# jdalcorso/radar-sounder-crw

Measured on AMD Instinct MI355X. Metric: radargram columns/sec (CRW fwd+bwd), higher is better.
Workload: dtype f32 (conv2-5 multiply on the bf16 matrix cores with hi/lo operand pairs, fp32 accumulate: fp32-grade; everything else fp32); 1 GPU; one synthetic 512x4096 radargram per GPU per step = 8 items [T=32,N=63,16x16] (patch 16x16, overlap (8, 0)), tau=0.01, CNN encoder, fwd+bwd+all-reduce+Adam; parallelism=dp1 (independent sequences), chain=fp32 MFMA 16x16x4, prefix form, encoder_convs=bf16x3

## Files before the change

include/crw_hip.h:

```cpp
#ifndef CRW_HIP_H
#define CRW_HIP_H

#include <stddef.h>
#include <stdint.h>

#ifdef __cplusplus
extern "C" {
#endif

#define CRW_ABI_VERSION 8

#define CRW_OK 0
#define CRW_EINVAL 1
#define CRW_EWORKSPACE 2
#define CRW_EHIP 3

#define CRW_CHAIN_F32 0
#define CRW_CHAIN_BF16 1
#define CRW_CHAIN_BF16X3 2

typedef void *crw_stream_t;

int crw_abi_version(void);
const char *crw_build_arch(void);
int crw_last_hip_error(void);

int crw_padded_nodes(int N, int chain);
size_t crw_walk_state_bytes(int B, int T, int N, int chain);
size_t crw_walk_scratch_bytes(int B, int T, int N, int chain);

size_t crw_affinity_ws_bytes(int B, int T, int N);
int crw_affinity_fwd(const float *emb, int B, int T, int N, int C, float tau,
                     float *ehat, float *norm, float *A, float *stats, void *ws, size_t ws_bytes, crw_stream_t stream);

int crw_walk_fwd(const float *A, const float *stats , int B, int T, int N,
                 int chain, void *state, size_t state_bytes, float *At_out, float *loss, crw_stream_t stream);

int crw_walk_bwd(const float *gloss, const float *A, int B, int T, int N, int chain,
                 void *state, size_t state_bytes, void *scratch, size_t scratch_bytes,
                 float *dA, crw_stream_t stream);

int crw_affinity_bwd(const float *dA, const float *ehat, const float *norm, int B, int T, int N, int C,
                     float tau, float *dehat_ws, float *demb, crw_stream_t stream);

int crw_normalize(const float *emb, int rows, int C, float *ehat, float *norm, crw_stream_t stream);

int crw_labelprop_topk(const float *ehat, int T, int N, int C, int cxt_size, int radius, float temp,
                       int knn, int first_frame, float *W, int32_t *I, crw_stream_t stream);
int crw_labelprop_topk_grid(const float *ehat, int T, int N, int C, int cxt_size, int radius, float temp, int knn, int first_frame,
                            int grid_w, float *W, int32_t *I, crw_stream_t stream);

int crw_labelprop_gather(const float *seed, const float *W, const int32_t *I, int T, int N, int M, int knn,
                         int first_frame, float *L, float *pred, crw_stream_t stream);
int crw_labelprop_propagate(const float *seed, const float *W, const int32_t *I, int T, int N, int M, int knn, int first_frame,
                            int cxt_size, float *L, float *pred, crw_stream_t stream);

int crw_labelprop_topk_scores(const float *ehat, int T, int N, int C, int cxt_size, int radius, float temp, int kcap, int first_frame,
                              int grid_w, float *V, int32_t *I, crw_stream_t stream);
int crw_labelprop_sweep_weights(const float *V, int F, int kcap, int N, const int *knns, int nk, float *W, crw_stream_t stream);
int crw_labelprop_propagate_batch(const float *seed, const float *W, const int32_t *I, size_t i_stride, int G, int T, int N, int M,
                                  int knn, int first_frame, int cxt_size, float *L, float *pred, crw_stream_t stream);

int crw_pelt_rbf(const double *signal, int n, double pen, int min_size, int jump, double gamma, int *bkps, int max_bkps);

int crw_xent_metric(const float *ehat, int T, int N, int C, float *xent, crw_stream_t stream);

#define CRW_DT_F32 0
#define CRW_DT_I8 1
size_t crw_confusion_ws_bytes(size_t P, int K);
int crw_confusion(const void *gt, int gt_dtype, const void *pred, int pred_dtype, const void *aux, int aux_dtype, size_t P, int K,
                  int ignore_gt, int ignore_pred, int ignore_aux, int64_t *counts ,
                  int64_t *dropped , void *ws, size_t ws_bytes, crw_stream_t stream);

#define CRW_CONF_MAXPROB 0
#define CRW_CONF_MARGIN 1
#define CRW_CONF_ENTROPY 2
int crw_labelprop_confidence(const float *L, int T, int N, int M, int kind, int first_frame, float *conf, crw_stream_t stream);

int crw_merge_confidence(const void *fwd_lab, const float *fwd_conf, const void *rev_lab, const float *rev_conf, int lab_dtype,
                         size_t P, void *out_lab, float *out_conf, uint8_t *took, crw_stream_t stream);

size_t crw_calibration_ws_bytes(size_t P, int K, int bins);
int crw_calibration(const void *gt, int gt_dtype, const void *pred, int pred_dtype, const float *conf, const void *aux, int aux_dtype,
                    size_t P, int K, int bins, int ignore_gt, int ignore_pred, int ignore_aux, int64_t *counts ,
                    double *conf_sum , int64_t *dropped , void *ws, size_t ws_bytes, crw_stream_t stream);

size_t crw_linear128_wgrad_ws_bytes(int P);
int crw_linear128_wgrad(const float *dy, const float *x, float *dw, int P, void *ws, size_t ws_bytes, crw_stream_t stream);

int crw_adam_step(float *p, const float *g, float *m, float *v, long n, float lr, float beta1, float beta2, float eps, int step,
                  crw_stream_t stream);

int crw_gemm_f32(const float *A, const float *B, float *C, int n, int batch, int transA, int transB,
                 int beta, crw_stream_t stream);

int crw_enc_pack_weights(const float *w, int cout, int cin, uint16_t *fwd_hi, uint16_t *fwd_lo,
                         uint16_t *bwd_hi, uint16_t *bwd_lo, crw_stream_t stream);
int crw_enc_pack_input(const float *x, int P, int C, uint16_t *x_hi, uint16_t *x_lo, crw_stream_t stream);
int crw_enc_pack_input_map(const float *x, int P, int C, int H, int W, uint16_t *x_hi, uint16_t *x_lo,
                           crw_stream_t stream);
int crw_enc_conv3x3(int mode, int split, int P, int cin, int cout, const uint16_t *x_hi, const uint16_t *x_lo,
                    const uint16_t *w_hi, const uint16_t *w_lo, const float *bias, const uint16_t *mask_hi,
                    uint16_t *y_hi, uint16_t *y_lo, float *y_f32, float *gap, const float *dgap,
                    crw_stream_t stream);
int crw_enc_conv3x3_map(int mode, int split, int P, int H, int W, int cin, int cout, const uint16_t *x_hi, const uint16_t *x_lo,
                        const uint16_t *w_hi, const uint16_t *w_lo, const float *bias, const uint16_t *mask_hi,
                        uint16_t *y_hi, uint16_t *y_lo, float *y_f32, float *gap_part, crw_stream_t stream);
int crw_enc_conv3x3_wgrad_map(int split, int P, int H, int W, int cin, int cout, const uint16_t *dy_hi, const uint16_t *dy_lo,
                              const uint16_t *x_hi, const uint16_t *x_lo, float *dw, float *db, void *ws, size_t ws_bytes,
                              crw_stream_t stream);
int crw_enc_gap_bwd(const float *dgap, const uint16_t *y_hi, int P, int C, int npix, uint16_t *dy_hi, uint16_t *dy_lo,
                    crw_stream_t stream);
size_t crw_enc_wgrad_ws_bytes(int P, int cin, int cout, int split);
int crw_enc_conv3x3_wgrad(int split, int P, int cin, int cout, const uint16_t *dy_hi, const uint16_t *dy_lo,
                          const uint16_t *x_hi, const uint16_t *x_lo, const float *dgap, float *dw, float *db,
                          void *ws, size_t ws_bytes, crw_stream_t stream);

int crw_enc_front_pack(const float *w2, uint16_t *fwd_hi, uint16_t *fwd_lo, uint16_t *bwd_hi, uint16_t *bwd_lo,
                       crw_stream_t stream);
size_t crw_enc_front_saved_bytes(int P);
int crw_enc_front_fwd(int split, const float *x, int P, int cin, const float *w1, const float *b1,
                      const uint16_t *w2_hi, const uint16_t *w2_lo, const float *b2, uint16_t *y_hi,
                      uint16_t *y_lo, void *saved, crw_stream_t stream);
int crw_enc_front_fwd_map(int split, const float *x, int P, int cin, int H, int W, const float *w1, const float *b1,
                          const uint16_t *w2_hi, const uint16_t *w2_lo, const float *b2, uint16_t *y_hi, uint16_t *y_lo,
                          crw_stream_t stream);
size_t crw_enc_front_ws_bytes(int P, int cin);
int crw_enc_front_bwd(int split, const float *x, int P, int cin, const float *w1, const float *b1,
                      const uint16_t *w2_hi, const uint16_t *w2_lo, const float *b2, const uint16_t *w2b_hi,
                      const uint16_t *w2b_lo, const float *dy, const void *saved, float *dw1, float *db1, float *dw2,
                      float *db2, void *ws, size_t ws_bytes, crw_stream_t stream);

int crw_enc_front_bwd_map(int split, const float *x, int P, int cin, int H, int W, const float *w1, const float *b1,
                          const uint16_t *w2_hi, const uint16_t *w2_lo, const float *b2, const uint16_t *w2b_hi,
                          const uint16_t *w2b_lo, const float *dy, float *dw1, float *db1, float *dw2, float *db2,
                          void *ws, size_t ws_bytes, crw_stream_t stream);

int crw_rn_padded_patches(int P);
int crw_rn_pack_conv(const float *w, int cout, int cin, int kh, int kw, uint16_t *fwd_hi, uint16_t *fwd_lo, uint16_t *bwd_hi,
                     uint16_t *bwd_lo, crw_stream_t stream);
int crw_rn_stem_toeplitz_ld(int w);
int crw_rn_stem_cols(int w);
int crw_rn_pack_stem(const float *w1, int h, int w, uint16_t *fwd_hi, uint16_t *fwd_lo, uint16_t *toep_hi, uint16_t *toep_lo,
                     crw_stream_t stream);
size_t crw_rn_conv_part_floats(int P, int G, int N);
int crw_rn_conv(int mode, int P, int Hs, int Ws, int Cs, int Hd, int Wd, int N, int kh, int kw, int stride, int pad,
                const uint16_t *a_hi, const uint16_t *a_lo, const uint16_t *b_hi, const uint16_t *b_lo, const float *bias, float *out,
                float *part, crw_stream_t stream);
size_t crw_rn_wgrad_ws_bytes(int mode, int P, int Hin, int Win, int Cin, int Hout, int Wout, int Cout, int kh, int kw, int stride, int pad);
int crw_rn_wgrad(int mode, int P, int Hin, int Win, int Cin, int Hout, int Wout, int Cout, int kh, int kw, int stride, int pad,
                 const uint16_t *x_hi, const uint16_t *x_lo, const uint16_t *d_hi, const uint16_t *d_lo, float *dw, void *ws,
                 size_t ws_bytes, crw_stream_t stream);
size_t crw_rn_bn_stats_ws_bytes(int C);
int crw_rn_bn_stats(const float *part, int P, int G, int C, const float *gamma, const float *beta, float *run_mean, float *run_var,
                    float momentum, float eps, float *coef, void *ws, size_t ws_bytes, crw_stream_t stream);
int crw_rn_bn_stats_rows(const float *part, int rows, double count, int C, const float *gamma, const float *beta, float *run_mean,
                         float *run_var, float momentum, float eps, float *coef, void *ws, size_t ws_bytes, crw_stream_t stream);
int crw_rn_bn_apply(const float *Z, const float *coef, const float *Zd, const float *coef_d, const uint16_t *res_hi,
                    const uint16_t *res_lo, int P, int npix, int C, int relu, uint16_t *y_hi, uint16_t *y_lo, crw_stream_t stream);
int crw_rn_bn_pool(const float *Z, const float *coef, int P, int H, int W, int C, uint16_t *y_hi, uint16_t *y_lo, uint8_t *amax,
                   crw_stream_t stream);
size_t crw_rn_bn_bwd_ws_bytes(int P, int npix, int C);
int crw_rn_bn_bwd(const float *g1, const float *g2, const uint16_t *mask_hi, const float *Z, const float *coef, const float *Zd,
                  const float *coef_d, int P, int npix, int C, uint16_t *dz_hi, uint16_t *dz_lo, uint16_t *dzd_hi, uint16_t *dzd_lo,
                  float *g_out, float *dgamma, float *dbeta, float *dgamma_d, float *dbeta_d, void *ws, size_t ws_bytes,
                  crw_stream_t stream);
size_t crw_rn_pool_bwd_ws_bytes(int P, int H, int W, int C);
int crw_rn_pool_bwd(const float *d1, const float *d2, const uint8_t *amax, const float *Z, const float *coef, int P, int H, int W, int C,
                    uint16_t *dz_hi, uint16_t *dz_lo, float *dgamma, float *dbeta, void *ws, size_t ws_bytes, crw_stream_t stream);
size_t crw_rn_stem_ws_bytes(void);
int crw_rn_stem_fwd(const float *x, int P, int cin, int h, int w, int Hm, int Wm, const float *w0, const float *b0, const float *gamma,
                    const float *beta, float *run_mean, float *run_var, float momentum, float eps, uint16_t *map_hi, uint16_t *map_lo,
                    float *stem, void *ws, size_t ws_bytes, crw_stream_t stream);
int crw_rn_stem_bwd(const float *dX0, const float *x, const float *stem, const float *w0, const float *b0, int P, int cin, int h, int w,
                    float *dw0, float *db0, float *dgamma, float *dbeta, void *ws, size_t ws_bytes, crw_stream_t stream);
int crw_rn_stem_stats(const float *x, int P, int cin, int h, int w, const float *w0, const float *b0, const float *gamma, const float *beta,
                      float *run_mean, float *run_var, float momentum, float eps, float *stem, void *ws, size_t ws_bytes,
                      crw_stream_t stream);
int crw_rn_stem16_rows(void);
int crw_rn_pack_stem16(const float *w1, uint16_t *wf, uint16_t *wt, crw_stream_t stream);
int crw_rn_stem16_fwd(const float *x, int P, int cin, const float *stem, const uint16_t *wf, float *Z1, float *part, crw_stream_t stream);
int crw_rn_stem_band_ok(int h, int w);
int crw_rn_stem_band_fwd(const float *x, int P, int cin, int h, int w, const float *stem, const uint16_t *wf, float *Z1, float *part,
                         crw_stream_t stream);
size_t crw_rn_stem16_ws_bytes(void);
int crw_rn_stem16_wgrad(const float *x, int P, int cin, const float *stem, const uint16_t *dz_hi, const uint16_t *dz_lo, float *dw, void *ws,
                        size_t ws_bytes, crw_stream_t stream);
int crw_rn_stem16_bwd(const float *x, int P, int cin, const float *stem, const float *w0, const float *b0, const uint16_t *wt,
                      const uint16_t *dz_hi, const uint16_t *dz_lo, float *dw0, float *db0, float *dgamma, float *dbeta, void *ws,
                      size_t ws_bytes, crw_stream_t stream);
int crw_rn_split(const float *x, int P, int C, uint16_t *hi, uint16_t *lo, crw_stream_t stream);
size_t crw_rn_colsum_ws_bytes(int C);
int crw_rn_colsum(const float *x, int rows, int C, float *out, void *ws, size_t ws_bytes, crw_stream_t stream);

#define CRW_RN_NPARAM 42
#define CRW_RN_NBN 13
size_t crw_rn_train_ws_bytes(int P, int cin, int h, int w);
int crw_rn_train_fwd(const float *x, int P, int cin, int h, int w, const float *const *prm, float *const *run_mean,
                     float *const *run_var, float momentum, float eps, float *out, void *ws, size_t ws_bytes, crw_stream_t stream);
int crw_rn_train_bwd(const float *dout, const float *x, int P, int cin, int h, int w, const float *const *prm, float *const *grads,
                     void *ws, size_t ws_bytes, crw_stream_t stream);
int crw_rn_train_fwd_nograd(const float *x, int P, int cin, int h, int w, const float *const *prm, float *const *run_mean,
// ... 19 lines not shown
```

radar-sounder-crw_amd/crw_hip.py:

```python
import ctypes
import os

import torch

_HERE = os.path.dirname(os.path.abspath(__file__))
LIB_PATH = os.environ.get("CRW_HIP_LIB") or os.path.join(_HERE, "libcrw_hip.so")

HEADER_PATH = os.path.join(os.path.dirname(_HERE), "include", "crw_hip.h")


def _header_abi_version():
    import re
    m = re.search(r"^#define\s+CRW_ABI_VERSION\s+(\d+)", open(HEADER_PATH).read(), re.M)
    if not m:
        raise RuntimeError(f"no CRW_ABI_VERSION in {HEADER_PATH}")
    return int(m.group(1))


ABI_VERSION = _header_abi_version()
CRW_OK, CRW_EINVAL, CRW_EWORKSPACE, CRW_EHIP = 0, 1, 2, 3
CHAIN_F32, CHAIN_BF16, CHAIN_BF16X3 = 0, 1, 2
_ERR = {1: "CRW_EINVAL (bad shape / null pointer / unsupported size)",
        2: "CRW_EWORKSPACE (workspace too small)", 3: "CRW_EHIP (HIP launch failed)"}

_c_int, _c_f, _c_sz, _p = ctypes.c_int, ctypes.c_float, ctypes.c_size_t, ctypes.c_void_p

SIGNATURES = {
    "crw_abi_version": (_c_int, []),
    "crw_build_arch": (ctypes.c_char_p, []),
    "crw_last_hip_error": (_c_int, []),
    "crw_padded_nodes": (_c_int, [_c_int, _c_int]),
    "crw_walk_state_bytes": (_c_sz, [_c_int, _c_int, _c_int, _c_int]),
    "crw_walk_scratch_bytes": (_c_sz, [_c_int, _c_int, _c_int, _c_int]),
    "crw_affinity_ws_bytes": (_c_sz, [_c_int, _c_int, _c_int]),
    "crw_affinity_fwd": (_c_int, [_p, _c_int, _c_int, _c_int, _c_int, _c_f, _p, _p, _p, _p, _p, _c_sz, _p]),
    "crw_walk_fwd": (_c_int, [_p, _p, _c_int, _c_int, _c_int, _c_int, _p, _c_sz, _p, _p, _p]),
    "crw_walk_bwd": (_c_int, [_p, _p, _c_int, _c_int, _c_int, _c_int, _p, _c_sz, _p, _c_sz, _p, _p]),
    "crw_affinity_bwd": (_c_int, [_p, _p, _p, _c_int, _c_int, _c_int, _c_int, _c_f, _p, _p, _p]),
    "crw_normalize": (_c_int, [_p, _c_int, _c_int, _p, _p, _p]),
    "crw_labelprop_topk": (_c_int, [_p, _c_int, _c_int, _c_int, _c_int, _c_int, _c_f, _c_int, _c_int, _p, _p, _p]),
    "crw_labelprop_topk_grid": (_c_int, [_p, _c_int, _c_int, _c_int, _c_int, _c_int, _c_f, _c_int, _c_int, _c_int, _p, _p, _p]),
    "crw_labelprop_gather": (_c_int, [_p, _p, _p, _c_int, _c_int, _c_int, _c_int, _c_int, _p, _p, _p]),
    "crw_pelt_rbf": (_c_int, [_p, _c_int, ctypes.c_double, _c_int, _c_int, ctypes.c_double, _p, _c_int]),
    "crw_labelprop_propagate": (_c_int, [_p, _p, _p, _c_int, _c_int, _c_int, _c_int, _c_int, _c_int, _p, _p, _p]),
    "crw_labelprop_topk_scores": (_c_int, [_p, _c_int, _c_int, _c_int, _c_int, _c_int, _c_f, _c_int, _c_int, _c_int, _p, _p, _p]),
    "crw_labelprop_sweep_weights": (_c_int, [_p, _c_int, _c_int, _c_int, _p, _c_int, _p, _p]),
    "crw_labelprop_propagate_batch": (_c_int, [_p, _p, _p, _c_sz] + [_c_int] * 7 + [_p, _p, _p]),
    "crw_xent_metric": (_c_int, [_p, _c_int, _c_int, _c_int, _p, _p]),
    "crw_confusion_ws_bytes": (_c_sz, [_c_sz, _c_int]),
    "crw_confusion": (_c_int, [_p, _c_int, _p, _c_int, _p, _c_int, _c_sz, _c_int, _c_int, _c_int, _c_int, _p, _p, _p, _c_sz, _p]),
    "crw_labelprop_confidence": (_c_int, [_p, _c_int, _c_int, _c_int, _c_int, _c_int, _p, _p]),
    "crw_merge_confidence": (_c_int, [_p, _p, _p, _p, _c_int, _c_sz, _p, _p, _p, _p]),
    "crw_calibration_ws_bytes": (_c_sz, [_c_sz, _c_int, _c_int]),
    "crw_calibration": (_c_int, [_p, _c_int, _p, _c_int, _p, _p, _c_int, _c_sz, _c_int, _c_int, _c_int, _c_int, _c_int, _p, _p, _p, _p,
                                 _c_sz, _p]),
    "crw_linear128_wgrad_ws_bytes": (_c_sz, [_c_int]),
    "crw_linear128_wgrad": (_c_int, [_p, _p, _p, _c_int, _p, _c_sz, _p]),
    "crw_adam_step": (_c_int, [_p, _p, _p, _p, ctypes.c_long, ctypes.c_float, ctypes.c_float, ctypes.c_float, ctypes.c_float,
                               _c_int, _p]),
    "crw_gemm_f32": (_c_int, [_p, _p, _p, _c_int, _c_int, _c_int, _c_int, _c_int, _p]),
    "crw_enc_pack_weights": (_c_int, [_p, _c_int, _c_int, _p, _p, _p, _p, _p]),
    "crw_enc_pack_input": (_c_int, [_p, _c_int, _c_int, _p, _p, _p]),
    "crw_enc_pack_input_map": (_c_int, [_p, _c_int, _c_int, _c_int, _c_int, _p, _p, _p]),
    "crw_enc_conv3x3_map": (_c_int, [_c_int, _c_int, _c_int, _c_int, _c_int, _c_int, _c_int, _p, _p, _p, _p, _p, _p, _p, _p, _p, _p, _p]),
    "crw_enc_conv3x3_wgrad_map": (_c_int, [_c_int, _c_int, _c_int, _c_int, _c_int, _c_int, _p, _p, _p, _p, _p, _p, _p, _c_sz, _p]),
    "crw_enc_conv3x3": (_c_int, [_c_int, _c_int, _c_int, _c_int, _c_int, _p, _p, _p, _p, _p, _p, _p, _p, _p, _p, _p, _p]),
    "crw_enc_gap_bwd": (_c_int, [_p, _p, _c_int, _c_int, _c_int, _p, _p, _p]),
    "crw_enc_wgrad_ws_bytes": (_c_sz, [_c_int, _c_int, _c_int, _c_int]),
    "crw_enc_conv3x3_wgrad": (_c_int, [_c_int, _c_int, _c_int, _c_int, _p, _p, _p, _p, _p, _p, _p, _p, _c_sz, _p]),
    "crw_enc_front_pack": (_c_int, [_p, _p, _p, _p, _p, _p]),
    "crw_enc_front_saved_bytes": (_c_sz, [_c_int]),
    "crw_enc_front_fwd": (_c_int, [_c_int, _p, _c_int, _c_int, _p, _p, _p, _p, _p, _p, _p, _p, _p]),
    "crw_enc_front_fwd_map": (_c_int, [_c_int, _p, _c_int, _c_int, _c_int, _c_int, _p, _p, _p, _p, _p, _p, _p, _p]),
    "crw_enc_front_ws_bytes": (_c_sz, [_c_int, _c_int]),
    "crw_enc_front_bwd": (_c_int, [_c_int, _p, _c_int, _c_int, _p, _p, _p, _p, _p, _p, _p, _p, _p, _p, _p, _p, _p, _p,
                                   _c_sz, _p]),
    "crw_enc_front_bwd_map": (_c_int, [_c_int, _p, _c_int, _c_int, _c_int, _c_int, _p, _p, _p, _p, _p, _p, _p, _p, _p, _p, _p, _p, _p,
                                       _c_sz, _p]),
    "crw_rn_padded_patches": (_c_int, [_c_int]),
    "crw_rn_pack_conv": (_c_int, [_p, _c_int, _c_int, _c_int, _c_int, _p, _p, _p, _p, _p]),
    "crw_rn_stem_toeplitz_ld": (_c_int, [_c_int]),
    "crw_rn_pack_stem": (_c_int, [_p, _c_int, _c_int, _p, _p, _p, _p, _p]),
    "crw_rn_conv_part_floats": (_c_sz, [_c_int, _c_int, _c_int]),
    "crw_rn_conv": (_c_int, [_c_int] * 12 + [_p] * 8),
    "crw_rn_wgrad_ws_bytes": (_c_sz, [_c_int] * 12),
    "crw_rn_wgrad": (_c_int, [_c_int] * 12 + [_p] * 6 + [_c_sz, _p]),
    "crw_rn_bn_stats_ws_bytes": (_c_sz, [_c_int]),
    "crw_rn_bn_stats": (_c_int, [_p, _c_int, _c_int, _c_int, _p, _p, _p, _p, _c_f, _c_f, _p, _p, _c_sz, _p]),
    "crw_rn_bn_apply": (_c_int, [_p, _p, _p, _p, _p, _p, _c_int, _c_int, _c_int, _c_int, _p, _p, _p]),
    "crw_rn_bn_pool": (_c_int, [_p, _p, _c_int, _c_int, _c_int, _c_int, _p, _p, _p, _p]),
    "crw_rn_bn_bwd_ws_bytes": (_c_sz, [_c_int, _c_int, _c_int]),
    "crw_rn_bn_bwd": (_c_int, [_p] * 7 + [_c_int] * 3 + [_p] * 10 + [_c_sz, _p]),
    "crw_rn_pool_bwd_ws_bytes": (_c_sz, [_c_int] * 4),
    "crw_rn_pool_bwd": (_c_int, [_p] * 5 + [_c_int] * 4 + [_p] * 5 + [_c_sz, _p]),
    "crw_rn_stem_ws_bytes": (_c_sz, []),
    "crw_rn_stem_fwd": (_c_int, [_p] + [_c_int] * 6 + [_p] * 6 + [_c_f, _c_f] + [_p] * 4 + [_c_sz, _p]),
    "crw_rn_stem_bwd": (_c_int, [_p] * 5 + [_c_int] * 4 + [_p] * 5 + [_c_sz, _p]),
    "crw_rn_split": (_c_int, [_p, _c_int, _c_int, _p, _p, _p]),
    "crw_rn_colsum_ws_bytes": (_c_sz, [_c_int]),
    "crw_rn_colsum": (_c_int, [_p, _c_int, _c_int, _p, _p, _c_sz, _p]),
    "crw_rn_bn_stats_rows": (_c_int, [_p, _c_int, ctypes.c_double, _c_int, _p, _p, _p, _p, _c_f, _c_f, _p, _p, _c_sz, _p]),
    "crw_rn_stem_stats": (_c_int, [_p] + [_c_int] * 4 + [_p] * 6 + [_c_f, _c_f, _p, _p, _c_sz, _p]),
    "crw_rn_stem16_rows": (_c_int, []),
    "crw_rn_pack_stem16": (_c_int, [_p, _p, _p, _p]),
    "crw_rn_stem16_fwd": (_c_int, [_p, _c_int, _c_int, _p, _p, _p, _p, _p]),
    "crw_rn_stem_band_ok": (_c_int, [_c_int, _c_int]),
    "crw_rn_stem_band_fwd": (_c_int, [_p, _c_int, _c_int, _c_int, _c_int, _p, _p, _p, _p, _p]),
    "crw_rn_stem16_ws_bytes": (_c_sz, []),
    "crw_rn_stem16_wgrad": (_c_int, [_p, _c_int, _c_int, _p, _p, _p, _p, _p, _c_sz, _p]),
    "crw_rn_stem16_bwd": (_c_int, [_p, _c_int, _c_int] + [_p] * 11 + [_c_sz, _p]),
    "crw_rn_train_ws_bytes": (_c_sz, [_c_int] * 4),
    "crw_rn_train_fwd": (_c_int, [_p] + [_c_int] * 4 + [_p, _p, _p, _c_f, _c_f, _p, _p, _c_sz, _p]),
    "crw_rn_train_fwd_nograd": (_c_int, [_p] + [_c_int] * 4 + [_p, _p, _p, _c_f, _c_f, _p, _p, _c_sz, _p]),
    "crw_rn_train_bwd": (_c_int, [_p, _p] + [_c_int] * 4 + [_p, _p, _p, _c_sz, _p]),
    "crw_rn_eval_fwd": (_c_int, [_p] + [_c_int] * 4 + [_p, _p, _p, _c_f, _p, _p, _c_sz, _p]),
    "crw_rn_stem_cols": (_c_int, [_c_int]),
    "crw_rn_timing_enable": (_c_int, [_c_int]),
    "crw_rn_timing_read": (_c_int, [_p, _c_int]),
    "crw_gemm_bf16_ws_bytes": (_c_sz, [_c_int, _c_int, _c_int]),
    "crw_gemm_bf16": (_c_int, [_p, _p, _p, _c_int, _c_int, _c_int, _c_int, _c_int, _c_int, _p, _c_sz, _c_int, _p]),
}

SWEEP_ENTRY_POINTS = ("crw_labelprop_topk_scores", "crw_labelprop_sweep_weights", "crw_labelprop_propagate_batch")

CONFIDENCE_ENTRY_POINTS = ("crw_labelprop_confidence", "crw_merge_confidence", "crw_calibration_ws_bytes", "crw_calibration")

_lib = None
_has_sweep = False
_has_confidence = False


def lib():
    global _lib, _has_sweep, _has_confidence
    if _lib is None:
        if not os.path.exists(LIB_PATH):
            raise RuntimeError(f"{LIB_PATH} not built -- the CRW hot path has no CPU/PyTorch fallback; "
                               "run `make -C radar-sounder-crw_amd/csrc` (hipcc --offload-arch=gfx950)")
        handle = ctypes.CDLL(LIB_PATH)
        missing = [n for n in SWEEP_ENTRY_POINTS + CONFIDENCE_ENTRY_POINTS if not hasattr(handle, n)]
        for name, (res, args) in SIGNATURES.items():
            if name in missing:
                continue
            fn = getattr(handle, name)
            fn.restype, fn.argtypes = res, args
        if handle.crw_abi_version() != ABI_VERSION:
            raise RuntimeError(f"{LIB_PATH} was built for ABI {handle.crw_abi_version()}, include/crw_hip.h says {ABI_VERSION}: "
                               "stale library -- rebuild with `make -C radar-sounder-crw_amd/csrc`")
        _lib = handle
        _has_sweep = not set(missing) & set(SWEEP_ENTRY_POINTS)
        _has_confidence = not set(missing) & set(CONFIDENCE_ENTRY_POINTS)
    return _lib


def has_sweep():
    lib()
    return _has_sweep


def _sweep_lib():
    if not has_sweep():
        raise RuntimeError(f"{LIB_PATH} is a stale libcrw_hip.so: it reports ABI {ABI_VERSION} but lacks {', '.join(SWEEP_ENTRY_POINTS)} "
                           "(added at that ABI) -- rebuild with `make -C radar-sounder-crw_amd/csrc`")
    return lib()


def has_confidence():
    lib()
    return _has_confidence


def _confidence_lib():
    if not has_confidence():
        raise RuntimeError(f"{LIB_PATH} is a stale libcrw_hip.so: it reports ABI {ABI_VERSION} but lacks "
                           f"{', '.join(CONFIDENCE_ENTRY_POINTS)} (added at that ABI) -- rebuild with `make -C radar-sounder-crw_amd/csrc`")
    return lib()


class CrwError(RuntimeError):

    def __init__(self, what, status, hip_error):
        super().__init__(f"{what} failed: {_ERR.get(status, status)} (hipError {hip_error})")
        self.what, self.status, self.hip_error = what, status, hip_error

    @property
    def device_failure(self):
        return self.status != CRW_EINVAL


def _check(status, what):
    if status != CRW_OK:
        raise CrwError(what, status, lib().crw_last_hip_error())


def _dev(t, name, dtype=torch.float32):
    if not t.is_cuda:
        raise RuntimeError(f"{name} must live on an MI355X device (got {t.device}); the HIP path has no CPU fallback")
    if t.dtype != dtype or not t.is_contiguous():
        raise RuntimeError(f"{name} must be contiguous {dtype}")
    return ctypes.c_void_p(t.data_ptr())


def _stream():
    return ctypes.c_void_p(torch.cuda.current_stream().cuda_stream)


KERNEL_EVENTS = None


def _ev_begin():
    if KERNEL_EVENTS is None:
        return None
    e = torch.cuda.Event(enable_timing=True)
    e.record()
    return e


def _ev_end(e0, key):
    if e0 is not None:
        e1 = torch.cuda.Event(enable_timing=True)
        e1.record()
        KERNEL_EVENTS.setdefault(key, []).append((e0, e1))


def padded_nodes(N, chain=CHAIN_F32):
    return lib().crw_padded_nodes(N, chain)


def affinity_fwd(emb, tau, want_stats=True):
    B, T, N, C = emb.shape
    ehat = torch.empty_like(emb)
    norm = torch.empty(B, T, N, device=emb.device, dtype=torch.float32)
    A = torch.empty(B, T - 1, N, N, device=emb.device, dtype=torch.float32)
    stats = ws = None
    nbytes = 0
    if want_stats and T > 1:
        stats = torch.empty(4, B, T - 1, N, device=emb.device, dtype=torch.float32)
        nbytes = lib().crw_affinity_ws_bytes(B, T, N)
        ws = torch.empty(max(nbytes, 16), dtype=torch.uint8, device=emb.device)
    _check(lib().crw_affinity_fwd(_dev(emb, "emb"), B, T, N, C, float(tau), _dev(ehat, "ehat"), _dev(norm, "norm"),
                                  _dev(A, "A"), _dev(stats, "stats") if stats is not None else None,
                                  ctypes.c_void_p(ws.data_ptr()) if ws is not None else None, nbytes, _stream()), "crw_affinity_fwd")
    return A, ehat, norm, stats


def affinity_bwd(dA, ehat, norm, tau):
    B, T, N, C = ehat.shape
    ws = torch.empty_like(ehat)
    demb = torch.empty_like(ehat)
    _check(lib().crw_affinity_bwd(_dev(dA, "dA"), _dev(ehat, "ehat"), _dev(norm, "norm"), B, T, N, C, float(tau),
                                  _dev(ws, "ws"), _dev(demb, "demb"), _stream()), "crw_affinity_bwd")
    return demb


def walk_fwd(A, chain=CHAIN_F32, want_At=False, stats=None):
    B, Tm1, N, _ = A.shape
    T = Tm1 + 1
    nbytes = lib().crw_walk_state_bytes(B, T, N, chain)
# ... 328 lines not shown
    n = torch.bincount(row, minlength=bins + 3)
    ok = torch.bincount(row, weights=(binned & (g == p)).to(torch.float64), minlength=bins + 3).to(torch.int64)
    s = torch.bincount(row, weights=torch.where(binned, c.to(torch.float64), torch.zeros(1, dtype=torch.float64)), minlength=bins + 3)
    return torch.stack([n[:bins], ok[:bins]], 1), s[:bins], n[bins:]


def gemm_f32(A, B, C=None, transA=False, transB=False, beta=False):
    batch, n, _ = A.shape
    if C is None:
        C = torch.empty_like(A)
    _check(lib().crw_gemm_f32(_dev(A, "A"), _dev(B, "B"), _dev(C, "C"), n, batch, int(transA), int(transB), int(beta),
                              _stream()), "crw_gemm_f32")
    return C


def gemm_bf16(A, B, C=None, transA=False, transB=False, beta=False, split=1, ws=None, convert=True):
    batch, n, _ = A.shape
    if C is None:
        C = torch.empty_like(A)
    nbytes = lib().crw_gemm_bf16_ws_bytes(n, batch, split)
    if ws is None:
        ws = torch.empty(nbytes, dtype=torch.uint8, device=A.device)
    _check(lib().crw_gemm_bf16(_dev(A, "A"), _dev(B, "B"), _dev(C, "C"), n, batch, int(transA), int(transB),
                               int(beta), int(split), ctypes.c_void_p(ws.data_ptr()), ws.numel(), int(convert),
                               _stream()), "crw_gemm_bf16")
    return C, ws


_BF = torch.bfloat16


def _bf(t, name):
    return _dev(t, name, _BF) if t is not None else None


def enc_pack_weights(w, split):
    cout, cin = w.shape[:2]
    mk = lambda a, b: torch.empty(9, a, b, dtype=_BF, device=w.device)
    fh, bh = mk(cout, cin), mk(cin, cout)
    fl, bl = (mk(cout, cin), mk(cin, cout)) if split == 3 else (None, None)
    _check(lib().crw_enc_pack_weights(_dev(w.contiguous(), "w"), cout, cin, _bf(fh, "fh"), _bf(fl, "fl"), _bf(bh, "bh"),
                                      _bf(bl, "bl"), _stream()), "crw_enc_pack_weights")
    return fh, fl, bh, bl


def enc_pack_input(x, split):
    P, C, H, W = x.shape
    if (H, W) != (10, 10):
        raise RuntimeError(f"the HIP conv stack handles 10x10 feature maps (16x16 patches), got {H}x{W}")
    xh = torch.empty(P, 100, C, dtype=_BF, device=x.device)
    xl = torch.empty_like(xh) if split == 3 else None
    _check(lib().crw_enc_pack_input(_dev(x.contiguous(), "x"), P, C, _bf(xh, "xh"), _bf(xl, "xl"), _stream()),
           "crw_enc_pack_input")
    return xh, xl


def enc_conv3x3(mode, split, xh, xl, wh, wl, cout, bias=None, mask=None, planes=True, f32=False, gap=False,
                dgap=None, lo_plane=True):
    P, _, cin = xh.shape
    dev = xh.device
    yh = torch.empty(P, 100, cout, dtype=_BF, device=dev) if planes else None
    yl = torch.empty_like(yh) if (planes and split == 3 and lo_plane) else None
    yf = torch.empty(P, 100, cout, dtype=torch.float32, device=dev) if f32 else None
    gp = torch.empty(P, cout, dtype=torch.float32, device=dev) if gap else None
    ev = _ev_begin()
    _check(lib().crw_enc_conv3x3(mode, split, P, cin, cout, _bf(xh, "xh"), _bf(xl, "xl"), _bf(wh, "wh"), _bf(wl, "wl"),
                                 _dev(bias, "bias") if bias is not None else None, _bf(mask, "mask"), _bf(yh, "yh"),
                                 _bf(yl, "yl"), _dev(yf, "yf") if f32 else None, _dev(gp, "gap") if gap else None,
                                 _dev(dgap, "dgap") if dgap is not None else None, _stream()), "crw_enc_conv3x3")
    _ev_end(ev, ("fwd", cin, cout) if mode == 0 else ("bwd", cout, cin))
    return yh, yl, yf, gp


def linear128_wgrad(dy, x):
    P = x.shape[0]
    dw = torch.empty(128, 128, dtype=torch.float32, device=x.device)
    nbytes = lib().crw_linear128_wgrad_ws_bytes(P)
    ws = torch.empty(nbytes, dtype=torch.uint8, device=x.device)
    _check(lib().crw_linear128_wgrad(_dev(dy.contiguous(), "dy"), _dev(x.contiguous(), "x"), _dev(dw, "dw"), P,
                                     ctypes.c_void_p(ws.data_ptr()), nbytes, _stream()), "crw_linear128_wgrad")
    return dw


def adam_step(p, g, m, v, step, lr, beta1=0.9, beta2=0.999, eps=1e-8):
    _check(lib().crw_adam_step(_dev(p, "p"), _dev(g, "g"), _dev(m, "m"), _dev(v, "v"), p.numel(), float(lr), float(beta1),
                               float(beta2), float(eps), int(step), _stream()), "crw_adam_step")


def enc_pack_input_map(x, split):
    P, C, H, W = x.shape
    xh = torch.empty(P, H * W, C, dtype=_BF, device=x.device)
    xl = torch.empty_like(xh) if split == 3 else None
    _check(lib().crw_enc_pack_input_map(_dev(x.contiguous(), "x"), P, C, H, W, _bf(xh, "xh"), _bf(xl, "xl"), _stream()),
           "crw_enc_pack_input_map")
    return xh, xl


def enc_conv3x3_map(split, xh, xl, wh, wl, cout, H, W, bias=None, planes=True, gap=False, lo_plane=True, mode=0, mask=None,
                    f32=False):
    P, hw, cin = xh.shape
    assert hw == H * W
    dev = xh.device
    yh = torch.empty(P, hw, cout, dtype=_BF, device=dev) if planes else None
    yl = torch.empty_like(yh) if (planes and split == 3 and lo_plane) else None
    yf = torch.empty(P, hw, cout, dtype=torch.float32, device=dev) if f32 else None
    ntile = ((H + 9) // 10) * ((W + 9) // 10)
    gp = torch.empty(P, ntile, cout, dtype=torch.float32, device=dev) if gap else None
    ev = _ev_begin()
    _check(lib().crw_enc_conv3x3_map(mode, split, P, H, W, cin, cout, _bf(xh, "xh"), _bf(xl, "xl"), _bf(wh, "wh"), _bf(wl, "wl"),
                                     _dev(bias, "bias") if bias is not None else None, _bf(mask, "mask"), _bf(yh, "yh"),
                                     _bf(yl, "yl"), _dev(yf, "yf") if f32 else None, _dev(gp, "gap") if gap else None, _stream()),
           "crw_enc_conv3x3_map")
    _ev_end(ev, ("fwd_map", cin, cout) if mode == 0 else ("bwd_map", cout, cin))
    if mode == 1:
        return yh, yl, yf
    return yh, yl, (gp.sum(1) / float(hw) if gap else None)


def enc_wgrad_map(split, dyh, dyl, xh, xl, H, W):
    P, hw, cout = dyh.shape
    cin = xh.shape[2]
    assert hw == H * W
    dw = torch.empty(cout, cin, 3, 3, dtype=torch.float32, device=xh.device)
    db = torch.empty(cout, dtype=torch.float32, device=xh.device)
    units = P * ((H + 9) // 10) * ((W + 9) // 10)
    nbytes = lib().crw_enc_wgrad_ws_bytes(units, cin, cout, split)
    ws = torch.empty(nbytes, dtype=torch.uint8, device=xh.device)
    ev = _ev_begin()
    _check(lib().crw_enc_conv3x3_wgrad_map(split, P, H, W, cin, cout, _bf(dyh, "dyh"), _bf(dyl, "dyl"), _bf(xh, "xh"),
                                           _bf(xl, "xl"), _dev(dw, "dw"), _dev(db, "db"), ctypes.c_void_p(ws.data_ptr()), nbytes,
                                           _stream()), "crw_enc_conv3x3_wgrad_map")
    _ev_end(ev, ("wgrad_map", cin, cout))
    return dw, db


def enc_gap_bwd(dgap, yh, split):
    P, npix, C = yh.shape
    dh = torch.empty_like(yh)
    dl = torch.empty_like(yh) if split == 3 else None
    _check(lib().crw_enc_gap_bwd(_dev(dgap.contiguous(), "dgap"), _bf(yh, "yh"), P, C, npix, _bf(dh, "dh"), _bf(dl, "dl"),
                                 _stream()), "crw_enc_gap_bwd")
    return dh, dl


def enc_wgrad(split, dyh, dyl, xh, xl, dgap=None):
    P, _, cout = dyh.shape
    cin = xh.shape[2]
    dw = torch.empty(cout, cin, 3, 3, dtype=torch.float32, device=xh.device)
    db = torch.empty(cout, dtype=torch.float32, device=xh.device)
    nbytes = lib().crw_enc_wgrad_ws_bytes(P, cin, cout, split)
    ws = torch.empty(nbytes, dtype=torch.uint8, device=xh.device)
    ev = _ev_begin()
    _check(lib().crw_enc_conv3x3_wgrad(split, P, cin, cout, _bf(dyh, "dyh"), _bf(dyl, "dyl"), _bf(xh, "xh"),
                                       _bf(xl, "xl"), _dev(dgap, "dgap") if dgap is not None else None,
                                       _dev(dw, "dw"), _dev(db, "db"), ctypes.c_void_p(ws.data_ptr()),
                                       nbytes, _stream()), "crw_enc_conv3x3_wgrad")
    _ev_end(ev, ("wgrad", cin, cout))
    return dw, db


def enc_front_pack(w2, split):
    fh = torch.empty(7, 32, 32, dtype=_BF, device=w2.device)
    bh = torch.empty(25, 8, 32, dtype=_BF, device=w2.device)
    fl, bl = (torch.empty_like(fh), torch.empty_like(bh)) if split == 3 else (None, None)
    _check(lib().crw_enc_front_pack(_dev(w2.contiguous(), "w2"), _bf(fh, "fh"), _bf(fl, "fl"), _bf(bh, "bh"),
                                    _bf(bl, "bl"), _stream()), "crw_enc_front_pack")
    return fh, fl, bh, bl


def enc_front_fwd(split, x, w1, b1, w2f, b2, save=False):
    P, cin = x.shape[:2]
    yh = torch.empty(P, 100, 32, dtype=_BF, device=x.device)
    yl = torch.empty_like(yh) if split == 3 else None
    saved = torch.empty(lib().crw_enc_front_saved_bytes(P), dtype=torch.uint8, device=x.device) if save else None
    ev = _ev_begin()
    _check(lib().crw_enc_front_fwd(split, _dev(x, "x"), P, cin, _dev(w1.contiguous(), "w1"), _dev(b1, "b1"),
                                   _bf(w2f[0], "w2h"), _bf(w2f[1], "w2l"), _dev(b2, "b2"), _bf(yh, "yh"), _bf(yl, "yl"),
                                   ctypes.c_void_p(saved.data_ptr()) if save else None, _stream()), "crw_enc_front_fwd")
    _ev_end(ev, ("front_fwd", cin, 32))
    return (yh, yl, saved) if save else (yh, yl)


def enc_front_fwd_map(split, x, w1, b1, w2f, b2):
    P, cin, H, W = x.shape
    yh = torch.empty(P, (H - 6) * (W - 6), 32, dtype=_BF, device=x.device)
    yl = torch.empty_like(yh) if split == 3 else None
    _check(lib().crw_enc_front_fwd_map(split, _dev(x.contiguous(), "x"), P, cin, H, W, _dev(w1.contiguous(), "w1"),
                                       _dev(b1, "b1"), _bf(w2f[0], "w2h"), _bf(w2f[1], "w2l"), _dev(b2, "b2"),
                                       _bf(yh, "yh"), _bf(yl, "yl"), _stream()), "crw_enc_front_fwd_map")
    return yh, yl


def enc_front_bwd(split, x, w1, b1, w2f, b2, w2b, dy, saved=None):
    P, cin = x.shape[:2]
    dev = x.device
    dw1 = torch.empty(8, cin, 5, 5, device=dev)
    db1 = torch.empty(8, device=dev)
    dw2 = torch.empty(32, 8, 5, 5, device=dev)
    db2 = torch.empty(32, device=dev)
    nbytes = lib().crw_enc_front_ws_bytes(P, cin)
    ws = torch.empty(nbytes, dtype=torch.uint8, device=dev)
    if saved is not None and saved.numel() < lib().crw_enc_front_saved_bytes(P):
        raise RuntimeError("saved record too small for this patch count")
    ev = _ev_begin()
    _check(lib().crw_enc_front_bwd(split, _dev(x, "x"), P, cin, _dev(w1.contiguous(), "w1"), _dev(b1, "b1"),
                                   _bf(w2f[0], "w2h"), _bf(w2f[1], "w2l"), _dev(b2, "b2"), _bf(w2b[0], "w2bh"),
                                   _bf(w2b[1], "w2bl"), _dev(dy.contiguous(), "dy"),
                                   ctypes.c_void_p(saved.data_ptr()) if saved is not None else None, _dev(dw1, "dw1"),
                                   _dev(db1, "db1"), _dev(dw2, "dw2"), _dev(db2, "db2"), ctypes.c_void_p(ws.data_ptr()), nbytes,
                                   _stream()), "crw_enc_front_bwd")
    _ev_end(ev, ("front_bwd", cin, 32))
    return dw1, db1, dw2, db2


def enc_front_bwd_map(split, x, w1, b1, w2f, b2, w2b, dy):
    P, cin, H, W = x.shape
    dev = x.device
    dw1 = torch.empty(8, cin, 5, 5, device=dev)
    db1 = torch.empty(8, device=dev)
    dw2 = torch.empty(32, 8, 5, 5, device=dev)
    db2 = torch.empty(32, device=dev)
    units = P * ((H - 6 + 9) // 10) * ((W - 6 + 9) // 10)
    nbytes = lib().crw_enc_front_ws_bytes(units, cin)
    ws = torch.empty(nbytes, dtype=torch.uint8, device=dev)
    _check(lib().crw_enc_front_bwd_map(split, _dev(x.contiguous(), "x"), P, cin, H, W, _dev(w1.contiguous(), "w1"), _dev(b1, "b1"),
                                       _bf(w2f[0], "w2h"), _bf(w2f[1], "w2l"), _dev(b2, "b2"), _bf(w2b[0], "w2bh"),
                                       _bf(w2b[1], "w2bl"), _dev(dy.contiguous(), "dy"), _dev(dw1, "dw1"), _dev(db1, "db1"),
                                       _dev(dw2, "dw2"), _dev(db2, "db2"), ctypes.c_void_p(ws.data_ptr()), nbytes, _stream()),
           "crw_enc_front_bwd_map")
    return dw1, db1, dw2, db2


RN_FWD, RN_BWD, RN_STEM_FWD, RN_STEM_BWD = 0, 1, 2, 3


def _ptr(t):
    return ctypes.c_void_p(t.data_ptr()) if t is not None else None


def _ws(nbytes, dev):
    return torch.empty(max(int(nbytes), 16), dtype=torch.uint8, device=dev)


def rn_padded(P):
    return lib().crw_rn_padded_patches(int(P))


def rn_pack_conv(w):
    w = w.detach()
    if w.dim() == 2:
# ... 319 lines not shown
```

radar-sounder-crw_amd/csrc/crw_common.h:

```cpp
#pragma once
#include <hip/hip_runtime.h>
#include <stdint.h>
#include <stddef.h>
#include "crw_hip.h"

namespace crw {

constexpr int WAVE = 64;

typedef float f32x4 __attribute__((ext_vector_type(4)));
typedef float f32x16 __attribute__((ext_vector_type(16)));
typedef short bf16x8 __attribute__((ext_vector_type(8)));

extern thread_local int g_last_hip_error;

inline void clear_stale_error() { (void)hipGetLastError(); }

inline int check_launch() {
  hipError_t e = hipGetLastError();
  if (e != hipSuccess) {
    g_last_hip_error = (int)e;
    return CRW_EHIP;
  }
  return CRW_OK;
}

#define CRW_TRY(expr)               \
  do {                              \
    int _st = (expr);               \
    if (_st != CRW_OK) return _st;  \
  } while (0)

inline int round_up(int x, int m) { return (x + m - 1) / m * m; }
inline size_t align_up(size_t x, size_t a) { return (x + a - 1) / a * a; }

inline int padded_nodes(int N) {
  if (N <= 128) return round_up(N, 32);
  if (N <= 1024) return round_up(N, 64);
  return round_up(N, 128);
}

__device__ inline float wave_max(float v) {
#pragma unroll
  for (int o = 32; o > 0; o >>= 1) v = fmaxf(v, __shfl_xor(v, o));
  return v;
}
__device__ inline float wave_sum(float v) {
#pragma unroll
  for (int o = 32; o > 0; o >>= 1) v += __shfl_xor(v, o);
  return v;
}

struct GemmProb {
  const void *A, *B, *A2, *B2;
  const void *Al, *Bl, *A2l, *B2l;
  float *C;
  void *Cb, *Cbl;
  long sA, sB, sA2, sB2, sC;
  int ta, tb, ta2, tb2;
  int beta;
};
constexpr int MAX_GROUP = 6;
struct GemmGroup {
  GemmProb p[MAX_GROUP];
  int nprob;
  int n;
  int batch;
};

int launch_gemm_group_f32(const GemmGroup &g, hipStream_t s);
int launch_gemm_group_bf16(const GemmGroup &g, int split, hipStream_t s);
int launch_split_bf16(const float *x, long count, void *hi, void *lo, hipStream_t s);

struct EdgeOperand {
  const float *p;
  long sb;
  long rs, cs;
};
struct EdgeGemm {
  EdgeOperand A, B, A2, B2;
  float *C;
  long sCb, ldc;
  int M, N, K, K2;
  int batch_inner;
  long sA_outer, sB_outer, sA2_outer, sB2_outer, sC_outer;
  int skip1_inner, skip2_inner;
  float scale;
  int divide;
};
int launch_edge_gemm(const EdgeGemm &g, int batch, hipStream_t s);
size_t affinity_part_floats(int B, int T, int N);
int launch_affinity_tiles(const float *ehat, int B, int T, int N, int C, float tau, float *A, float *stats, float *part,
                          hipStream_t s);
int launch_affinity_bwd_tiles(const float *dA, const float *ehat, int B, int T, int N, int C, float tau, float *dehat,
                              hipStream_t s);

int launch_softmax_fwd(const float *A, const float *stats_ext, int B, int Tm1, int N, int Np, float *F, float *Gt, void *Fh,
                       void *Fl, void *Gh, void *Gl, float *stats , hipStream_t s);
int launch_stats_dense(const float *A, int nmat, int N, float *stats, hipStream_t s);
int launch_softmax_bwd(const float *A, const float *stats, const float *dF, const float *dGt, int B, int Tm1, int N, int Np,
                       float *dots, float *dA, hipStream_t s);
int launch_chain_small_fwd(const float *Gt, const float *F, float *Lt, float *R, int B, int K, int n, hipStream_t s);
int launch_chain_small_bwd(const float *Gt, const float *F, float *dLt, float *dR, int B, int K, int n,
                           hipStream_t s);
int launch_identity(float *R, void *Rb, int batch, int Np, int N, hipStream_t s, float *copy_dst = nullptr,
                    const float *copy_src = nullptr);
int launch_copy_f32(float *dst, const float *src, long dst_bs, long src_bs, long n_per_batch, int batch,
                    hipStream_t s);
int launch_loss_rows(const float *At, int nmat, int N, int Np, float *lse, float *terms, hipStream_t s);
int launch_loss_reduce(const float *terms, long n, float scale, float *loss, hipStream_t s);
int launch_dAt(const float *At, const float *lse, const float *gloss, float coef, int nmat, int N, int Np,
               float *dAt, void *dAt_hi, void *dAt_lo, hipStream_t s);
int launch_unpad_At(const float *At, int K, int B, int N, int Np, float *out, hipStream_t s);

}
```

radar-sounder-crw_amd/csrc/encoder_conv.hip:

```cpp
#include "crw_common.h"
#include <type_traits>
#include <cstdlib>

namespace crw {
namespace {

constexpr int IMG_W = 10, PAD_W = 12, NPIX = 100, NPAD = 144, MT = 7;

typedef __bf16 bf8 __attribute__((ext_vector_type(8)));
typedef short s4v __attribute__((ext_vector_type(4)));
typedef short s8v __attribute__((ext_vector_type(8)));
typedef __attribute__((address_space(3))) char *lds_cp;

__device__ inline uint16_t f2bf(float x) { return __builtin_bit_cast(uint16_t, (__bf16)x); }
__device__ inline float bf2f(uint16_t h) { return __builtin_bit_cast(float, (uint32_t)h << 16); }

template <int C>
constexpr int row_stride() { return C * 2 + 16; }
template <int C>
constexpr int plane_bytes() { return NPAD * row_stride<C>(); }
template <int C>
__device__ inline int px_off(int pp, int chunk) { return pp * row_stride<C>() + 16 * chunk; }
template <int C>
constexpr int crs() { return C * 2 + 32; }
constexpr int PLANE_ROWS = NPAD - PAD_W;


__device__ inline int interior_pp(int i) { return (i / IMG_W + 1) * PAD_W + (i % IMG_W + 1); }

template <int C, int NTHREADS, int RS = row_stride<C>()>
struct PlaneLoad {
  static constexpr int NCH = C / 8, TOTAL = NPIX * NCH, ITER = (TOTAL + NTHREADS - 1) / NTHREADS;
  uint4 v[ITER];
  __device__ inline void load(const uint16_t *__restrict__ src, int tid) {
#pragma unroll
    for (int i = 0; i < ITER; ++i) {
      const int c = min(tid + i * NTHREADS, TOTAL - 1);
      v[i] = *reinterpret_cast<const uint4 *>(src + (long)c * 8);
    }
  }
  __device__ inline void store(char *dst, int tid) const {
#pragma unroll
    for (int i = 0; i < ITER; ++i) {
      const int c = tid + i * NTHREADS;
      if (TOTAL % NTHREADS == 0 || c < TOTAL)
        *reinterpret_cast<uint4 *>(dst + interior_pp(c / NCH) * RS + 16 * (c % NCH)) = v[i];
    }
  }
};

__device__ inline void gap_split8(const float *__restrict__ dg8, uint32_t (&gh)[4], uint32_t (&gl)[4]) {
#pragma clang fp contract(off)
  const float4 g0 = *reinterpret_cast<const float4 *>(dg8);
  const float4 g1 = *reinterpret_cast<const float4 *>(dg8 + 4);
  const float gv[8] = {g0.x, g0.y, g0.z, g0.w, g1.x, g1.y, g1.z, g1.w};
#pragma unroll
  for (int w = 0; w < 4; ++w) {
    const float a0 = gv[2 * w] * (1.0f / NPIX), a1 = gv[2 * w + 1] * (1.0f / NPIX);
    const uint16_t h0 = f2bf(a0), h1 = f2bf(a1);
    gh[w] = (uint32_t)h0 | ((uint32_t)h1 << 16);
    gl[w] = (uint32_t)f2bf(a0 - bf2f(h0)) | ((uint32_t)f2bf(a1 - bf2f(h1)) << 16);
  }
}
__device__ inline void gap_mask8(const uint4 &y, const uint32_t (&gh)[4], const uint32_t (&gl)[4], uint4 &oh, uint4 &ol) {
  const uint32_t yw[4] = {y.x, y.y, y.z, y.w};
  uint32_t h[4], l[4];
#pragma unroll
  for (int w = 0; w < 4; ++w) {
    const uint32_t m = ((yw[w] & 0x7fffu) ? 0xffffu : 0u) | ((yw[w] & 0x7fff0000u) ? 0xffff0000u : 0u);
    h[w] = gh[w] & m;
    l[w] = gl[w] & m;
  }
  oh = uint4{h[0], h[1], h[2], h[3]};
  ol = uint4{l[0], l[1], l[2], l[3]};
}

template <int C, int NTHREADS, int SPLIT, int RS = row_stride<C>()>
__device__ inline void gap_planes_to_lds(const uint16_t *__restrict__ yh, const float *__restrict__ dgap_row,
                                         char *dst_hi, char *dst_lo, int tid) {
  constexpr int NCH = C / 8, TOTAL = NPIX * NCH, ITER = (TOTAL + NTHREADS - 1) / NTHREADS;
  uint4 v[ITER];
#pragma unroll
  for (int i = 0; i < ITER; ++i) {
// ... 913 lines not shown
      load_dy(more ? n + 1 : n);
      load_x(xq >= 0 ? xq : 0, xpl);
    }
    kstep(n);
    if (DIAG == 2 || DIAG == 3) {
      if (DIAG & 1) continue;
      __syncthreads();
      continue;
    }
    if (DIAG == 4) {
      asm volatile("" ::"v"(sy[0].x), "v"(sy[NPL - 1].y), "v"(sx[0].x), "v"(sx[1].y));
      __syncthreads();
      continue;
    }
    if (more) store_dy(n + 1);
    if (xq >= 0) store_x(xq, xpl);
    if (a.dgap && q_2 >= 0) stage_gap(q_2);
    if (!(DIAG & 1)) __syncthreads();
  }

  float *dwp = a.dw_part + (long)wg_slice * COUT * CIN * 9;
#pragma unroll
  for (int tap = 0; tap < 9; ++tap)
#pragma unroll
    for (int j = 0; j < NCOW; ++j)
#pragma unroll
      for (int r = 0; r < 4; ++r) {
        const int co = co0w + 16 * j + 4 * g + r, ci = ci_base + 16 * wci + (lane & 15);
        dwp[((long)tap * COUT + co) * CIN + ci] = acc[tap][j][r];
      }
  if (bias_wg && (lane & 15) == 0) {
#pragma unroll
    for (int r = 0; r < 4; ++r) a.db_part[(long)wg_slice * COUT + co0w + 16 * wci + 4 * g + r] = accb[r];
  }
}

__global__ __launch_bounds__(256) void slice_sum_kernel(const float *__restrict__ part, int nslice, long n,
                                                        float *__restrict__ out) {
  for (long e = (long)blockIdx.x * 256 + threadIdx.x; e < n; e += (long)gridDim.x * 256) {
    float s = 0.f;
    for (int k = 0; k < nslice; ++k) s += part[(long)k * n + e];
    out[e] = s;
  }
}

__global__ __launch_bounds__(256) void slice_sum_dw_kernel(const float *__restrict__ part, int nslice, int coci,
                                                           float *__restrict__ out, int nblk_dw,
                                                           const float *__restrict__ bpart, int cout, float *__restrict__ bout) {
  __shared__ float red[4][64];
  const long n = 9L * coci;
  const int lane = threadIdx.x & 63, q = threadIdx.x >> 6;
  if ((int)blockIdx.x >= nblk_dw) {
    const int e = ((int)blockIdx.x - nblk_dw) * 4 + q;
    if (e >= cout) return;
    float s = 0.f;
    for (int k = lane; k < nslice; k += 64) s += bpart[(long)k * cout + e];
    s = wave_sum(s);
    if (lane == 0) bout[e] = s;
    return;
  }
  const long e = (long)blockIdx.x * 64 + lane;
  const int per = (nslice + 3) / 4, k0 = q * per, k1 = min(nslice, k0 + per);
  float s = 0.f;
  if (e < n) {
    int k = k0;
    for (; k + 8 <= k1; k += 8) {
      float v[8];
#pragma unroll
      for (int u = 0; u < 8; ++u) v[u] = part[(long)(k + u) * n + e];
#pragma unroll
      for (int u = 0; u < 8; ++u) s += v[u];
    }
    for (; k < k1; ++k) s += part[(long)k * n + e];
  }
  red[q][lane] = s;
  __syncthreads();
  if (q == 0 && e < n) {
    const float t = (red[0][lane] + red[1][lane]) + (red[2][lane] + red[3][lane]);
    const int tap = e / coci, cc = e % coci;
    out[(long)cc * 9 + tap] = t;
  }
}

__device__ inline long frag_index(int tap, int n, int k, int N, int K) {
  return ((((long)tap * (K / 32) + k / 32) * (N / 16) + n / 16) * 64 + ((k % 32) / 8) * 16 + n % 16) * 8 + k % 8;
}
__global__ __launch_bounds__(256) void pack_weights_kernel(const float *__restrict__ w, int CO, int CI,
                                                           uint16_t *fh, uint16_t *fl, uint16_t *bh, uint16_t *bl) {
  const long n = (long)CO * CI * 9;
  for (long e = (long)blockIdx.x * 256 + threadIdx.x; e < n; e += (long)gridDim.x * 256) {
    const int tap = e % 9, ci = (e / 9) % CI, co = e / (9L * CI);
    const float v = w[e];
    const uint16_t h = f2bf(v), l = f2bf(v - bf2f(h));
    const long of = frag_index(tap, co, ci, CO, CI), ob = frag_index(8 - tap, ci, co, CI, CO);
    fh[of] = h; bh[ob] = h;
    if (fl) { fl[of] = l; bl[ob] = l; }
  }
}

__global__ __launch_bounds__(256) void pack_input_kernel(const float *__restrict__ x, int P, int C, int npix, uint16_t *xh,
                                                         uint16_t *xl) {
  const long n = (long)P * npix * C;
  for (long e = (long)blockIdx.x * 256 + threadIdx.x; e < n; e += (long)gridDim.x * 256) {
    const int c = e % C, i = (e / C) % npix;
    const long p = e / ((long)C * npix);
    const float v = x[(p * C + c) * npix + i];
    const uint16_t h = f2bf(v);
    xh[e] = h;
    if (xl) xl[e] = f2bf(v - bf2f(h));
  }
}

__global__ __launch_bounds__(256) void gap_bwd_kernel(const float *__restrict__ dgap, const uint16_t *__restrict__ yh,
                                                      int P, int C, int npix, uint16_t *dh, uint16_t *dl) {
  const long n8 = (long)P * npix * C / 8;
  const int c8 = C / 8;
  const float inv = 1.0f / (float)npix;
  for (long e = (long)blockIdx.x * 256 + threadIdx.x; e < n8; e += (long)gridDim.x * 256) {
#pragma clang fp contract(off)
    const int c = (int)(e % c8) * 8;
    const long p = e / ((long)c8 * npix);
    const uint4 y = *reinterpret_cast<const uint4 *>(yh + e * 8);
    const float4 g0 = *reinterpret_cast<const float4 *>(dgap + p * C + c), g1 = *reinterpret_cast<const float4 *>(dgap + p * C + c + 4);
    const float gv[8] = {g0.x, g0.y, g0.z, g0.w, g1.x, g1.y, g1.z, g1.w};
    const uint32_t yw[4] = {y.x, y.y, y.z, y.w};
    uint32_t h[4], l[4];
#pragma unroll
    for (int w = 0; w < 4; ++w) {
      const float a0 = (yw[w] & 0x7fffu) ? gv[2 * w] * inv : 0.f, a1 = (yw[w] & 0x7fff0000u) ? gv[2 * w + 1] * inv : 0.f;
      const uint16_t h0 = f2bf(a0), h1 = f2bf(a1);
      h[w] = (uint32_t)h0 | ((uint32_t)h1 << 16);
      l[w] = (uint32_t)f2bf(a0 - bf2f(h0)) | ((uint32_t)f2bf(a1 - bf2f(h1)) << 16);
    }
    *reinterpret_cast<uint4 *>(dh + e * 8) = uint4{h[0], h[1], h[2], h[3]};
    if (dl) *reinterpret_cast<uint4 *>(dl + e * 8) = uint4{l[0], l[1], l[2], l[3]};
  }
}

template <int C>
constexpr size_t conv_lds_bytes(int npl) { return (size_t)(npl - 1) * PLANE_ROWS * crs<C>() + (size_t)NPAD * crs<C>(); }

template <int SPLIT, int CIN, int COUT, int MODE, int NW>
int launch_conv_nw(const ConvArgs &a, hipStream_t s) {
  constexpr int CMAX = CIN > COUT ? CIN : COUT;
  size_t lds = conv_lds_bytes<CMAX>(SPLIT == 3 ? 2 : 1);
#ifdef CRW_CONV_STAMPS
  if (const char *e = getenv("CRW_CONV_LDS_PAD")) lds += (size_t)atoi(e);
#endif
  static bool attr = false;
  if (!attr && lds > 64 * 1024) {
    if (hipFuncSetAttribute((const void *)conv3x3_kernel<SPLIT, CIN, COUT, MODE, NW>,
                            hipFuncAttributeMaxDynamicSharedMemorySize, (int)lds) != hipSuccess) {
      g_last_hip_error = (int)hipGetLastError();
      return CRW_EHIP;
    }
    attr = true;
  }
  hipLaunchKernelGGL((conv3x3_kernel<SPLIT, CIN, COUT, MODE, NW>), dim3(a.P), dim3(NW * 64), lds, s, a);
  return check_launch();
}

constexpr int MT_SMALL = 4;

template <int SPLIT, int CIN, int COUT, int MODE, int MTL>
int launch_conv_map_cls(const ConvArgs &a, hipStream_t s) {
  constexpr int CMAX = CIN > COUT ? CIN : COUT, NW = (SPLIT == 3 ? 8 : 4);
  const size_t lds = (size_t)(SPLIT == 3 ? 2 : 1) * NPAD * row_stride<CMAX>();
  static bool attr = false;
  if (!attr && lds > 64 * 1024) {
    if (hipFuncSetAttribute((const void *)conv3x3_kernel<SPLIT, CIN, COUT, MODE, NW, true, MTL>,
                            hipFuncAttributeMaxDynamicSharedMemorySize, (int)lds) != hipSuccess) {
      g_last_hip_error = (int)hipGetLastError();
      return CRW_EHIP;
    }
    attr = true;
  }
  hipLaunchKernelGGL((conv3x3_kernel<SPLIT, CIN, COUT, MODE, NW, true, MTL>), dim3(a.P * a.ncls), dim3(NW * 64), lds, s, a);
  return check_launch();
}

// ... 291 lines not shown
```

radar-sounder-crw_amd/csrc/encoder_front.hip:

```cpp
#include "crw_common.h"
#include <type_traits>
#include <cstdlib>

namespace crw {
namespace {

typedef __bf16 bf8 __attribute__((ext_vector_type(8)));
typedef short s4v __attribute__((ext_vector_type(4)));
typedef short s8v __attribute__((ext_vector_type(8)));
typedef __attribute__((address_space(3))) char *lds_cp;

__device__ inline uint16_t f2bf(float x) { return __builtin_bit_cast(uint16_t, (__bf16)x); }
__device__ inline float bf2f(uint16_t h) { return __builtin_bit_cast(float, (uint32_t)h << 16); }

__device__ inline void lds_barrier() { asm volatile("s_waitcnt lgkmcnt(0)\n\ts_barrier" ::: "memory"); }

constexpr int XPW = 18;
constexpr int C1W = 14, C1N = C1W * C1W;
constexpr int A1W = 13, A1PW = 15;
constexpr int C2W = 11, C2N = C2W * C2W;
constexpr int OW = 10, ON = 100;
constexpr int D2PW = 19;
constexpr int D2HALF = D2PW * D2PW * 32;
constexpr int KS2 = 7;
constexpr int NTH = 1024, NWV = NTH / 64;

constexpr int SV_A1 = 169 * 16, SV_K2 = 100 * 32, SV_K1 = 1360;
constexpr int SV_OFF_A1L = SV_A1, SV_OFF_K2 = 2 * SV_A1, SV_OFF_K1 = 2 * SV_A1 + SV_K2, SV_BYTES = 2 * SV_A1 + SV_K2 + SV_K1;
static_assert(SV_BYTES % 16 == 0 && SV_A1 % 16 == 0 && SV_K2 % 16 == 0, "16-byte chunks");

struct FrontArgs {
  const float *x;
  const float *w1, *b1;
  const uint16_t *w2h, *w2l;
  const float *b2;
  uint16_t *yh, *yl;
  int P, cin;
  char *saved;
};

template <bool PAD>
__device__ inline int c1_idx(int y, int x) { return PAD ? (y + 1) * (C1W + 2) + x + 1 : y * C1W + x; }
template <bool PAD>
__device__ inline int c2_idx(int y, int x) { return PAD ? (y + 1) * (C2W + 2) + x + 1 : y * C2W + x; }

struct FwdLds {
  float *xs;
  float *w1;
  float *c1r;
  char *a1h, *a1l;
  char *w2h, *w2l;
  float *c2r;
};

template <bool PAD>
__device__ inline void conv1_relu(const FwdLds &L, int cin, int tid) {
  if (tid < C1N * 2) {
    const int pix = tid >> 1, c0 = 4 * (tid & 1);
    const int y = pix / C1W, xx = pix % C1W;
    float4 acc = *reinterpret_cast<const float4 *>(L.w1 + 8 * cin * 25 + c0);
    for (int ci = 0; ci < cin; ++ci) {
      const float *xs = L.xs + (ci * XPW + y) * XPW + xx;
      const float *w = L.w1 + ci * 25 * 8 + c0;
#pragma unroll
      for (int t = 0; t < 25; ++t) {
        const float v = xs[(t / 5) * XPW + t % 5];
        const float4 wv = *reinterpret_cast<const float4 *>(w + t * 8);
        acc.x = fmaf(v, wv.x, acc.x);
        acc.y = fmaf(v, wv.y, acc.y);
        acc.z = fmaf(v, wv.z, acc.z);
        acc.w = fmaf(v, wv.w, acc.w);
      }
    }
    *reinterpret_cast<float4 *>(L.c1r + c1_idx<PAD>(y, xx) * 8 + c0) = float4{fmaxf(acc.x, 0.f), fmaxf(acc.y, 0.f), fmaxf(acc.z, 0.f), fmaxf(acc.w, 0.f)};
  }
}

__device__ inline int argmax4(float a, float b, float c, float d);
template <int SPLIT, bool PAD, int NT = NTH>
__device__ inline void pool1(const FwdLds &L, int tid, char *sv = nullptr) {
  constexpr int ROW = (PAD ? C1W + 2 : C1W) * 8;
  for (int e = tid; e < A1W * A1W * 8; e += NT) {
    const int c = e & 7, p = e >> 3, y = p / A1W, x = p % A1W;
// ... 145 lines not shown
  FwdLds L;
  L.xs = (float *)take(sizeof(float) * cin * MXW * MXW);
  L.w1 = (float *)take(sizeof(float) * (8 * cin * 25 + 8));
  L.c1r = (float *)take(sizeof(float) * MC1W * MC1W * 8);
  L.a1h = take(A1PW * A1PW * 16);
  L.a1l = take(A1PW * A1PW * 16);
  L.w2h = take(KS2 * 32 * 32 * 2);
  L.w2l = take(KS2 * 32 * 32 * 2);
  L.c2r = (float *)take(sizeof(float) * C2N * 32);
  for (int e = tid; e < 8 * cin * 25; e += NT) {
    const int t = e % 25, ci = (e / 25) % cin, co = e / (25 * cin);
    L.w1[(ci * 25 + t) * 8 + co] = a.f.w1[e];
  }
  if (tid < 8) L.w1[8 * cin * 25 + tid] = a.f.b1[tid];
  for (int e = tid; e < KS2 * 32 * 32 / 8; e += NT) {
    const int d = w2_lds_chunk(e);
    reinterpret_cast<uint4 *>(L.w2h)[d] = reinterpret_cast<const uint4 *>(a.f.w2h)[e];
    if (SPLIT == 3) reinterpret_cast<uint4 *>(L.w2l)[d] = reinterpret_cast<const uint4 *>(a.f.w2l)[e];
  }
  const float b2r = a.f.b2[16 * ((tid >> 6) & 1) + (tid & 15)];
  const int H = a.H, W = a.W, Ho = H - 6, Wo = W - 6, ntile = a.tiles_x * a.tiles_y;
  const long nwork = (long)a.f.P * ntile;
  __syncthreads();
  for (long wk = blockIdx.x; wk < nwork; wk += gridDim.x) {
    const int pt = (int)(wk / ntile), tile = (int)(wk % ntile);
    const int oy0 = (tile / a.tiles_x) * OW, ox0 = (tile % a.tiles_x) * OW;
    for (int e = tid; e < cin * MXW * MXW; e += NT) {
      const int ci = e / (MXW * MXW), r = (e / MXW) % MXW, c = e % MXW;
      const int iy = oy0 + r - 2, ix = ox0 + c - 2;
      L.xs[e] = (iy >= 0 && iy < H && ix >= 0 && ix < W) ? a.f.x[(((long)pt * cin + ci) * H + iy) * W + ix] : 0.f;
    }
    lds_barrier();
    if (tid < MC1W * MC1W * 2) {
      const int pix = tid >> 1, c0 = 4 * (tid & 1);
      const int y = pix / MC1W, xx = pix % MC1W;
      float4 acc = *reinterpret_cast<const float4 *>(L.w1 + 8 * cin * 25 + c0);
      for (int ci = 0; ci < cin; ++ci) {
        const float *xs = L.xs + (ci * MXW + y) * MXW + xx;
        const float *w = L.w1 + ci * 25 * 8 + c0;
#pragma unroll
        for (int t = 0; t < 25; ++t) {
          const float v = xs[(t / 5) * MXW + t % 5];
          const float4 wv = *reinterpret_cast<const float4 *>(w + t * 8);
          acc.x = fmaf(v, wv.x, acc.x);
          acc.y = fmaf(v, wv.y, acc.y);
          acc.z = fmaf(v, wv.z, acc.z);
          acc.w = fmaf(v, wv.w, acc.w);
        }
      }
      *reinterpret_cast<float4 *>(L.c1r + pix * 8 + c0) = float4{fmaxf(acc.x, 0.f), fmaxf(acc.y, 0.f), fmaxf(acc.z, 0.f), fmaxf(acc.w, 0.f)};
    }
    lds_barrier();
    for (int e = tid; e < A1PW * A1PW * 8; e += NT) {
      const int c = e & 7, q = e >> 3, r = q / A1PW, cc = q % A1PW;
      const int ay = oy0 + r - 1, ax = ox0 + cc - 1;
      float v = 0.f;
      if (ay >= 0 && ay < H - 3 && ax >= 0 && ax < W - 3) {
        const float *s1 = L.c1r + (r * MC1W + cc) * 8 + c;
        v = fmaxf(fmaxf(s1[0], s1[8]), fmaxf(s1[MC1W * 8], s1[MC1W * 8 + 8]));
      }
      const uint16_t h = f2bf(v);
      *reinterpret_cast<uint16_t *>(L.a1h + q * 16 + 2 * c) = h;
      if (SPLIT == 3) *reinterpret_cast<uint16_t *>(L.a1l + q * 16 + 2 * c) = f2bf(v - bf2f(h));
    }
    lds_barrier();
    conv2_relu<SPLIT, false, NT>(L, b2r, tid);
    lds_barrier();
    for (int e = tid; e < ON * 32; e += NT) {
      const int c = e & 31, q = e >> 5, y = q / OW, x = q % OW;
      if (oy0 + y < Ho && ox0 + x < Wo) {
        const float *s2 = L.c2r + (y * C2W + x) * 32 + c;
        const float v = fmaxf(fmaxf(s2[0], s2[32]), fmaxf(s2[C2W * 32], s2[C2W * 32 + 32]));
        const uint16_t h = f2bf(v);
        const long o = (((long)pt * Ho + oy0 + y) * Wo + ox0 + x) * 32 + c;
        a.f.yh[o] = h;
        if (SPLIT == 3) a.f.yl[o] = f2bf(v - bf2f(h));
      }
    }
  }
}

__global__ __launch_bounds__(256) void pack_w2_kernel(const float *__restrict__ w, uint16_t *fh, uint16_t *fl,
                                                      uint16_t *bh, uint16_t *bl) {
  for (int e = blockIdx.x * 256 + threadIdx.x; e < KS2 * 32 * 32; e += gridDim.x * 256) {
    const int k = e & 31, co = (e >> 5) & 31, s = e >> 10;
    const int tap = 4 * s + (k >> 3), ci = k & 7;
    const float v = tap < 25 ? w[(co * 8 + ci) * 25 + tap] : 0.f;
    const uint16_t h = f2bf(v);
    fh[e] = h;
    if (fl) fl[e] = f2bf(v - bf2f(h));
  }
  for (int e = blockIdx.x * 256 + threadIdx.x; e < 25 * 8 * 32; e += gridDim.x * 256) {
    const int co = e & 31, ci = (e >> 5) & 7, tap = e >> 8;
    const float v = w[(co * 8 + ci) * 25 + tap];
    const uint16_t h = f2bf(v);
    bh[e] = h;
    if (bl) bl[e] = f2bf(v - bf2f(h));
  }
}

struct FrontBwdArgs {
  FrontArgs f;
  const uint16_t *w2bh, *w2bl;
  const float *dy;
  float *part;
  int patches_per_block;
  long long *stamps;
  int H, W, tiles_x, tiles_y;
};
[[maybe_unused]] constexpr int NPHASE = 10;
#ifdef CRW_CONV_STAMPS
#define FRONT_STAMP(k)                                                       \
  if (a.stamps && tid == 0) {                                                \
    const long long now_ = (long long)__builtin_amdgcn_s_memtime();          \
    phase_[k] += now_ - prev_;                                               \
    prev_ = now_;                                                            \
  }
#else
#define FRONT_STAMP(k)
#endif

__device__ inline s4v tr_read0(uint32_t lds_addr) {
  s4v v;
  asm volatile("ds_read_b64_tr_b16 %0, %1" : "=v"(v) : "v"(lds_addr) : "memory");
  return v;
}
__device__ inline bf8 tr_pair(uint32_t a_lo, uint32_t a_hi) {
  const s4v lo = tr_read0(a_lo), hi = tr_read0(a_hi);
  const s8v v = {lo[0], lo[1], lo[2], lo[3], hi[0], hi[1], hi[2], hi[3]};
  return __builtin_bit_cast(bf8, v);
}

__device__ inline int argmax4(float a, float b, float c, float d) {
  int k = 0;
  float m = a;
  if (b > m) { m = b; k = 1; }
  if (c > m) { m = c; k = 2; }
  if (d > m) { m = d; k = 3; }
  return k;
}

template <int W, int CS>
__device__ inline float pool_bwd_pixel(const float *__restrict__ in, const float *__restrict__ dout, int y, int x, int c) {
  const float *ctr = in + ((y + 1) * (W + 2) + x + 1) * CS + c;
  float nb[3][3], dv[2][2];
#pragma unroll
  for (int dy = 0; dy < 3; ++dy)
#pragma unroll
    for (int dx = 0; dx < 3; ++dx) nb[dy][dx] = ctr[((dy - 1) * (W + 2) + (dx - 1)) * CS];
#pragma unroll
  for (int dyw = 0; dyw < 2; ++dyw)
#pragma unroll
    for (int dxw = 0; dxw < 2; ++dxw) {
      const int wy = min(max(y - dyw, 0), W - 2), wx = min(max(x - dxw, 0), W - 2);
      dv[dyw][dxw] = dout[(wy * (W - 1) + wx) * CS + c];
    }
  const float mine = nb[1][1];
  float gsum = 0.f;
#pragma unroll
  for (int dyw = 0; dyw < 2; ++dyw)
#pragma unroll
    for (int dxw = 0; dxw < 2; ++dxw) {
      const int wy = y - dyw, wx = x - dxw;
      bool win = mine > 0.f && wy >= 0 && wy < W - 1 && wx >= 0 && wx < W - 1;
      const int k = dyw * 2 + dxw;
#pragma unroll
      for (int j = 0; j < 4; ++j)
        if (j != k) {
          const float v = nb[1 - dyw + (j >> 1)][1 - dxw + (j & 1)];
          win = win && (j < k ? mine > v : mine >= v);
        }
      gsum += win ? dv[dyw][dxw] : 0.f;
    }
  return gsum;
}

template <int SPLIT>
__global__ __launch_bounds__(NTH) void front_bwd_kernel(FrontBwdArgs a) {
  extern __shared__ __attribute__((aligned(16))) char lds[];
  char *p = lds;
  const int cin = a.f.cin;
// ... 970 lines not shown
```

radar-sounder-crw_amd/csrc/gemm_f32.hip:

```cpp
#include "crw_common.h"
#include <cstdlib>

namespace crw {

thread_local int g_last_hip_error = 0;

namespace {

constexpr int BK = 16;

template <int R>
struct Stager {
  static constexpr int NV4 = R * BK / 4;
  static constexpr int PER = (NV4 + 255) / 256;
  float4 v[PER];

  __device__ inline void load(const float *__restrict__ X, int n, int r0, int k0, bool kcontig, int tid) {
#pragma unroll
    for (int i = 0; i < PER; ++i) {
      int e = tid + i * 256;
      if (NV4 % 256 == 0 || e < NV4) {
        if (kcontig) {
          int r = e >> 2, kq = e & 3;
          v[i] = *reinterpret_cast<const float4 *>(X + (long)(r0 + r) * n + k0 + 4 * kq);
        } else {
          int k = e / (R / 4), rq = e % (R / 4);
          v[i] = *reinterpret_cast<const float4 *>(X + (long)(k0 + k) * n + r0 + 4 * rq);
        }
      }
    }
  }
  template <int LD>
  __device__ inline void store(float *S, bool kcontig, int tid) const {
#pragma unroll
    for (int i = 0; i < PER; ++i) {
      int e = tid + i * 256;
      if (NV4 % 256 == 0 || e < NV4) {
        if (kcontig) {
          int r = e >> 2, kq = e & 3;
          S[(4 * kq + 0) * LD + r] = v[i].x;
          S[(4 * kq + 1) * LD + r] = v[i].y;
          S[(4 * kq + 2) * LD + r] = v[i].z;
          S[(4 * kq + 3) * LD + r] = v[i].w;
        } else {
          int k = e / (R / 4), rq = e % (R / 4);
          *reinterpret_cast<float4 *>(S + k * LD + 4 * rq) = v[i];
        }
      }
    }
  }
};

template <int BM, int BN>
__global__ __launch_bounds__(256) void gemm_pad_f32_kernel(GemmGroup g) {
  constexpr int LDA = BM + 16, LDB = BN + 16;
  constexpr int TM = BM / 2 / 16, TN = BN / 2 / 16;
  __shared__ __attribute__((aligned(16))) float lds[BK * LDA + BK * LDB];
  float *As = lds, *Bs = lds + BK * LDA;

  const GemmProb &p = g.p[blockIdx.z];
  const int n = g.n;
  const int tiles_n = n / BN;
  const int m0 = (blockIdx.x / tiles_n) * BM, n0 = (blockIdx.x % tiles_n) * BN;
  const long b = blockIdx.y;
  const int tid = threadIdx.x, lane = tid & 63, wave = tid >> 6;
  const int wm = (wave >> 1) * (BM / 2), wn = (wave & 1) * (BN / 2);

  const int nk = n / BK;
  const int nprod = p.A2 ? 2 : 1;
  const int nt = nk * nprod;

  f32x4 acc[TM][TN];
#pragma unroll
  for (int i = 0; i < TM; ++i)
#pragma unroll
    for (int j = 0; j < TN; ++j) acc[i][j] = f32x4{0.f, 0.f, 0.f, 0.f};

  Stager<BM> sa;
  Stager<BN> sb;
  auto issue = [&](int t) {
    const bool second = t >= nk;
    const int k0 = (second ? t - nk : t) * BK;
    const float *A = second ? (const float *)p.A2 + b * p.sA2 : (const float *)p.A + b * p.sA;
    const float *Bp = second ? (const float *)p.B2 + b * p.sB2 : (const float *)p.B + b * p.sB;
    const bool ta = second ? p.ta2 : p.ta, tb = second ? p.tb2 : p.tb;
    sa.load(A, n, m0, k0, !ta, tid);
    sb.load(Bp, n, n0, k0, tb, tid);
  };
  auto commit = [&](int t) {
    const bool second = t >= nk;
    const bool ta = second ? p.ta2 : p.ta, tb = second ? p.tb2 : p.tb;
    sa.template store<LDA>(As, !ta, tid);
    sb.template store<LDB>(Bs, tb, tid);
  };

  issue(0);
  for (int t = 0; t < nt; ++t) {
    commit(t);
    __syncthreads();
    if (t + 1 < nt) issue(t + 1);
#pragma unroll
    for (int kk = 0; kk < BK; kk += 4) {
      float a[TM], bv[TN];
      const int kr = kk + (lane >> 4), c = lane & 15;
#pragma unroll
      for (int i = 0; i < TM; ++i) a[i] = As[kr * LDA + wm + i * 16 + c];
#pragma unroll
      for (int j = 0; j < TN; ++j) bv[j] = Bs[kr * LDB + wn + j * 16 + c];
#pragma unroll
      for (int i = 0; i < TM; ++i)
#pragma unroll
        for (int j = 0; j < TN; ++j) acc[i][j] = __builtin_amdgcn_mfma_f32_16x16x4f32(a[i], bv[j], acc[i][j], 0, 0, 0);
    }
    __syncthreads();
  }

  float *C = p.C + b * p.sC;
#pragma unroll
  for (int i = 0; i < TM; ++i)
#pragma unroll
    for (int j = 0; j < TN; ++j) {
      const int col = n0 + wn + j * 16 + (lane & 15);
#pragma unroll
      for (int r = 0; r < 4; ++r) {
        const int row = m0 + wm + i * 16 + (lane >> 4) * 4 + r;
        float v = acc[i][j][r];
        float *dst = C + (long)row * n + col;
        if (p.beta) v += *dst;
        *dst = v;
      }
    }
}

constexpr int EB = 64, ELD = 65;

__device__ inline void edge_stage(const float *__restrict__ base, long rs, long cs, bool a_side, int R, int K,
                                  int r0, int k0, float *S, int tid) {
  const long sr = a_side ? rs : cs, sk = a_side ? cs : rs;
  const bool kfast = (sk == 1);
#pragma unroll
  for (int i = 0; i < EB * BK / 256; ++i) {
    int e = tid + i * 256;
    int k, r;
    if (kfast) { k = e % BK; r = e / BK; } else { r = e % EB; k = e / EB; }
    float v = 0.f;
    if (r0 + r < R && k0 + k < K) v = base[(long)(r0 + r) * sr + (long)(k0 + k) * sk];
    S[k * ELD + r] = v;
  }
}

__global__ __launch_bounds__(256) void edge_gemm_kernel(EdgeGemm g) {
  __shared__ float As[BK * ELD], Bs[BK * ELD];
  const int tid = threadIdx.x, lane = tid & 63, wave = tid >> 6;
  const int m0 = blockIdx.y * EB, n0 = blockIdx.x * EB;
  const int outer = blockIdx.z / g.batch_inner, inner = blockIdx.z % g.batch_inner;
  const int wm = (wave >> 1) * 32, wn = (wave & 1) * 32;

  f32x4 acc[2][2];
#pragma unroll
  for (int i = 0; i < 2; ++i)
#pragma unroll
    for (int j = 0; j < 2; ++j) acc[i][j] = f32x4{0.f, 0.f, 0.f, 0.f};

  for (int prod = 0; prod < 2; ++prod) {
    const EdgeOperand &oa = prod ? g.A2 : g.A;
    const EdgeOperand &ob = prod ? g.B2 : g.B;
    if (oa.p == nullptr) continue;
    if (inner == (prod ? g.skip2_inner : g.skip1_inner)) continue;
    const int K = prod ? g.K2 : g.K;
    const float *A = oa.p + (long)outer * (prod ? g.sA2_outer : g.sA_outer) + (long)inner * oa.sb;
    const float *Bp = ob.p + (long)outer * (prod ? g.sB2_outer : g.sB_outer) + (long)inner * ob.sb;
    for (int k0 = 0; k0 < K; k0 += BK) {
      edge_stage(A, oa.rs, oa.cs, true, g.M, K, m0, k0, As, tid);
      edge_stage(Bp, ob.rs, ob.cs, false, g.N, K, n0, k0, Bs, tid);
      __syncthreads();
#pragma unroll
      for (int kk = 0; kk < BK; kk += 4) {
        const int kr = kk + (lane >> 4), c = lane & 15;
        float a[2], bv[2];
#pragma unroll
        for (int i = 0; i < 2; ++i) a[i] = As[kr * ELD + wm + i * 16 + c];
#pragma unroll
        for (int j = 0; j < 2; ++j) bv[j] = Bs[kr * ELD + wn + j * 16 + c];
#pragma unroll
        for (int i = 0; i < 2; ++i)
#pragma unroll
          for (int j = 0; j < 2; ++j)
            acc[i][j] = __builtin_amdgcn_mfma_f32_16x16x4f32(a[i], bv[j], acc[i][j], 0, 0, 0);
      }
      __syncthreads();
    }
  }

  float *C = g.C + (long)outer * g.sC_outer + (long)inner * g.sCb;
#pragma unroll
  for (int i = 0; i < 2; ++i)
#pragma unroll
    for (int j = 0; j < 2; ++j) {
      const int col = n0 + wn + j * 16 + (lane & 15);
#pragma unroll
      for (int r = 0; r < 4; ++r) {
        const int row = m0 + wm + i * 16 + (lane >> 4) * 4 + r;
        if (row < g.M && col < g.N) {
          float v = acc[i][j][r];
          C[(long)row * g.ldc + col] = g.divide ? v / g.scale : v * g.scale;
        }
      }
    }
}

template <int R>
struct BoundStager {
  static constexpr int NV4 = R * BK / 4, PER = (NV4 + 255) / 256;
  float4 v[PER];
  template <bool AL = true>
  __device__ inline void load(const float *__restrict__ X, long ld, int r0, int k0, bool kcontig, int rmax, int kmax, int tid) {
#pragma unroll
    for (int i = 0; i < PER; ++i) {
      const int e = min(tid + i * 256, NV4 - 1);
      if (kcontig) {
        const int r = e >> 2, k = k0 + 4 * (e & 3);
        if constexpr (AL) {
          const float4 t = *reinterpret_cast<const float4 *>(X + (long)min(r0 + r, rmax - 1) * ld + min(k, kmax - 4));
          v[i] = k < kmax ? t : float4{0.f, 0.f, 0.f, 0.f};
        } else {
          const float *row = X + (long)min(r0 + r, rmax - 1) * ld;
          float t[4];
#pragma unroll
          for (int u = 0; u < 4; ++u) {
            const float x = row[min(k + u, kmax - 1)];
            t[u] = k + u < kmax ? x : 0.f;
          }
          v[i] = float4{t[0], t[1], t[2], t[3]};
        }
      } else {
        const int k = k0 + e / (R / 4), r = r0 + 4 * (e % (R / 4));
        if constexpr (AL) {
          const float4 t = *reinterpret_cast<const float4 *>(X + (long)min(k, kmax - 1) * ld + min(r, rmax - 4));
          v[i] = (k < kmax && r < rmax) ? t : float4{0.f, 0.f, 0.f, 0.f};
        } else {
          const float *row = X + (long)min(k, kmax - 1) * ld;
          float t[4];
#pragma unroll
          for (int u = 0; u < 4; ++u) {
            const float x = row[min(r + u, rmax - 1)];
            t[u] = (k < kmax && r + u < rmax) ? x : 0.f;
          }
          v[i] = float4{t[0], t[1], t[2], t[3]};
        }
      }
    }
  }
  template <int LD>
  __device__ inline void store(float *S, bool kcontig, int tid) const {
#pragma unroll
    for (int i = 0; i < PER; ++i) {
      const int e = tid + i * 256;
      if (NV4 % 256 == 0 || e < NV4) {
        if (kcontig) {
          const int r = e >> 2, kq = e & 3;
          S[(4 * kq + 0) * LD + r] = v[i].x;
          S[(4 * kq + 1) * LD + r] = v[i].y;
          S[(4 * kq + 2) * LD + r] = v[i].z;
          S[(4 * kq + 3) * LD + r] = v[i].w;
        } else {
          const int k = e / (R / 4), rq = e % (R / 4);
          *reinterpret_cast<float4 *>(S + k * LD + 4 * rq) = v[i];
        }
      }
    }
  }
};

template <int TM, int TN, int LDA, int LDB>
__device__ inline void mfma_block(const float *As, const float *Bs, int wm, int wn, int lane, f32x4 (&acc)[TM][TN]) {
#pragma unroll
  for (int kk = 0; kk < BK; kk += 4) {
    float a[TM], bv[TN];
    const int kr = kk + (lane >> 4), c = lane & 15;
#pragma unroll
    for (int i = 0; i < TM; ++i) a[i] = As[kr * LDA + wm + i * 16 + c];
#pragma unroll
    for (int j = 0; j < TN; ++j) bv[j] = Bs[kr * LDB + wn + j * 16 + c];
#pragma unroll
    for (int i = 0; i < TM; ++i)
#pragma unroll
      for (int j = 0; j < TN; ++j) acc[i][j] = __builtin_amdgcn_mfma_f32_16x16x4f32(a[i], bv[j], acc[i][j], 0, 0, 0);
  }
}

typedef __bf16 bf8v __attribute__((ext_vector_type(8)));
__device__ inline uint16_t bf_of(float x) { return __builtin_bit_cast(uint16_t, (__bf16)x); }
__device__ inline float f_of(uint16_t h) { return __builtin_bit_cast(float, (uint32_t)h << 16); }
__device__ inline void split3(float x, uint16_t &h, uint16_t &m, uint16_t &l) {
#pragma clang fp contract(off)
  h = bf_of(x);
  const float r1 = x - f_of(h);
  m = bf_of(r1);
  l = bf_of(r1 - f_of(m));
}
constexpr int X6K = 32;
__device__ inline int x6_off(int row, int chunk) { return row * 64 + 16 * (chunk ^ ((row & 8) ? 3 : 0)); }
template <int PL>
__device__ inline void x6_put4(char *planes, int row, int kq, float4 v) {
  const float x[4] = {v.x, v.y, v.z, v.w};
  uint16_t h[4], m[4], l[4];
#pragma unroll
  for (int u = 0; u < 4; ++u) split3(x[u], h[u], m[u], l[u]);
  char *dst = planes + x6_off(row, kq >> 1) + 8 * (kq & 1);
  *reinterpret_cast<uint2 *>(dst) = uint2{(uint32_t)h[0] | ((uint32_t)h[1] << 16), (uint32_t)h[2] | ((uint32_t)h[3] << 16)};
  *reinterpret_cast<uint2 *>(dst + PL) = uint2{(uint32_t)m[0] | ((uint32_t)m[1] << 16), (uint32_t)m[2] | ((uint32_t)m[3] << 16)};
  *reinterpret_cast<uint2 *>(dst + 2 * PL) = uint2{(uint32_t)l[0] | ((uint32_t)l[1] << 16), (uint32_t)l[2] | ((uint32_t)l[3] << 16)};
}
template <int TM, int TN, int PLA, int PLB>
__device__ inline void x6_block(const char *Ap, const char *Bp, int wm, int wn, int lane, f32x4 (&acc)[TM][TN]) {
  const int r16 = lane & 15, g = lane >> 4;
  bf8v ah[TM], am[TM], al[TM], bh[TN], bm[TN], bl[TN];
#pragma unroll
  for (int i = 0; i < TM; ++i) {
    const char *p = Ap + x6_off(wm + 16 * i + r16, g);
    ah[i] = *reinterpret_cast<const bf8v *>(p);
    am[i] = *reinterpret_cast<const bf8v *>(p + PLA);
    al[i] = *reinterpret_cast<const bf8v *>(p + 2 * PLA);
  }
#pragma unroll
  for (int j = 0; j < TN; ++j) {
    const char *p = Bp + x6_off(wn + 16 * j + r16, g);
    bh[j] = *reinterpret_cast<const bf8v *>(p);
    bm[j] = *reinterpret_cast<const bf8v *>(p + PLB);
    bl[j] = *reinterpret_cast<const bf8v *>(p + 2 * PLB);
  }
#pragma unroll
  for (int i = 0; i < TM; ++i)
#pragma unroll
    for (int j = 0; j < TN; ++j) {
      f32x4 c = acc[i][j];
      c = __builtin_amdgcn_mfma_f32_16x16x32_bf16(al[i], bh[j], c, 0, 0, 0);
      c = __builtin_amdgcn_mfma_f32_16x16x32_bf16(ah[i], bl[j], c, 0, 0, 0);
      c = __builtin_amdgcn_mfma_f32_16x16x32_bf16(am[i], bm[j], c, 0, 0, 0);
      c = __builtin_amdgcn_mfma_f32_16x16x32_bf16(am[i], bh[j], c, 0, 0, 0);
      c = __builtin_amdgcn_mfma_f32_16x16x32_bf16(ah[i], bm[j], c, 0, 0, 0);
      c = __builtin_amdgcn_mfma_f32_16x16x32_bf16(ah[i], bh[j], c, 0, 0, 0);
      acc[i][j] = c;
    }
}
template <int R>
struct X6StagerK {
  static constexpr int PER = R * 8 / 256;
  float4 v[PER];
  __device__ inline void load(const float *__restrict__ X, long ld, int r0, int k0, int rmax, int kmax, int tid) {
#pragma unroll
    for (int i = 0; i < PER; ++i) {
      const int e = tid + i * 256, r = e >> 3, k = k0 + 4 * (e & 7);
      const float4 t = *reinterpret_cast<const float4 *>(X + (long)min(r0 + r, rmax - 1) * ld + min(k, kmax - 4));
      v[i] = k < kmax ? t : float4{0.f, 0.f, 0.f, 0.f};
    }
  }
  template <int PL>
  __device__ inline void store(char *planes, int tid) const {
#pragma unroll
    for (int i = 0; i < PER; ++i) {
      const int e = tid + i * 256;
      x6_put4<PL>(planes, e >> 3, e & 7, v[i]);
    }
  }
};
struct X6StagerR {
  float4 v[4];
  __device__ inline void load(const float *__restrict__ X, long ld, int r0, int k0, int rmax, int kmax, int tid) {
    const int rq = tid & 31, kq = tid >> 5, r = r0 + 4 * rq;
#pragma unroll
    for (int u = 0; u < 4; ++u) {
      const int k = k0 + 4 * kq + u;
      const float4 t = *reinterpret_cast<const float4 *>(X + (long)min(k, kmax - 1) * ld + min(r, rmax - 4));
      v[u] = (k < kmax && r < rmax) ? t : float4{0.f, 0.f, 0.f, 0.f};
    }
  }
  template <int PL>
  __device__ inline void store(char *planes, int tid) const {
    const int rq = tid & 31, kq = tid >> 5;
    x6_put4<PL>(planes, 4 * rq + 0, kq, float4{v[0].x, v[1].x, v[2].x, v[3].x});
    x6_put4<PL>(planes, 4 * rq + 1, kq, float4{v[0].y, v[1].y, v[2].y, v[3].y});
    x6_put4<PL>(planes, 4 * rq + 2, kq, float4{v[0].z, v[1].z, v[2].z, v[3].z});
    x6_put4<PL>(planes, 4 * rq + 3, kq, float4{v[0].w, v[1].w, v[2].w, v[3].w});
  }
};

template <int CTRL>
__device__ inline float dpp_f(float x) {
  return __builtin_bit_cast(float, __builtin_amdgcn_update_dpp(0, __builtin_bit_cast(int, x), CTRL, 0xf, 0xf, false));
}
__device__ inline float row16_max(float x) {
  x = fmaxf(x, dpp_f<0x128>(x));
  x = fmaxf(x, dpp_f<0x124>(x));
  x = fmaxf(x, dpp_f<0x122>(x));
  return fmaxf(x, dpp_f<0x121>(x));
}
__device__ inline float row16_sum(float x) {
  x += dpp_f<0x128>(x);
  x += dpp_f<0x124>(x);
  x += dpp_f<0x122>(x);
  return x + dpp_f<0x121>(x);
}

constexpr int AT = 128, ATLD = AT + 4;

template <bool X6, int TS = 128>
__global__ __launch_bounds__(256) void affinity_tile_kernel(const float *__restrict__ ehat, int T, int N, int C, float tau,
                                                            float *__restrict__ A, float *__restrict__ part, int tiles,
                                                            float *__restrict__ direct) {
  constexpr int LD = TS + 16, TW = TS / 32, HW = TS / 2, TSLD = TS + 4;
  static_assert(!X6 || TS == 128, "the bf16 form is built for 128-tiles");
  extern __shared__ __attribute__((aligned(16))) float lds_f[];
  float *As = lds_f, *Bs = lds_f + BK * LD, *tile = lds_f;
  const int tm = blockIdx.x / tiles, tn = blockIdx.x % tiles, m0 = tm * TS, n0 = tn * TS;
  const long amat = blockIdx.y;
  const long b = amat / (T - 1), t = amat % (T - 1);
  const float *E0 = ehat + (b * T + t) * (long)N * C, *E1 = E0 + (long)N * C;
  const int tid = threadIdx.x, lane = tid & 63, wave = tid >> 6;
  const int wm = (wave >> 1) * HW, wn = (wave & 1) * HW;
  f32x4 acc[TW][TW];
#pragma unroll
  for (int i = 0; i < TW; ++i)
#pragma unroll
    for (int j = 0; j < TW; ++j) acc[i][j] = f32x4{0.f, 0.f, 0.f, 0.f};
  if constexpr (X6) {
    constexpr int PL = AT * 64;
    char *Ap = reinterpret_cast<char *>(lds_f), *Bp = Ap + 3 * PL;
    X6StagerK<AT> sa0, sb0, sa1, sb1;
    const int nk = C / X6K;
    sa0.load(E0, C, m0, 0, N, C, tid);
    sb0.load(E1, C, n0, 0, N, C, tid);
    sa1.load(E0, C, m0, min(1, nk - 1) * X6K, N, C, tid);
    sb1.load(E1, C, n0, min(1, nk - 1) * X6K, N, C, tid);
    for (int kt = 0; kt < nk; kt += 2) {
      sa0.store<PL>(Ap, tid);
      sb0.store<PL>(Bp, tid);
      __syncthreads();
      sa0.load(E0, C, m0, min(kt + 2, nk - 1) * X6K, N, C, tid);
      sb0.load(E1, C, n0, min(kt + 2, nk - 1) * X6K, N, C, tid);
      x6_block<TW, TW, PL, PL>(Ap, Bp, wm, wn, lane, acc);
      __syncthreads();
      if (kt + 1 < nk) {
        sa1.store<PL>(Ap, tid);
        sb1.store<PL>(Bp, tid);
        __syncthreads();
        sa1.load(E0, C, m0, min(kt + 3, nk - 1) * X6K, N, C, tid);
        sb1.load(E1, C, n0, min(kt + 3, nk - 1) * X6K, N, C, tid);
        x6_block<TW, TW, PL, PL>(Ap, Bp, wm, wn, lane, acc);
        __syncthreads();
      }
    }
  } else {
  BoundStager<TS> sa, sb;
  const int nk = (C + BK - 1) / BK;
  sa.load(E0, C, m0, 0, true, N, C, tid);
  sb.load(E1, C, n0, 0, true, N, C, tid);
  for (int kt = 0; kt < nk; ++kt) {
    sa.template store<LD>(As, true, tid);
    sb.template store<LD>(Bs, true, tid);
    __syncthreads();
    if (kt + 1 < nk) {
      sa.load(E0, C, m0, (kt + 1) * BK, true, N, C, tid);
      sb.load(E1, C, n0, (kt + 1) * BK, true, N, C, tid);
    }
    mfma_block<TW, TW, LD, LD>(As, Bs, wm, wn, lane, acc);
    __syncthreads();
  }
  }
  float v[TW][TW][4];
#pragma unroll
  for (int i = 0; i < TW; ++i)
#pragma unroll
    for (int j = 0; j < TW; ++j)
#pragma unroll
      for (int r = 0; r < 4; ++r) v[i][j][r] = acc[i][j][r] / tau;
  const int g = lane >> 4, r16 = lane & 15;
#pragma unroll
  for (int i = 0; i < TW; ++i)
#pragma unroll
    for (int j = 0; j < TW; ++j)
#pragma unroll
      for (int r = 0; r < 4; ++r) tile[(wm + 16 * i + 4 * g + r) * TSLD + wn + 16 * j + r16] = v[i][j][r];
  float *rpart = tile + TS * TSLD, *cpart = rpart + 2 * TS * 2;
  if (part || direct) {
    bool cok[TW], rok[TW][4];
#pragma unroll
    for (int j = 0; j < TW; ++j) cok[j] = n0 + wn + 16 * j + r16 < N;
#pragma unroll
    for (int i = 0; i < TW; ++i)
#pragma unroll
      for (int r = 0; r < 4; ++r) rok[i][r] = m0 + wm + 16 * i + 4 * g + r < N;
#pragma unroll
    for (int i = 0; i < TW; ++i)
#pragma unroll
      for (int r = 0; r < 4; ++r) {
        float m = -INFINITY;
#pragma unroll
        for (int j = 0; j < TW; ++j) m = cok[j] ? fmaxf(m, v[i][j][r]) : m;
        m = row16_max(m);
        float sum = 0.f;
#pragma unroll
        for (int j = 0; j < TW; ++j) sum += cok[j] ? expf(v[i][j][r] - m) : 0.f;
        sum = row16_sum(sum);
        if (r16 == 0) {
          float *dst = rpart + ((wave & 1) * TS + wm + 16 * i + 4 * g + r) * 2;
          dst[0] = m;
          dst[1] = sum;
        }
      }
#pragma unroll
    for (int j = 0; j < TW; ++j) {
      float m = -INFINITY;
#pragma unroll
      for (int i = 0; i < TW; ++i)
#pragma unroll
        for (int r = 0; r < 4; ++r) m = rok[i][r] ? fmaxf(m, v[i][j][r]) : m;
      m = fmaxf(m, __shfl_xor(m, 16));
      m = fmaxf(m, __shfl_xor(m, 32));
      float sum = 0.f;
#pragma unroll
      for (int i = 0; i < TW; ++i)
#pragma unroll
        for (int r = 0; r < 4; ++r) sum += rok[i][r] ? expf(v[i][j][r] - m) : 0.f;
      sum += __shfl_xor(sum, 16);
      sum += __shfl_xor(sum, 32);
      if (g == 0) {
        float *dst = cpart + ((wave >> 1) * TS + wn + 16 * j + r16) * 2;
        dst[0] = m;
        dst[1] = sum;
      }
    }
  }
  __syncthreads();
  float *Ab = A + amat * (long)N * N;
  if ((N & 3) == 0) {
    for (int e = tid; e < TS * TS / 4; e += 256) {
      const int r = e / (TS / 4), c = 4 * (e % (TS / 4));
      if (m0 + r < N && n0 + c < N)
        *reinterpret_cast<float4 *>(Ab + (long)(m0 + r) * N + n0 + c) = *reinterpret_cast<const float4 *>(tile + r * TSLD + c);
    }
  } else {
    for (int e = tid; e < TS * TS; e += 256) {
      const int r = e / TS, c = e % TS;
      if (m0 + r < N && n0 + c < N) Ab[(long)(m0 + r) * N + n0 + c] = tile[r * TSLD + c];
    }
  }
  if (!part && !direct) return;
  if (tid >= 2 * TS) return;
  const int idx = tid % TS;
  const bool rows = tid < TS;
  const float *pp = (rows ? rpart : cpart) + idx * 2;
  const float ma = pp[0], sa = pp[1], mb = pp[TS * 2], sb = pp[TS * 2 + 1];
  const float m = fmaxf(ma, mb);
  const float sum = (sa > 0.f ? sa * expf(ma - m) : 0.f) + (sb > 0.f ? sb * expf(mb - m) : 0.f);
  const int gi = (rows ? m0 : n0) + idx;
  if (gi < N) {
    const long nmat = gridDim.y;
    if (direct) {
      direct[((rows ? 0 : 2) * nmat + amat) * N + gi] = m;
      direct[((rows ? 1 : 3) * nmat + amat) * N + gi] = sum;
    } else {
      float *dst = part + ((((rows ? 0 : nmat) + amat) * tiles + (rows ? tn : tm)) * (long)N + gi) * 2;
      dst[0] = m;
      dst[1] = sum;
    }
  }
}

__global__ __launch_bounds__(256) void affinity_stats_merge_kernel(const float *__restrict__ part, int nmat, int tiles, int N,
                                                                   float *__restrict__ stats) {
  const long i = (long)blockIdx.x * 256 + threadIdx.x;
  if (i >= 2L * nmat * N) return;
  const long which = i / ((long)nmat * N), rem = i % ((long)nmat * N), mat = rem / N, n = rem % N;
  const float *p = part + ((which * nmat + mat) * tiles * (long)N + n) * 2;
  float m = -INFINITY;
  for (int t = 0; t < tiles; ++t) m = fmaxf(m, p[(long)t * N * 2]);
  float s = 0.f;
  for (int t = 0; t < tiles; ++t) s += p[(long)t * N * 2 + 1] * expf(p[(long)t * N * 2] - m);
  stats[((2 * which) * nmat + mat) * N + n] = m;
  stats[((2 * which + 1) * nmat + mat) * N + n] = s;
}

template <int TN, int RM = 128, bool AL = true>
__global__ __launch_bounds__(256) void affinity_bwd_tile_kernel(const float *__restrict__ dA, const float *__restrict__ ehat,
                                                                int T, int N, float tau, float *__restrict__ dehat) {
  constexpr int C = 32 * TN, LDA = RM + 16, LDB = C + 16, TM = RM / 32;
  __shared__ __attribute__((aligned(16))) float lds_f[BK * LDA + BK * LDB];
  float *As = lds_f, *Bs = lds_f + BK * LDA;
  const int m0 = blockIdx.x * RM;
  const long bt = blockIdx.y, b = bt / T, t = bt % T;
  const int tid = threadIdx.x, lane = tid & 63, wave = tid >> 6;
  const int wm = (wave >> 1) * (RM / 2), wn = (wave & 1) * (C / 2);
  f32x4 acc[TM][TN];
#pragma unroll
  for (int i = 0; i < TM; ++i)
#pragma unroll
    for (int j = 0; j < TN; ++j) acc[i][j] = f32x4{0.f, 0.f, 0.f, 0.f};
  BoundStager<RM> sa;
  BoundStager<C> sb;
  const long NN = (long)N * N, NC = (long)N * C;
  const int nk = (N + BK - 1) / BK;
  for (int prod = 0; prod < 2; ++prod) {
    if (prod == 0 ? t == T - 1 : t == 0) continue;
    const float *X = dA + (b * (T - 1) + (prod == 0 ? t : t - 1)) * NN;
    const float *E = ehat + (b * T + (prod == 0 ? t + 1 : t - 1)) * NC;
    const bool akc = prod == 0;
    sa.template load<AL>(X, N, m0, 0, akc, N, N, tid);
    sb.load(E, C, 0, 0, false, C, N, tid);
    for (int kt = 0; kt < nk; ++kt) {
      sa.template store<LDA>(As, akc, tid);
      sb.template store<LDB>(Bs, false, tid);
      __syncthreads();
      if (kt + 1 < nk) {
        sa.template load<AL>(X, N, m0, (kt + 1) * BK, akc, N, N, tid);
        sb.load(E, C, 0, (kt + 1) * BK, false, C, N, tid);
      }
      mfma_block<TM, TN, LDA, LDB>(As, Bs, wm, wn, lane, acc);
      __syncthreads();
    }
  }
  float *D = dehat + bt * NC;
#pragma unroll
  for (int i = 0; i < TM; ++i)
#pragma unroll
    for (int j = 0; j < TN; ++j)
#pragma unroll
      for (int r = 0; r < 4; ++r) {
        const int row = m0 + wm + 16 * i + 4 * (lane >> 4) + r;
        if (row < N) D[(long)row * C + wn + 16 * j + (lane & 15)] = acc[i][j][r] / tau;
      }
}

__global__ __launch_bounds__(256) void affinity_bwd_x6_kernel(const float *__restrict__ dA, const float *__restrict__ ehat,
                                                              int T, int N, float tau, float *__restrict__ dehat) {
  constexpr int C = 128, PL = AT * 64;
  __shared__ __attribute__((aligned(16))) char lds_c[6 * PL];
  char *Ap = lds_c, *Bp = lds_c + 3 * PL;
  const int m0 = blockIdx.x * AT;
  const long bt = blockIdx.y, b = bt / T, t = bt % T;
  const int tid = threadIdx.x, lane = tid & 63, wave = tid >> 6;
  const int wm = (wave >> 1) * 64, wn = (wave & 1) * 64;
  f32x4 acc[4][4];
#pragma unroll
  for (int i = 0; i < 4; ++i)
#pragma unroll
    for (int j = 0; j < 4; ++j) acc[i][j] = f32x4{0.f, 0.f, 0.f, 0.f};
  X6StagerK<AT> sak;
  X6StagerR sar, sb;
  const long NN = (long)N * N, NC = (long)N * C;
  const int nk = (N + X6K - 1) / X6K;
  for (int prod = 0; prod < 2; ++prod) {
    if (prod == 0 ? t == T - 1 : t == 0) continue;
    const float *X = dA + (b * (T - 1) + (prod == 0 ? t : t - 1)) * NN;
    const float *E = ehat + (b * T + (prod == 0 ? t + 1 : t - 1)) * NC;
    if (prod == 0) sak.load(X, N, m0, 0, N, N, tid);
    else sar.load(X, N, m0, 0, N, N, tid);
    sb.load(E, C, 0, 0, C, N, tid);
    for (int kt = 0; kt < nk; ++kt) {
      if (prod == 0) sak.store<PL>(Ap, tid);
      else sar.store<PL>(Ap, tid);
      sb.store<PL>(Bp, tid);
      __syncthreads();
      if (kt + 1 < nk) {
        if (prod == 0) sak.load(X, N, m0, (kt + 1) * X6K, N, N, tid);
        else sar.load(X, N, m0, (kt + 1) * X6K, N, N, tid);
        sb.load(E, C, 0, (kt + 1) * X6K, C, N, tid);
      }
      x6_block<4, 4, PL, PL>(Ap, Bp, wm, wn, lane, acc);
      __syncthreads();
    }
  }
  float *D = dehat + bt * NC;
#pragma unroll
  for (int i = 0; i < 4; ++i)
#pragma unroll
    for (int j = 0; j < 4; ++j)
#pragma unroll
      for (int r = 0; r < 4; ++r) {
        const int row = m0 + wm + 16 * i + 4 * (lane >> 4) + r;
        if (row < N) D[(long)row * C + wn + 16 * j + (lane & 15)] = acc[i][j][r] / tau;
      }
}

int pick_tile(int n, long batch_times_prob) {
  const int cand[3] = {128, 64, 32};
  for (int i = 0; i < 3; ++i) {
    int t = cand[i];
    if (n % t) continue;
    long blocks = (long)(n / t) * (n / t) * batch_times_prob;
    if (blocks >= 512 || t == 32) return t;
  }
  return 32;
}

}

int launch_gemm_group_f32(const GemmGroup &g, hipStream_t s) {
  if (g.nprob < 1 || g.nprob > MAX_GROUP || g.n <= 0 || g.n % 32 || g.batch < 1) return CRW_EINVAL;
  const int tile = pick_tile(g.n, (long)g.batch * g.nprob);
  dim3 grid((g.n / tile) * (g.n / tile), g.batch, g.nprob);
  if (tile == 128)
    hipLaunchKernelGGL((gemm_pad_f32_kernel<128, 128>), grid, dim3(256), 0, s, g);
  else if (tile == 64)
    hipLaunchKernelGGL((gemm_pad_f32_kernel<64, 64>), grid, dim3(256), 0, s, g);
  else
    hipLaunchKernelGGL((gemm_pad_f32_kernel<32, 32>), grid, dim3(256), 0, s, g);
  return check_launch();
}

int launch_edge_gemm(const EdgeGemm &g, int batch, hipStream_t s) {
  if (g.M < 1 || g.N < 1 || batch < 1) return CRW_EINVAL;
  dim3 grid((g.N + EB - 1) / EB, (g.M + EB - 1) / EB, batch);
  hipLaunchKernelGGL(edge_gemm_kernel, grid, dim3(256), 0, s, g);
  return check_launch();
}

bool affinity_on_bf16(int N, int C) {
  const char *e = getenv("CRW_AFFINITY_F32");
  const bool force_f32 = e && e[0] && e[0] != '0';
  return !force_f32 && N >= 256 && C % 32 == 0;
}

size_t affinity_part_floats(int B, int T, int N) {
  const size_t tiles = (N + AT - 1) / AT;
  return (size_t)2 * B * (T - 1) * tiles * N * 2;
}

int launch_affinity_tiles(const float *ehat, int B, int T, int N, int C, float tau, float *A, float *stats, float *part,
                          hipStream_t s) {
  if (C % 4 || C < 4 || (stats && !part)) return CRW_EINVAL;
  const int tiles = (N + AT - 1) / AT, nmat = B * (T - 1);
  const size_t lds = sizeof(float) * (size_t)(AT * ATLD + 2 * 2 * AT * 2);
  static bool attr = false;
  if (!attr) {
    if (hipFuncSetAttribute((const void *)affinity_tile_kernel<false>, hipFuncAttributeMaxDynamicSharedMemorySize, (int)lds) != hipSuccess ||
        hipFuncSetAttribute((const void *)affinity_tile_kernel<true>, hipFuncAttributeMaxDynamicSharedMemorySize, (int)lds) != hipSuccess) {
      g_last_hip_error = (int)hipGetLastError();
      return CRW_EHIP;
    }
    attr = true;
  }
  const bool single = tiles == 1;
  if (N <= 64) {
    const size_t lds64 = sizeof(float) * (size_t)(64 * 68 + 2 * 2 * 64 * 2);
    hipLaunchKernelGGL((affinity_tile_kernel<false, 64>), dim3(1, nmat), dim3(256), lds64, s, ehat, T, N, C, tau, A, nullptr, 1,
                       stats);
    return check_launch();
  }
  if (affinity_on_bf16(N, C))
    hipLaunchKernelGGL(affinity_tile_kernel<true>, dim3(tiles * tiles, nmat), dim3(256), lds, s, ehat, T, N, C, tau, A,
                       (stats && !single) ? part : nullptr, tiles, (stats && single) ? stats : nullptr);
  else
    hipLaunchKernelGGL(affinity_tile_kernel<false>, dim3(tiles * tiles, nmat), dim3(256), lds, s, ehat, T, N, C, tau, A,
                       (stats && !single) ? part : nullptr, tiles, (stats && single) ? stats : nullptr);
  if (stats && !single) {
    const long n = 2L * nmat * N;
    hipLaunchKernelGGL(affinity_stats_merge_kernel, dim3((unsigned)((n + 255) / 256)), dim3(256), 0, s, part, nmat, tiles, N, stats);
  }
  return check_launch();
}

int launch_affinity_bwd_tiles(const float *dA, const float *ehat, int B, int T, int N, int C, float tau, float *dehat,
                              hipStream_t s) {
  if (N < 1) return CRW_EINVAL;
  const dim3 grid((N + AT - 1) / AT, B * T);
  if (N <= 64 || (N & 3)) {
#define CRW_AFB(TNV)                                                                                                            \
  if (N <= 64 && !(N & 3)) hipLaunchKernelGGL((affinity_bwd_tile_kernel<TNV, 64, true>), dim3(1, B * T), dim3(256), 0, s, dA, ehat, T, N, tau, dehat); \
  else if (N <= 64) hipLaunchKernelGGL((affinity_bwd_tile_kernel<TNV, 64, false>), dim3(1, B * T), dim3(256), 0, s, dA, ehat, T, N, tau, dehat);       \
  else hipLaunchKernelGGL((affinity_bwd_tile_kernel<TNV, 128, false>), grid, dim3(256), 0, s, dA, ehat, T, N, tau, dehat);
    switch (C) {
      case 32: CRW_AFB(1) break;
      case 64: CRW_AFB(2) break;
      case 128: CRW_AFB(4) break;
      default: return CRW_EINVAL;
    }
#undef CRW_AFB
    return check_launch();
  }
  if (C == 128 && affinity_on_bf16(N, C)) {
    hipLaunchKernelGGL(affinity_bwd_x6_kernel, grid, dim3(256), 0, s, dA, ehat, T, N, tau, dehat);
    return check_launch();
  }
  switch (C) {
    case 32: hipLaunchKernelGGL(affinity_bwd_tile_kernel<1>, grid, dim3(256), 0, s, dA, ehat, T, N, tau, dehat); break;
    case 64: hipLaunchKernelGGL(affinity_bwd_tile_kernel<2>, grid, dim3(256), 0, s, dA, ehat, T, N, tau, dehat); break;
    case 128: hipLaunchKernelGGL(affinity_bwd_tile_kernel<4>, grid, dim3(256), 0, s, dA, ehat, T, N, tau, dehat); break;
    default: return CRW_EINVAL;
  }
  return check_launch();
}

__global__ __launch_bounds__(256) void batch_sum_kernel(const float *__restrict__ part, int nb, int n, float *__restrict__ out) {
  const int e = blockIdx.x * 256 + threadIdx.x;
  if (e >= n) return;
  float s = 0.f;
  int b = 0;
  for (; b + 8 <= nb; b += 8) {
    float v[8];
#pragma unroll
    for (int u = 0; u < 8; ++u) v[u] = part[(long)(b + u) * n + e];
#pragma unroll
    for (int u = 0; u < 8; ++u) s += v[u];
  }
  for (; b < nb; ++b) s += part[(long)b * n + e];
  out[e] = s;
}

}

extern "C" size_t crw_linear128_wgrad_ws_bytes(int P) { return P < 128 ? 0 : (size_t)(P / 128) * 128 * 128 * sizeof(float); }

extern "C" int crw_linear128_wgrad(const float *dy, const float *x, float *dw, int P, void *ws, size_t ws_bytes,
                                   crw_stream_t stream) {
  crw::clear_stale_error();
  if (!dy || !x || !dw || !ws || P < 128 || P % 128) return CRW_EINVAL;
  if (ws_bytes < crw_linear128_wgrad_ws_bytes(P)) return CRW_EWORKSPACE;
  hipStream_t s = (hipStream_t)stream;
  crw::GemmGroup g{};
  g.nprob = 1;
  g.n = 128;
  g.batch = P / 128;
  crw::GemmProb &p = g.p[0];
  p.A = dy; p.B = x; p.C = static_cast<float *>(ws);
  p.sA = p.sB = p.sC = 128L * 128;
  p.ta = 1; p.tb = 0; p.beta = 0;
  CRW_TRY(crw::launch_gemm_group_f32(g, s));
  hipLaunchKernelGGL(crw::batch_sum_kernel, dim3(128 * 128 / 256), dim3(256), 0, s, static_cast<const float *>(ws), P / 128,
                     128 * 128, dw);
  return crw::check_launch();
}

extern "C" int crw_gemm_f32(const float *A, const float *B, float *C, int n, int batch, int transA, int transB,
                            int beta, crw_stream_t stream) {
  crw::clear_stale_error();
  if (!A || !B || !C) return CRW_EINVAL;
  crw::GemmGroup g{};
  g.nprob = 1;
  g.n = n;
  g.batch = batch;
  crw::GemmProb &p = g.p[0];
  p.A = A; p.B = B; p.C = C;
  p.sA = p.sB = p.sC = (long)n * n;
  p.ta = transA; p.tb = transB; p.beta = beta;
  return crw::launch_gemm_group_f32(g, (hipStream_t)stream);
}
```

radar-sounder-crw_amd/csrc/walk.hip:

```cpp
#include "crw_common.h"

namespace crw {
namespace {

constexpr float EPS_NORM = 1e-12f;

__global__ __launch_bounds__(256) void zero3_kernel(float *__restrict__ a, float *__restrict__ b, float *__restrict__ c, long n4) {
  for (long e = (long)blockIdx.x * 256 + threadIdx.x; e < n4; e += (long)gridDim.x * 256) {
    reinterpret_cast<float4 *>(a)[e] = float4{0.f, 0.f, 0.f, 0.f};
    reinterpret_cast<float4 *>(b)[e] = float4{0.f, 0.f, 0.f, 0.f};
    reinterpret_cast<float4 *>(c)[e] = float4{0.f, 0.f, 0.f, 0.f};
  }
}

__global__ __launch_bounds__(256) void normalize_kernel(const float *__restrict__ e, long rows, int C,
                                                        float *__restrict__ ehat, float *__restrict__ norm) {
  const int lane = threadIdx.x & 63;
  const long row = (long)blockIdx.x * 4 + (threadIdx.x >> 6);
  if (row >= rows) return;
  const float *x = e + row * C;
  float ss = 0.f;
  for (int c = lane; c < C; c += 64) ss += x[c] * x[c];
  ss = wave_sum(ss);
  const float d = fmaxf(sqrtf(ss), EPS_NORM);
  for (int c = lane; c < C; c += 64) ehat[row * C + c] = x[c] / d;
  if (lane == 0 && norm) norm[row] = d;
}

__global__ __launch_bounds__(256) void normalize_bwd_kernel(const float *__restrict__ dehat,
                                                            const float *__restrict__ ehat,
                                                            const float *__restrict__ norm, long rows, int C,
                                                            float *__restrict__ de) {
  const int lane = threadIdx.x & 63;
  const long row = (long)blockIdx.x * 4 + (threadIdx.x >> 6);
  if (row >= rows) return;
  float dot = 0.f;
  for (int c = lane; c < C; c += 64) dot += ehat[row * C + c] * dehat[row * C + c];
  dot = wave_sum(dot);
  const float d = norm[row];
  for (int c = lane; c < C; c += 64) de[row * C + c] = (dehat[row * C + c] - ehat[row * C + c] * dot) / d;
}

struct Mat {
  float *f = nullptr;
  uint16_t *h = nullptr, *l = nullptr;
};
struct WalkState {
  Mat F, Gt, Lt, R, At;
  float *lse, *terms, *stats;
  size_t bytes;
};
struct WalkScratch {
  Mat dAt, dF, dGt, dLt, dR;
  float *stats;
  size_t bytes;
};

template <typename T>
T *carve(char *&p, size_t count) {
  T *r = reinterpret_cast<T *>(p);
  p += align_up(count * sizeof(T), 256);
  return r;
}

Mat carve_mat(char *&p, size_t count, int chain, bool want_f32_in_bf16_mode, bool want_img_in_bf16_mode = true) {
  Mat m;
  if (chain == CRW_CHAIN_F32 || want_f32_in_bf16_mode) m.f = carve<float>(p, count);
  if (chain != CRW_CHAIN_F32 && want_img_in_bf16_mode) {
    m.h = carve<uint16_t>(p, count);
    if (chain == CRW_CHAIN_BF16X3) m.l = carve<uint16_t>(p, count);
  }
  return m;
}

int chain_padded_nodes(int N, int chain) { return chain == CRW_CHAIN_F32 ? padded_nodes(N) : round_up(N, 128); }

WalkState layout_state(void *base, int B, int T, int N, int chain) {
  const size_t Np = chain_padded_nodes(N, chain), K = T - 2, nA = (size_t)B * (T - 1), M = Np * Np;
  char *p = static_cast<char *>(base);
  WalkState s;
  s.F = carve_mat(p, nA * M, chain, false);
  s.Gt = carve_mat(p, nA * M, chain, false);
  s.Lt = carve_mat(p, K * B * M, chain, false);
  s.R = carve_mat(p, K * B * M, chain, false);
  s.At = carve_mat(p, K * B * M, chain, true, false);
  s.lse = carve<float>(p, K * B * Np);
  s.terms = carve<float>(p, K * B * Np);
  s.stats = carve<float>(p, 4 * nA * Np);
  s.bytes = p - static_cast<char *>(base);
  return s;
}

WalkScratch layout_scratch(void *base, int B, int T, int N, int chain) {
  const size_t Np = chain_padded_nodes(N, chain), K = T - 2, nA = (size_t)B * (T - 1), M = Np * Np;
  char *p = static_cast<char *>(base);
  WalkScratch s;
  s.dAt = carve_mat(p, K * B * M, chain, false);
  s.dF = carve_mat(p, nA * M, chain, true, false);
  s.dGt = carve_mat(p, nA * M, chain, true, false);
  s.dLt = carve_mat(p, K * B * M, chain, true);
  s.dR = carve_mat(p, K * B * M, chain, true);
  s.stats = carve<float>(p, 2 * nA * Np);
  s.bytes = p - static_cast<char *>(base);
  return s;
}

bool bad_shape(int B, int T, int N) { return B < 1 || T < 2 || N < 1 || N > 16384 || (long)B * T > 65535; }
bool bad_chain(int chain) { return chain != CRW_CHAIN_F32 && chain != CRW_CHAIN_BF16 && chain != CRW_CHAIN_BF16X3; }

struct Opnd {
  const Mat *m;
  long off;
  long stride;
};
void set_a(GemmProb &p, int chain, Opnd o, int t) {
  if (chain == CRW_CHAIN_F32) p.A = o.m->f + o.off;
  else { p.A = o.m->h + o.off; p.Al = o.m->l ? o.m->l + o.off : nullptr; }
  p.sA = o.stride; p.ta = t;
}
void set_b(GemmProb &p, int chain, Opnd o, int t) {
  if (chain == CRW_CHAIN_F32) p.B = o.m->f + o.off;
  else { p.B = o.m->h + o.off; p.Bl = o.m->l ? o.m->l + o.off : nullptr; }
  p.sB = o.stride; p.tb = t;
}
void set_a2(GemmProb &p, int chain, Opnd o, int t) {
  if (chain == CRW_CHAIN_F32) p.A2 = o.m->f + o.off;
  else { p.A2 = o.m->h + o.off; p.A2l = o.m->l ? o.m->l + o.off : nullptr; }
  p.sA2 = o.stride; p.ta2 = t;
}
void set_b2(GemmProb &p, int chain, Opnd o, int t) {
  if (chain == CRW_CHAIN_F32) p.B2 = o.m->f + o.off;
  else { p.B2 = o.m->h + o.off; p.B2l = o.m->l ? o.m->l + o.off : nullptr; }
  p.sB2 = o.stride; p.tb2 = t;
}
void set_c(GemmProb &p, Opnd o) {
  p.C = o.m->f ? o.m->f + o.off : nullptr;
  p.Cb = o.m->h ? o.m->h + o.off : nullptr;
  p.Cbl = o.m->l ? o.m->l + o.off : nullptr;
  p.sC = o.stride;
}
int launch_group_once(const GemmGroup &g, int chain, hipStream_t s) {
  if (chain == CRW_CHAIN_F32) return launch_gemm_group_f32(g, s);
  return launch_gemm_group_bf16(g, chain == CRW_CHAIN_BF16X3 ? 3 : 1, s);
}
int launch_group(const GemmGroup &g, int chain, hipStream_t s) {
  constexpr int MAXB = 32768;
  if (g.batch <= MAXB) return launch_group_once(g, chain, s);
  const size_t es = chain == CRW_CHAIN_F32 ? 4 : 2;
  for (int b0 = 0; b0 < g.batch; b0 += MAXB) {
    GemmGroup sub = g;
    sub.batch = g.batch - b0 < MAXB ? g.batch - b0 : MAXB;
    for (int i = 0; i < g.nprob; ++i) {
      GemmProb &q = sub.p[i];
      auto adv = [&](const void *&ptr, long stride) { if (ptr) ptr = (const char *)ptr + (size_t)b0 * stride * es; };
      adv(q.A, q.sA); adv(q.Al, q.sA); adv(q.B, q.sB); adv(q.Bl, q.sB);
      adv(q.A2, q.sA2); adv(q.A2l, q.sA2); adv(q.B2, q.sB2); adv(q.B2l, q.sB2);
      if (q.C) q.C += (long)b0 * q.sC;
      if (q.Cb) q.Cb = (uint16_t *)q.Cb + (long)b0 * q.sC;
      if (q.Cbl) q.Cbl = (uint16_t *)q.Cbl + (long)b0 * q.sC;
    }
    CRW_TRY(launch_group_once(sub, chain, s));
  }
  return CRW_OK;
}

}
}

using namespace crw;

extern "C" {

int crw_abi_version(void) { return CRW_ABI_VERSION; }
const char *crw_build_arch(void) { return "gfx950"; }
int crw_last_hip_error(void) { return g_last_hip_error; }
int crw_padded_nodes(int N, int chain) { return (N < 1 || bad_chain(chain)) ? 0 : chain_padded_nodes(N, chain); }

size_t crw_walk_state_bytes(int B, int T, int N, int chain) {
  if (bad_shape(B, T, N) || bad_chain(chain) || T < 3) return 256;
  return layout_state(nullptr, B, T, N, chain).bytes;
}
size_t crw_walk_scratch_bytes(int B, int T, int N, int chain) {
  if (bad_shape(B, T, N) || bad_chain(chain) || T < 3) return 256;
  return layout_scratch(nullptr, B, T, N, chain).bytes;
}

int crw_normalize(const float *emb, int rows, int C, float *ehat, float *norm, crw_stream_t stream) {
  crw::clear_stale_error();
  if (!emb || !ehat || rows < 1 || C < 1) return CRW_EINVAL;
  hipLaunchKernelGGL(normalize_kernel, dim3((rows + 3) / 4), dim3(256), 0, (hipStream_t)stream, emb, (long)rows, C,
                     ehat, norm);
  return check_launch();
}

size_t crw_affinity_ws_bytes(int B, int T, int N) {
  if (bad_shape(B, T, N)) return 0;
  return affinity_part_floats(B, T, N) * sizeof(float);
}

int crw_affinity_fwd(const float *emb, int B, int T, int N, int C, float tau, float *ehat, float *norm, float *A,
                     float *stats, void *ws, size_t ws_bytes, crw_stream_t stream) {
  crw::clear_stale_error();
  if (!emb || !ehat || !norm || !A || bad_shape(B, T, N) || C < 1 || !(tau > 0.f)) return CRW_EINVAL;
  if (stats && (!ws || ws_bytes < crw_affinity_ws_bytes(B, T, N))) return CRW_EWORKSPACE;
  hipStream_t s = (hipStream_t)stream;
  CRW_TRY(crw_normalize(emb, B * T * N, C, ehat, norm, stream));
  if (C % 4 == 0)
    return launch_affinity_tiles(ehat, B, T, N, C, tau, A, stats, static_cast<float *>(ws), s);
  EdgeGemm g{};
  const long NC = (long)N * C, NN = (long)N * N;
  g.A = EdgeOperand{ehat, NC, C, 1};
  g.B = EdgeOperand{ehat + NC, NC, 1, C};
  g.C = A;
  g.sCb = NN; g.ldc = N;
  g.M = N; g.N = N; g.K = C;
  g.batch_inner = T - 1;
  g.sA_outer = g.sB_outer = (long)T * NC;
  g.sC_outer = (long)(T - 1) * NN;
  g.skip1_inner = g.skip2_inner = -1;
  g.scale = tau; g.divide = 1;
  CRW_TRY(launch_edge_gemm(g, B * (T - 1), s));
  if (stats) CRW_TRY(launch_stats_dense(A, B * (T - 1), N, stats, s));
  return CRW_OK;
}

int crw_walk_fwd(const float *A, const float *stats_ext, int B, int T, int N, int chain, void *state, size_t state_bytes,
                 float *At_out, float *loss, crw_stream_t stream) {
  crw::clear_stale_error();
  if (!A || !loss || bad_shape(B, T, N) || bad_chain(chain)) return CRW_EINVAL;
  hipStream_t s = (hipStream_t)stream;
  if (T < 3) {
    if (hipMemsetAsync(loss, 0, sizeof(float), s) != hipSuccess) return CRW_EHIP;
    return CRW_OK;
  }
  if (!state) return CRW_EINVAL;
  WalkState st = layout_state(state, B, T, N, chain);
  if (state_bytes < st.bytes) return CRW_EWORKSPACE;
  const int Np = chain_padded_nodes(N, chain), K = T - 2, nA = B * (T - 1);
  const long M = (long)Np * Np, BM = (long)B * M;
  const bool small = chain == CRW_CHAIN_F32 && Np <= 64;

  (void)nA;
  CRW_TRY(launch_softmax_fwd(A, stats_ext, B, T - 1, N, Np, st.F.f, st.Gt.f, st.F.h, st.F.l, st.Gt.h, st.Gt.l, st.stats, s));
  if (chain == CRW_CHAIN_F32) {
    CRW_TRY(launch_identity(st.R.f, nullptr, B, Np, N, s, st.Lt.f, st.Gt.f));
  } else {
    CRW_TRY(launch_copy_f32((float *)st.Lt.h, (const float *)st.Gt.h, 0, 0, BM / 2, 1, s));
    if (st.Lt.l) CRW_TRY(launch_copy_f32((float *)st.Lt.l, (const float *)st.Gt.l, 0, 0, BM / 2, 1, s));
    CRW_TRY(launch_identity(nullptr, st.R.h, B, Np, N, s));
    if (st.R.l && hipMemsetAsync(st.R.l, 0, sizeof(uint16_t) * BM, s) != hipSuccess) return CRW_EHIP;
  }

  if (small) {
    CRW_TRY(launch_chain_small_fwd(st.Gt.f, st.F.f, st.Lt.f, st.R.f, B, K, Np, s));
  } else {
    for (int i = 1; i < K; ++i) {
      GemmGroup g{};
      g.n = Np; g.batch = B;
      GemmProb &p1 = g.p[g.nprob++];
      set_a(p1, chain, {&st.Gt, i * BM, M}, 0);
      set_b(p1, chain, {&st.Lt, (i - 1) * BM, M}, 0);
      set_c(p1, {&st.Lt, i * BM, M});
      GemmProb &p2 = g.p[g.nprob++];
      set_a(p2, chain, {&st.F, i * BM, M}, 0);
      set_b(p2, chain, {&st.R, (i - 1) * BM, M}, 0);
      set_c(p2, {&st.R, i * BM, M});
      CRW_TRY(launch_group(g, chain, s));
    }
  }
  {
    GemmGroup g{};
    g.n = Np; g.batch = K * B;
    GemmProb &p0 = g.p[g.nprob++];
    set_a(p0, chain, {&st.Lt, 0, M}, 1);
    set_b(p0, chain, {&st.R, 0, M}, 0);
    set_c(p0, {&st.At, 0, M});
    CRW_TRY(launch_group(g, chain, s));
  }
  CRW_TRY(launch_loss_rows(st.At.f, K * B, N, Np, st.lse, st.terms, s));
  CRW_TRY(launch_loss_reduce(st.terms, (long)K * B * Np, 1.0f / ((float)B * (float)N * (float)N), loss, s));
  if (At_out) CRW_TRY(launch_unpad_At(st.At.f, K, B, N, Np, At_out, s));
  return CRW_OK;
}

int crw_walk_bwd(const float *gloss, const float *A, int B, int T, int N, int chain, void *state, size_t state_bytes,
                 void *scratch, size_t scratch_bytes, float *dA, crw_stream_t stream) {
  crw::clear_stale_error();
  if (!gloss || !A || !dA || bad_shape(B, T, N) || bad_chain(chain)) return CRW_EINVAL;
  hipStream_t s = (hipStream_t)stream;
  const long NN = (long)N * N;
  if (T < 3) {
    if (hipMemsetAsync(dA, 0, sizeof(float) * B * (T - 1) * NN, s) != hipSuccess) return CRW_EHIP;
    return CRW_OK;
  }
  if (!state || !scratch) return CRW_EINVAL;
  WalkState st = layout_state(state, B, T, N, chain);
  WalkScratch sc = layout_scratch(scratch, B, T, N, chain);
  if (state_bytes < st.bytes || scratch_bytes < sc.bytes) return CRW_EWORKSPACE;
  const int Np = chain_padded_nodes(N, chain), K = T - 2;
  const long M = (long)Np * Np, BM = (long)B * M;
  const bool small = chain == CRW_CHAIN_F32 && Np <= 64;

  const float coef = 1.0f / ((float)N * (float)B * (float)N);
  CRW_TRY(launch_dAt(st.At.f, st.lse, gloss, coef, K * B, N, Np, sc.dAt.f, sc.dAt.h, sc.dAt.l, s));
  if ((reinterpret_cast<uintptr_t>(sc.dF.f) | reinterpret_cast<uintptr_t>(sc.dGt.f)) & 15) {
    if (hipMemsetAsync(sc.dF.f, 0, sizeof(float) * BM, s) != hipSuccess) return CRW_EHIP;
    if (hipMemsetAsync(sc.dF.f + (long)(T - 2) * BM, 0, sizeof(float) * BM, s) != hipSuccess) return CRW_EHIP;
    if (hipMemsetAsync(sc.dGt.f + (long)(T - 2) * BM, 0, sizeof(float) * BM, s) != hipSuccess) return CRW_EHIP;
  } else {
    const long n4 = BM / 4;
    const long blocks = (n4 + 255) / 256;
    hipLaunchKernelGGL(zero3_kernel, dim3((unsigned)(blocks > 2048 ? 2048 : blocks)), dim3(256), 0, s, sc.dF.f,
                       sc.dF.f + (long)(T - 2) * BM, sc.dGt.f + (long)(T - 2) * BM, n4);
    CRW_TRY(check_launch());
  }

  {
    GemmGroup g{};
    g.n = Np; g.batch = K * B;
    GemmProb &p0 = g.p[g.nprob++];
    set_a(p0, chain, {&st.R, 0, M}, 0);
    set_b(p0, chain, {&sc.dAt, 0, M}, 1);
    set_c(p0, {&sc.dLt, 0, M});
    GemmProb &p1 = g.p[g.nprob++];
    set_a(p1, chain, {&st.Lt, 0, M}, 0);
    set_b(p1, chain, {&sc.dAt, 0, M}, 0);
    set_c(p1, {&sc.dR, 0, M});
    CRW_TRY(launch_group(g, chain, s));
  }
  if (small) {
    CRW_TRY(launch_chain_small_bwd(st.Gt.f, st.F.f, sc.dLt.f, sc.dR.f, B, K, Np, s));
  } else {
    for (int i = K - 2; i >= 0; --i) {
      GemmGroup g{};
      g.n = Np; g.batch = B;
      GemmProb &p0 = g.p[g.nprob++];
      set_a(p0, chain, {&st.Gt, (i + 1) * BM, M}, 1);
      set_b(p0, chain, {&sc.dLt, (i + 1) * BM, M}, 0);
      set_c(p0, {&sc.dLt, i * BM, M});
      p0.beta = 1;
      GemmProb &p1 = g.p[g.nprob++];
      set_a(p1, chain, {&st.F, (i + 1) * BM, M}, 1);
      set_b(p1, chain, {&sc.dR, (i + 1) * BM, M}, 0);
      set_c(p1, {&sc.dR, i * BM, M});
      p1.beta = 1;
      CRW_TRY(launch_group(g, chain, s));
    }
  }
  if (K > 1) {
    GemmGroup g{};
    g.n = Np; g.batch = (K - 1) * B;
    GemmProb &p2 = g.p[g.nprob++];
    set_a(p2, chain, {&sc.dLt, BM, M}, 0);
    set_b(p2, chain, {&st.Lt, 0, M}, 1);
    set_c(p2, {&sc.dGt, BM, M});
    GemmProb &p3 = g.p[g.nprob++];
    set_a(p3, chain, {&sc.dR, BM, M}, 0);
    set_b(p3, chain, {&st.R, 0, M}, 1);
    set_c(p3, {&sc.dF, BM, M});
    CRW_TRY(launch_group(g, chain, s));
  }
  CRW_TRY(launch_copy_f32(sc.dGt.f, sc.dLt.f, 0, 0, BM, 1, s));
  CRW_TRY(launch_softmax_bwd(A, st.stats, sc.dF.f, sc.dGt.f, B, T - 1, N, Np, sc.stats, dA, s));
  return CRW_OK;
}

int crw_affinity_bwd(const float *dA, const float *ehat, const float *norm, int B, int T, int N, int C, float tau,
                     float *dehat_ws, float *demb, crw_stream_t stream) {
  crw::clear_stale_error();
  if (!dA || !ehat || !norm || !dehat_ws || !demb || bad_shape(B, T, N) || C < 1 || !(tau > 0.f)) return CRW_EINVAL;
  hipStream_t s = (hipStream_t)stream;
  const long NC = (long)N * C, NN = (long)N * N;
  if (C == 32 || C == 64 || C == 128) {
    CRW_TRY(launch_affinity_bwd_tiles(dA, ehat, B, T, N, C, tau, dehat_ws, s));
    const long rows_ = (long)B * T * N;
    hipLaunchKernelGGL(normalize_bwd_kernel, dim3((unsigned)((rows_ + 3) / 4)), dim3(256), 0, s, dehat_ws, ehat, norm, rows_, C, demb);
    return check_launch();
  }
  EdgeGemm g{};
  g.A = EdgeOperand{dA, NN, N, 1};
  g.B = EdgeOperand{ehat + NC, NC, C, 1};
  g.sA_outer = (long)(T - 1) * NN; g.sB_outer = (long)T * NC;
  g.K = N; g.skip1_inner = T - 1;
  g.A2 = EdgeOperand{dA - NN, NN, 1, N};
  g.B2 = EdgeOperand{ehat - NC, NC, C, 1};
  g.sA2_outer = (long)(T - 1) * NN; g.sB2_outer = (long)T * NC;
  g.K2 = N; g.skip2_inner = 0;
  g.C = dehat_ws; g.sCb = NC; g.ldc = C; g.sC_outer = (long)T * NC;
  g.M = N; g.N = C;
  g.batch_inner = T;
  g.scale = tau; g.divide = 1;
  CRW_TRY(launch_edge_gemm(g, B * T, s));
  const long rows = (long)B * T * N;
  hipLaunchKernelGGL(normalize_bwd_kernel, dim3((unsigned)((rows + 3) / 4)), dim3(256), 0, s, dehat_ws, ehat, norm,
                     rows, C, demb);
  return check_launch();
}

}
```

radar-sounder-crw_amd/encoder.py:

```python
import warnings

import torch
import torch.nn as nn
import torch.nn.functional as TF

FEATURE_DIM = 128


class _HipEncoder(torch.autograd.Function):

    @staticmethod
    def forward(ctx, x, w1, b1, w2, b2, w3, b3, w4, b4, w5, b5, split, bwd_split=None):
        import crw_hip
        x = x.contiguous()
        w2p = crw_hip.enc_front_pack(w2, split)
        packed = [crw_hip.enc_pack_weights(w, split) for w in (w3, w4, w5)]
        ctx.bwd_split = bwd_split or split
        x3h, x3l, fsaved = crw_hip.enc_front_fwd(split, x, w1, b1, w2p[:2], b2, save=True)
        y3h, y3l, _, _ = crw_hip.enc_conv3x3(0, split, x3h, x3l, packed[0][0], packed[0][1], 64, bias=b3)
        y4h, y4l, _, _ = crw_hip.enc_conv3x3(0, split, y3h, y3l, packed[1][0], packed[1][1], 128, bias=b4)
        y5h, _, _, gap = crw_hip.enc_conv3x3(0, split, y4h, y4l, packed[2][0], packed[2][1], 128, bias=b5, gap=True,
                                             lo_plane=False)
        ctx.split = split
        ctx.save_for_backward(x, w1.detach(), b1.detach(), b2.detach(), *w2p, x3h, x3l, y3h, y3l, y4h, y4l, y5h,
                              *[t for pk in packed for t in (pk[2], pk[3])], fsaved)
        return gap

    @staticmethod
    def backward(ctx, dgap):
        import crw_hip
        s = ctx.bwd_split
        if ctx.needs_input_grad[0]:
            raise RuntimeError("the fused HIP encoder does not produce a gradient for its input patches (the reference never "
                               "asks for one); set CNN.hip_convs = None to differentiate with respect to the input")
        sv = ctx.saved_tensors
        x, w1, b1, b2 = sv[:4]
        w2p = sv[4:8]
        x3h, x3l, y3h, y3l, y4h, y4l, y5h = sv[8:15]
        bwd_w = [(sv[15], sv[16]), (sv[17], sv[18]), (sv[19], sv[20])]
        fsaved = sv[21]
        if s == 1:
            x3l = y3l = y4l = None
            bwd_w = [(h, None) for h, _ in bwd_w]
            w2p = (w2p[0], None, w2p[2], None)
        dgap = dgap.contiguous().float()
        dw5, db5 = crw_hip.enc_wgrad(s, y5h, None, y4h, y4l, dgap=dgap)
        d4h, d4l, _, _ = crw_hip.enc_conv3x3(1, s, y5h, None, *bwd_w[2], 128, mask=y4h, dgap=dgap)
        dw4, db4 = crw_hip.enc_wgrad(s, d4h, d4l, y3h, y3l)
        d3h, d3l, _, _ = crw_hip.enc_conv3x3(1, s, d4h, d4l, *bwd_w[1], 64, mask=y3h)
        dw3, db3 = crw_hip.enc_wgrad(s, d3h, d3l, x3h, x3l)
        _, _, dx3, _ = crw_hip.enc_conv3x3(1, s, d3h, d3l, *bwd_w[0], 32, planes=False, f32=True)
        dw1, db1, dw2, db2 = crw_hip.enc_front_bwd(s, x, w1, b1, w2p[:2], b2, w2p[2:], dx3, saved=fsaved)
        return None, dw1, db1, dw2, db2, dw3, db3, dw4, db4, dw5, db5, None, None

class _HipMapEncoder(torch.autograd.Function):

    @staticmethod
    def forward(ctx, x, w1, b1, w2, b2, w3, b3, w4, b4, w5, b5, split):
        import crw_hip
        x = x.contiguous()
        P, _, h, w = x.shape
        H, W = h - 6, w - 6
        w2p = crw_hip.enc_front_pack(w2, split)
        packed = [crw_hip.enc_pack_weights(wt, split) for wt in (w3, w4, w5)]
        x3h, x3l = crw_hip.enc_front_fwd_map(split, x, w1, b1, w2p[:2], b2)
        y3h, y3l, _ = crw_hip.enc_conv3x3_map(split, x3h, x3l, packed[0][0], packed[0][1], 64, H, W, bias=b3)
        y4h, y4l, _ = crw_hip.enc_conv3x3_map(split, y3h, y3l, packed[1][0], packed[1][1], 128, H, W, bias=b4)
        y5h, _, gap = crw_hip.enc_conv3x3_map(split, y4h, y4l, packed[2][0], packed[2][1], 128, H, W, bias=b5, gap=True,
                                              lo_plane=False)
        ctx.split, ctx.hw = split, (H, W)
        ctx.save_for_backward(x, w1.detach(), b1.detach(), b2.detach(), *w2p, x3h, x3l, y3h, y3l, y4h, y4l, y5h,
                              *[t for pk in packed for t in (pk[2], pk[3])])
        return gap

    @staticmethod
    def backward(ctx, dgap):
        import crw_hip
        if ctx.needs_input_grad[0]:
            raise RuntimeError("the fused HIP encoder does not produce a gradient for its input patches (the reference never "
                               "asks for one); set CNN.hip_convs = None to differentiate with respect to the input")
        s, (H, W) = ctx.split, ctx.hw
        sv = ctx.saved_tensors
        x, w1, b1, b2 = sv[:4]
        w2p = sv[4:8]
        x3h, x3l, y3h, y3l, y4h, y4l, y5h = sv[8:15]
        bw = [(sv[15], sv[16]), (sv[17], sv[18]), (sv[19], sv[20])]
        d5h, d5l = crw_hip.enc_gap_bwd(dgap.contiguous().float(), y5h, s)
        dw5, db5 = crw_hip.enc_wgrad_map(s, d5h, d5l, y4h, y4l, H, W)
        d4h, d4l, _ = crw_hip.enc_conv3x3_map(s, d5h, d5l, *bw[2], 128, H, W, mode=1, mask=y4h)
        dw4, db4 = crw_hip.enc_wgrad_map(s, d4h, d4l, y3h, y3l, H, W)
        d3h, d3l, _ = crw_hip.enc_conv3x3_map(s, d4h, d4l, *bw[1], 64, H, W, mode=1, mask=y3h)
        dw3, db3 = crw_hip.enc_wgrad_map(s, d3h, d3l, x3h, x3l, H, W)
        _, _, dx3 = crw_hip.enc_conv3x3_map(s, d3h, d3l, *bw[0], 32, H, W, mode=1, planes=False, f32=True)
        dw1, db1, dw2, db2 = crw_hip.enc_front_bwd_map(s, x, w1, b1, w2p[:2], b2, w2p[2:], dx3)
        return None, dw1, db1, dw2, db2, dw3, db3, dw4, db4, dw5, db5, None


class _HipLinear(torch.autograd.Function):

    @staticmethod
    def forward(ctx, x, w, b):
        ctx.save_for_backward(x, w)
        return TF.linear(x, w, b)

    @staticmethod
    def backward(ctx, dy):
        import crw_hip
        x, w = ctx.saved_tensors
        dy = dy.contiguous()
        return dy @ w, crw_hip.linear128_wgrad(dy, x), dy.sum(0)


_CNN_STACK = (("1", 8, 5, True), ("2", 32, 5, True), ("3", 64, 3, False), ("4", 128, 3, False), ("5", 128, 3, False))


def _report(module):
    n = sum(p.numel() for p in module.parameters() if p.requires_grad)
    print(f"Number of trainable parameters: {n}")
    return n


class CNN(nn.Module):
    _warned_fallback = False

    def __init__(self, pos_embed):
        super().__init__()
        cin = 2 if pos_embed else 1
        for name, cout, k, pooled in _CNN_STACK:
            setattr(self, "conv" + name, nn.Conv2d(cin, cout, kernel_size=k, padding=1))
            setattr(self, "relu" + name, nn.ReLU())
            if pooled:
                setattr(self, "pool" + name, nn.MaxPool2d(kernel_size=2, stride=1))
            cin = cout
        self.global_avg_pool = nn.AdaptiveAvgPool2d(1)
        self.fc = nn.Linear(cin, FEATURE_DIM)
        self.num_params = _report(self)
        self.hip_convs = "bf16x3"

    def forward(self, x):
        if self.hip_convs and x.is_cuda and x.shape[-2:] == (16, 16) and x.dtype == torch.float32:
            c = [getattr(self, "conv%d" % i) for i in range(1, 6)]
            gap = _HipEncoder.apply(x, c[0].weight, c[0].bias, c[1].weight, c[1].bias, c[2].weight, c[2].bias,
                                    c[3].weight, c[3].bias, c[4].weight, c[4].bias,
                                    3 if self.hip_convs in ("bf16x3", "mixed") else 1, 1 if self.hip_convs == "mixed" else None)
            return self._head(gap)
        if self.hip_convs and x.is_cuda and x.dtype == torch.float32 and min(x.shape[-2:]) >= 7:
            if not torch.is_grad_enabled():
                return self._head(self._hip_inference_trunk(x))
            c = [getattr(self, "conv%d" % i) for i in range(1, 6)]
            gap = _HipMapEncoder.apply(x, c[0].weight, c[0].bias, c[1].weight, c[1].bias, c[2].weight, c[2].bias,
                                       c[3].weight, c[3].bias, c[4].weight, c[4].bias,
                                       3 if self.hip_convs in ("bf16x3", "mixed") else 1)
            return self._head(gap)
        if self.hip_convs and x.is_cuda and not CNN._warned_fallback:
            CNN._warned_fallback = True
            warnings.warn(f"CNN.forward: input {tuple(x.shape)} {x.dtype} (grad enabled: {torch.is_grad_enabled()}) is not covered by "
                          "the HIP conv kernels (float32 patches of at least 7x7 on an MI355X): this call "
                          "runs on PyTorch-ROCm / MIOpen convolutions", RuntimeWarning, stacklevel=2)
        for name, _, _, pooled in _CNN_STACK:
            x = getattr(self, "relu" + name)(getattr(self, "conv" + name)(x))
            if pooled:
                x = getattr(self, "pool" + name)(x)
        return self.fc(self.global_avg_pool(x).flatten(1))

    def _head(self, gap):
        if gap.shape[0] % 128 == 0 and gap.shape[0] >= 128 and self.fc.weight.shape == (128, 128) and self.fc.bias is not None:
            return _HipLinear.apply(gap, self.fc.weight, self.fc.bias)
        return self.fc(gap)

    def _hip_inference_trunk(self, x):
        import crw_hip
        split = 3 if self.hip_convs in ("bf16x3", "mixed") else 1
        P, _, h, w = x.shape
        H, W = h - 6, w - 6
        w2p = crw_hip.enc_front_pack(self.conv2.weight, split)
        xh, xl = crw_hip.enc_front_fwd_map(split, x, self.conv1.weight, self.conv1.bias, w2p[:2], self.conv2.bias)
        pk = [crw_hip.enc_pack_weights(getattr(self, "conv" + n).weight, split) for n in ("3", "4", "5")]
        y3h, y3l, _ = crw_hip.enc_conv3x3_map(split, xh, xl, pk[0][0], pk[0][1], 64, H, W, bias=self.conv3.bias)
        y4h, y4l, _ = crw_hip.enc_conv3x3_map(split, y3h, y3l, pk[1][0], pk[1][1], 128, H, W, bias=self.conv4.bias)
        _, _, gap = crw_hip.enc_conv3x3_map(split, y4h, y4l, pk[2][0], pk[2][1], 128, H, W, bias=self.conv5.bias,
                                            planes=False, gap=True)
        return gap


class _Residual(nn.Module):

    def __init__(self, cin, cout, stride, shortcut):
        super().__init__()
        self.conv1 = nn.Conv2d(cin, cout, 3, stride, 1, bias=False)
        self.bn1 = nn.BatchNorm2d(cout)
        self.relu = nn.ReLU(inplace=True)
        self.conv2 = nn.Conv2d(cout, cout, 3, 1, 1, bias=False)
        self.bn2 = nn.BatchNorm2d(cout)
# ... 67 lines not shown
```

Baseline: 655,200 radargram columns/s.

## Fuse encoder weight packing, linear bias grad, and small-walk kernels per step

Replaces four separate weight-packing launches (conv2 plus three 3x3 layers) with one multi-job pack kernel, and folds the linear layer's bias-gradient row sum into the weight-gradient GEMM. It also adds fused single-block walk kernels for small N (softmax, cycle, local grad, softmax bwd) and extends the affinity kernels with optional normalized-embedding outputs. The aim is to cut per-step launch count and redundant passes over small tensors. The risk is added complexity, and parts of the diff (walk kernels) may not be wired in.

```diff
diff --git a/include/crw_hip.h b/include/crw_hip.h
--- a/include/crw_hip.h
+++ b/include/crw_hip.h
@@ -87,6 +87,9 @@
 
 size_t crw_linear128_wgrad_ws_bytes(int P);
 int crw_linear128_wgrad(const float *dy, const float *x, float *dw, int P, void *ws, size_t ws_bytes, crw_stream_t stream);
+size_t crw_linear128_wgrad_bias_ws_bytes(int P);
+int crw_linear128_wgrad_bias(const float *dy, const float *x, float *dw, float *db, int P, void *ws, size_t ws_bytes,
+                             crw_stream_t stream);
 
 int crw_adam_step(float *p, const float *g, float *m, float *v, long n, float lr, float beta1, float beta2, float eps, int step,
                   crw_stream_t stream);
@@ -118,6 +121,8 @@
 
 int crw_enc_front_pack(const float *w2, uint16_t *fwd_hi, uint16_t *fwd_lo, uint16_t *bwd_hi, uint16_t *bwd_lo,
                        crw_stream_t stream);
+int crw_enc_pack_all(const float *w2, const float *const *w_host, const int *cout_host, const int *cin_host,
+                     uint16_t *const *planes_host, int split, crw_stream_t stream);
 size_t crw_enc_front_saved_bytes(int P);
 int crw_enc_front_fwd(int split, const float *x, int P, int cin, const float *w1, const float *b1,
                       const uint16_t *w2_hi, const uint16_t *w2_lo, const float *b2, uint16_t *y_hi,
diff --git a/radar-sounder-crw_amd/crw_hip.py b/radar-sounder-crw_amd/crw_hip.py
--- a/radar-sounder-crw_amd/crw_hip.py
+++ b/radar-sounder-crw_amd/crw_hip.py
@@ -56,6 +56,8 @@
                                  _c_sz, _p]),
     "crw_linear128_wgrad_ws_bytes": (_c_sz, [_c_int]),
     "crw_linear128_wgrad": (_c_int, [_p, _p, _p, _c_int, _p, _c_sz, _p]),
+    "crw_linear128_wgrad_bias_ws_bytes": (_c_sz, [_c_int]),
+    "crw_linear128_wgrad_bias": (_c_int, [_p, _p, _p, _p, _c_int, _p, _c_sz, _p]),
     "crw_adam_step": (_c_int, [_p, _p, _p, _p, ctypes.c_long, ctypes.c_float, ctypes.c_float, ctypes.c_float, ctypes.c_float,
                                _c_int, _p]),
     "crw_gemm_f32": (_c_int, [_p, _p, _p, _c_int, _c_int, _c_int, _c_int, _c_int, _p]),
@@ -69,6 +71,7 @@
     "crw_enc_wgrad_ws_bytes": (_c_sz, [_c_int, _c_int, _c_int, _c_int]),
     "crw_enc_conv3x3_wgrad": (_c_int, [_c_int, _c_int, _c_int, _c_int, _p, _p, _p, _p, _p, _p, _p, _p, _c_sz, _p]),
     "crw_enc_front_pack": (_c_int, [_p, _p, _p, _p, _p, _p]),
+    "crw_enc_pack_all": (_c_int, [_p, _p, _p, _p, _p, _c_int, _p]),
     "crw_enc_front_saved_bytes": (_c_sz, [_c_int]),
     "crw_enc_front_fwd": (_c_int, [_c_int, _p, _c_int, _c_int, _p, _p, _p, _p, _p, _p, _p, _p, _p]),
     "crw_enc_front_fwd_map": (_c_int, [_c_int, _p, _c_int, _c_int, _c_int, _c_int, _p, _p, _p, _p, _p, _p, _p, _p]),
@@ -125,19 +128,22 @@
 
 CONFIDENCE_ENTRY_POINTS = ("crw_labelprop_confidence", "crw_merge_confidence", "crw_calibration_ws_bytes", "crw_calibration")
 
+STEP_FUSION_ENTRY_POINTS = ("crw_linear128_wgrad_bias_ws_bytes", "crw_linear128_wgrad_bias", "crw_enc_pack_all")
+
 _lib = None
 _has_sweep = False
 _has_confidence = False
+_has_step_fusion = False
 
 
 def lib():
-    global _lib, _has_sweep, _has_confidence
+    global _lib, _has_sweep, _has_confidence, _has_step_fusion
     if _lib is None:
         if not os.path.exists(LIB_PATH):
             raise RuntimeError(f"{LIB_PATH} not built -- the CRW hot path has no CPU/PyTorch fallback; "
                                "run `make -C radar-sounder-crw_amd/csrc` (hipcc --offload-arch=gfx950)")
         handle = ctypes.CDLL(LIB_PATH)
-        missing = [n for n in SWEEP_ENTRY_POINTS + CONFIDENCE_ENTRY_POINTS if not hasattr(handle, n)]
+        missing = [n for n in SWEEP_ENTRY_POINTS + CONFIDENCE_ENTRY_POINTS + STEP_FUSION_ENTRY_POINTS if not hasattr(handle, n)]
         for name, (res, args) in SIGNATURES.items():
             if name in missing:
                 continue
@@ -149,6 +155,7 @@
         _lib = handle
         _has_sweep = not set(missing) & set(SWEEP_ENTRY_POINTS)
         _has_confidence = not set(missing) & set(CONFIDENCE_ENTRY_POINTS)
+        _has_step_fusion = not set(missing) & set(STEP_FUSION_ENTRY_POINTS)
     return _lib
 
 
@@ -173,6 +180,18 @@
     if not has_confidence():
         raise RuntimeError(f"{LIB_PATH} is a stale libcrw_hip.so: it reports ABI {ABI_VERSION} but lacks "
                            f"{', '.join(CONFIDENCE_ENTRY_POINTS)} (added at that ABI) -- rebuild with `make -C radar-sounder-crw_amd/csrc`")
+    return lib()
+
+
+def has_step_fusion():
+    lib()
+    return _has_step_fusion
+
+
+def _step_fusion_lib():
+    if not has_step_fusion():
+        raise RuntimeError(f"{LIB_PATH} is a stale libcrw_hip.so: it reports ABI {ABI_VERSION} but lacks "
+                           f"{', '.join(STEP_FUSION_ENTRY_POINTS)} (added at that ABI) -- rebuild with `make -C radar-sounder-crw_amd/csrc`")
     return lib()
 
 
@@ -667,6 +686,17 @@
     return dw
 
 
+def linear128_wgrad_bias(dy, x):
+    P = x.shape[0]
+    dw = torch.empty(128, 128, dtype=torch.float32, device=x.device)
+    db = torch.empty(128, dtype=torch.float32, device=x.device)
+    nbytes = _step_fusion_lib().crw_linear128_wgrad_bias_ws_bytes(P)
+    ws = torch.empty(nbytes, dtype=torch.uint8, device=x.device)
+    _check(lib().crw_linear128_wgrad_bias(_dev(dy.contiguous(), "dy"), _dev(x.contiguous(), "x"), _dev(dw, "dw"), _dev(db, "db"), P,
+                                          ctypes.c_void_p(ws.data_ptr()), nbytes, _stream()), "crw_linear128_wgrad_bias")
+    return dw, db
+
+
 def adam_step(p, g, m, v, step, lr, beta1=0.9, beta2=0.999, eps=1e-8):
     _check(lib().crw_adam_step(_dev(p, "p"), _dev(g, "g"), _dev(m, "m"), _dev(v, "v"), p.numel(), float(lr), float(beta1),
                                float(beta2), float(eps), int(step), _stream()), "crw_adam_step")
@@ -751,6 +781,28 @@
     _check(lib().crw_enc_front_pack(_dev(w2.contiguous(), "w2"), _bf(fh, "fh"), _bf(fl, "fl"), _bf(bh, "bh"),
                                     _bf(bl, "bl"), _stream()), "crw_enc_front_pack")
     return fh, fl, bh, bl
+
+
+def enc_pack_all(w2, ws, split):
+    if len(ws) != 3:
+        raise RuntimeError("enc_pack_all packs conv2 and three 3x3 layers")
+    w2 = w2.contiguous()
+    ws = [w.contiguous() for w in ws]
+    dev = w2.device
+    shapes = [((7, 32, 32), (25, 8, 32))] + [((9, w.shape[0], w.shape[1]), (9, w.shape[1], w.shape[0])) for w in ws]
+    out = []
+    for f, b in shapes:
+        fh, bh = torch.empty(f, dtype=_BF, device=dev), torch.empty(b, dtype=_BF, device=dev)
+        fl, bl = (torch.empty_like(fh), torch.empty_like(bh)) if split == 3 else (None, None)
+        out.append((fh, fl, bh, bl))
+    for t in [w2] + ws:
+        _dev(t, "w")
+    wp = (ctypes.c_void_p * 3)(*[w.data_ptr() for w in ws])
+    co = (ctypes.c_int * 3)(*[w.shape[0] for w in ws])
+    ci = (ctypes.c_int * 3)(*[w.shape[1] for w in ws])
+    planes = (ctypes.c_void_p * 16)(*[t.data_ptr() if t is not None else None for pk in out for t in pk])
+    _check(_step_fusion_lib().crw_enc_pack_all(_dev(w2, "w2"), wp, co, ci, planes, split, _stream()), "crw_enc_pack_all")
+    return out
 
 
 def enc_front_fwd(split, x, w1, b1, w2f, b2, save=False):
diff --git a/radar-sounder-crw_amd/csrc/crw_common.h b/radar-sounder-crw_amd/csrc/crw_common.h
--- a/radar-sounder-crw_amd/csrc/crw_common.h
+++ b/radar-sounder-crw_amd/csrc/crw_common.h
@@ -59,6 +59,7 @@
   long sA, sB, sA2, sB2, sC;
   int ta, tb, ta2, tb2;
   int beta;
+  float *Asum;
 };
 constexpr int MAX_GROUP = 6;
 struct GemmGroup {
@@ -91,9 +92,9 @@
 int launch_edge_gemm(const EdgeGemm &g, int batch, hipStream_t s);
 size_t affinity_part_floats(int B, int T, int N);
 int launch_affinity_tiles(const float *ehat, int B, int T, int N, int C, float tau, float *A, float *stats, float *part,
-                          hipStream_t s);
+                          hipStream_t s, float *ehat_out = nullptr, float *norm_out = nullptr);
 int launch_affinity_bwd_tiles(const float *dA, const float *ehat, int B, int T, int N, int C, float tau, float *dehat,
-                              hipStream_t s);
+                              hipStream_t s, const float *norm = nullptr, float *de = nullptr);
 
 int launch_softmax_fwd(const float *A, const float *stats_ext, int B, int Tm1, int N, int Np, float *F, float *Gt, void *Fh,
                        void *Fl, void *Gh, void *Gl, float *stats , hipStream_t s);
@@ -113,4 +114,13 @@
                float *dAt, void *dAt_hi, void *dAt_lo, hipStream_t s);
 int launch_unpad_At(const float *At, int K, int B, int N, int Np, float *out, hipStream_t s);
 
+int launch_walk_softmax_small(const float *A, const float *stats_ext, int B, int Tm1, int N, int Np, float *F, float *Gt, float *Lt1,
+                              float *R1, float *stats, unsigned *ticket, hipStream_t s);
+int launch_walk_cycle_small(const float *Lt, const float *R, int nmat, int N, int Np, float *At, float *lse, float *terms, float scale,
+                            float *loss, unsigned *ticket, hipStream_t s);
+int launch_walk_local_small(const float *At, const float *lse, const float *gloss, float coef, const float *R, const float *Lt, int nmat,
+                            int N, int Np, float *dLt, float *dR, hipStream_t s);
+int launch_walk_softmax_bwd_small(const float *A, const float *stats, const float *Lt, const float *R, const float *dLt, const float *dR,
+                                  int B, int Tm1, int N, int Np, float *dA, hipStream_t s);
+
 }
diff --git a/radar-sounder-crw_amd/csrc/enc_pack.h b/radar-sounder-crw_amd/csrc/enc_pack.h
--- /dev/null
+++ b/radar-sounder-crw_amd/csrc/enc_pack.h
@@ -0,0 +1,48 @@
+#pragma once
+#include <stdint.h>
+
+namespace crw {
+namespace encpack {
+
+constexpr int KS2 = 7;
+
+__device__ inline uint16_t f2bf(float x) { return __builtin_bit_cast(uint16_t, (__bf16)x); }
+__device__ inline float bf2f(uint16_t h) { return __builtin_bit_cast(float, (uint32_t)h << 16); }
+
+__device__ inline void pack_w2(const float *__restrict__ w, uint16_t *fh, uint16_t *fl, uint16_t *bh, uint16_t *bl, int first,
+                               int stride) {
+  for (int e = first; e < KS2 * 32 * 32; e += stride) {
+    const int k = e & 31, co = (e >> 5) & 31, s = e >> 10;
+    const int tap = 4 * s + (k >> 3), ci = k & 7;
+    const float v = tap < 25 ? w[(co * 8 + ci) * 25 + tap] : 0.f;
+    const uint16_t h = f2bf(v);
+    fh[e] = h;
+    if (fl) fl[e] = f2bf(v - bf2f(h));
+  }
+  for (int e = first; e < 25 * 8 * 32; e += stride) {
+    const int co = e & 31, ci = (e >> 5) & 7, tap = e >> 8;
+    const float v = w[(co * 8 + ci) * 25 + tap];
+    const uint16_t h = f2bf(v);
+    bh[e] = h;
+    if (bl) bl[e] = f2bf(v - bf2f(h));
+  }
+}
+
+__device__ inline long frag_index(int tap, int n, int k, int N, int K) {
+  return ((((long)tap * (K / 32) + k / 32) * (N / 16) + n / 16) * 64 + ((k % 32) / 8) * 16 + n % 16) * 8 + k % 8;
+}
+__device__ inline void pack_w3x3(const float *__restrict__ w, int CO, int CI, uint16_t *fh, uint16_t *fl, uint16_t *bh, uint16_t *bl,
+                                 long first, long stride) {
+  const long n = (long)CO * CI * 9;
+  for (long e = first; e < n; e += stride) {
+    const int tap = e % 9, ci = (e / 9) % CI, co = e / (9L * CI);
+    const float v = w[e];
+    const uint16_t h = f2bf(v), l = f2bf(v - bf2f(h));
+    const long of = frag_index(tap, co, ci, CO, CI), ob = frag_index(8 - tap, ci, co, CI, CO);
+    fh[of] = h; bh[ob] = h;
+    if (fl) { fl[of] = l; bl[ob] = l; }
+  }
+}
+
+}
+}
diff --git a/radar-sounder-crw_amd/csrc/enc_pack.hip b/radar-sounder-crw_amd/csrc/enc_pack.hip
--- /dev/null
+++ b/radar-sounder-crw_amd/csrc/enc_pack.hip
@@ -0,0 +1,57 @@
+#include "crw_common.h"
+#include "enc_pack.h"
+
+namespace crw {
+namespace {
+
+struct EncPackJob {
+  const float *w;
+  uint16_t *fh, *fl, *bh, *bl;
+  int cout, cin;
+  int first_block;
+};
+struct EncPackJobs {
+  EncPackJob job[4];
+  int total_blocks;
+};
+
+__global__ __launch_bounds__(256) void enc_pack_all_kernel(EncPackJobs jobs) {
+  int j = 0;
+  while (j + 1 < 4 && (int)blockIdx.x >= jobs.job[j + 1].first_block) ++j;
+  const EncPackJob &q = jobs.job[j];
+  const int nblk = (j + 1 < 4 ? jobs.job[j + 1].first_block : jobs.total_blocks) - q.first_block;
+  const long first = (long)((int)blockIdx.x - q.first_block) * 256 + threadIdx.x, stride = (long)nblk * 256;
+  if (j == 0) encpack::pack_w2(q.w, q.fh, q.fl, q.bh, q.bl, (int)first, (int)stride);
+  else encpack::pack_w3x3(q.w, q.cout, q.cin, q.fh, q.fl, q.bh, q.bl, first, stride);
+}
+
+}
+}
+
+using namespace crw;
+
+extern "C" int crw_enc_pack_all(const float *w2, const float *const *w, const int *cout, const int *cin, uint16_t *const *planes,
+                                int split, crw_stream_t stream) {
+  clear_stale_error();
+  if (!w2 || !w || !cout || !cin || !planes || (split != 1 && split != 3)) return CRW_EINVAL;
+  EncPackJobs jobs{};
+  int blocks = 0;
+  for (int j = 0; j < 4; ++j) {
+    EncPackJob &q = jobs.job[j];
+    uint16_t *const *p = planes + 4 * j;
+    q.w = j == 0 ? w2 : w[j - 1];
+    q.fh = p[0]; q.fl = p[1]; q.bh = p[2]; q.bl = p[3];
+    if (!q.w || !q.fh || !q.bh || (split == 3) != (q.fl != nullptr) || (split == 3) != (q.bl != nullptr)) return CRW_EINVAL;
+    long n = 7 * 32 * 32;
+    if (j > 0) {
+      q.cout = cout[j - 1]; q.cin = cin[j - 1];
+      if (q.cout < 32 || q.cout % 32 || q.cin < 32 || q.cin % 32 || q.cout > 1024 || q.cin > 1024) return CRW_EINVAL;
+      n = (long)q.cout * q.cin * 9;
+    }
+    q.first_block = blocks;
+    blocks += (int)((n + 255) / 256);
+  }
+  jobs.total_blocks = blocks;
+  hipLaunchKernelGGL(enc_pack_all_kernel, dim3(blocks), dim3(256), 0, (hipStream_t)stream, jobs);
+  return check_launch();
+}
diff --git a/radar-sounder-crw_amd/csrc/encoder_conv.hip b/radar-sounder-crw_amd/csrc/encoder_conv.hip
--- a/radar-sounder-crw_amd/csrc/encoder_conv.hip
+++ b/radar-sounder-crw_amd/csrc/encoder_conv.hip
@@ -1,4 +1,5 @@
 #include "crw_common.h"
+#include "enc_pack.h"
 #include <type_traits>
 #include <cstdlib>
 
@@ -1078,20 +1079,9 @@
   }
 }
 
-__device__ inline long frag_index(int tap, int n, int k, int N, int K) {
-  return ((((long)tap * (K / 32) + k / 32) * (N / 16) + n / 16) * 64 + ((k % 32) / 8) * 16 + n % 16) * 8 + k % 8;
-}
 __global__ __launch_bounds__(256) void pack_weights_kernel(const float *__restrict__ w, int CO, int CI,
                                                            uint16_t *fh, uint16_t *fl, uint16_t *bh, uint16_t *bl) {
-  const long n = (long)CO * CI * 9;
-  for (long e = (long)blockIdx.x * 256 + threadIdx.x; e < n; e += (long)gridDim.x * 256) {
-    const int tap = e % 9, ci = (e / 9) % CI, co = e / (9L * CI);
-    const float v = w[e];
-    const uint16_t h = f2bf(v), l = f2bf(v - bf2f(h));
-    const long of = frag_index(tap, co, ci, CO, CI), ob = frag_index(8 - tap, ci, co, CI, CO);
-    fh[of] = h; bh[ob] = h;
-    if (fl) { fl[of] = l; bl[ob] = l; }
-  }
+  encpack::pack_w3x3(w, CO, CI, fh, fl, bh, bl, (long)blockIdx.x * 256 + threadIdx.x, (long)gridDim.x * 256);
 }
 
 __global__ __launch_bounds__(256) void pack_input_kernel(const float *__restrict__ x, int P, int C, int npix, uint16_t *xh,
diff --git a/radar-sounder-crw_amd/csrc/encoder_front.hip b/radar-sounder-crw_amd/csrc/encoder_front.hip
--- a/radar-sounder-crw_amd/csrc/encoder_front.hip
+++ b/radar-sounder-crw_amd/csrc/encoder_front.hip
@@ -1,4 +1,5 @@
 #include "crw_common.h"
+#include "enc_pack.h"
 #include <type_traits>
 #include <cstdlib>
 
@@ -310,21 +311,8 @@
 
 __global__ __launch_bounds__(256) void pack_w2_kernel(const float *__restrict__ w, uint16_t *fh, uint16_t *fl,
                                                       uint16_t *bh, uint16_t *bl) {
-  for (int e = blockIdx.x * 256 + threadIdx.x; e < KS2 * 32 * 32; e += gridDim.x * 256) {
-    const int k = e & 31, co = (e >> 5) & 31, s = e >> 10;
-    const int tap = 4 * s + (k >> 3), ci = k & 7;
-    const float v = tap < 25 ? w[(co * 8 + ci) * 25 + tap] : 0.f;
-    const uint16_t h = f2bf(v);
-    fh[e] = h;
-    if (fl) fl[e] = f2bf(v - bf2f(h));
-  }
-  for (int e = blockIdx.x * 256 + threadIdx.x; e < 25 * 8 * 32; e += gridDim.x * 256) {
-    const int co = e & 31, ci = (e >> 5) & 7, tap = e >> 8;
-    const float v = w[(co * 8 + ci) * 25 + tap];
-    const uint16_t h = f2bf(v);
-    bh[e] = h;
-    if (bl) bl[e] = f2bf(v - bf2f(h));
-  }
+  static_assert(KS2 == encpack::KS2, "conv2 k-steps");
+  encpack::pack_w2(w, fh, fl, bh, bl, blockIdx.x * 256 + threadIdx.x, gridDim.x * 256);
 }
 
 struct FrontBwdArgs {
diff --git a/radar-sounder-crw_amd/csrc/gemm_f32.hip b/radar-sounder-crw_amd/csrc/gemm_f32.hip
--- a/radar-sounder-crw_amd/csrc/gemm_f32.hip
+++ b/radar-sounder-crw_amd/csrc/gemm_f32.hip
@@ -51,7 +51,7 @@
   }
 };
 
-template <int BM, int BN>
+template <int BM, int BN, bool ROWSUM = false>
 __global__ __launch_bounds__(256) void gemm_pad_f32_kernel(GemmGroup g) {
   constexpr int LDA = BM + 16, LDB = BN + 16;
   constexpr int TM = BM / 2 / 16, TN = BN / 2 / 16;
@@ -94,11 +94,16 @@
     sb.template store<LDB>(Bs, tb, tid);
   };
 
+  float rowsum = 0.f;
   issue(0);
   for (int t = 0; t < nt; ++t) {
     commit(t);
     __syncthreads();
     if (t + 1 < nt) issue(t + 1);
+    if (ROWSUM && n0 == 0 && tid < BM) {
+#pragma unroll
+      for (int kk = 0; kk < BK; ++kk) rowsum += As[kk * LDA + tid];
+    }
 #pragma unroll
     for (int kk = 0; kk < BK; kk += 4) {
       float a[TM], bv[TN];
@@ -115,6 +120,7 @@
     __syncthreads();
   }
 
+  if (ROWSUM && n0 == 0 && tid < BM) p.Asum[b * p.sC + m0 + tid] = rowsum;
   float *C = p.C + b * p.sC;
 #pragma unroll
   for (int i = 0; i < TM; ++i)
@@ -251,6 +257,13 @@
       }
     }
   }
+  __device__ inline void div_rows(const float *dn, int tid) {
+#pragma unroll
+    for (int i = 0; i < PER; ++i) {
+      const float d = dn[min(tid + i * 256, NV4 - 1) >> 2];
+      v[i] = float4{v[i].x / d, v[i].y / d, v[i].z / d, v[i].w / d};
+    }
+  }
   template <int LD>
   __device__ inline void store(float *S, bool kcontig, int tid) const {
 #pragma unroll
@@ -405,12 +418,15 @@
 
 constexpr int AT = 128, ATLD = AT + 4;
 
-template <bool X6, int TS = 128>
+template <bool X6, int TS = 128, bool NORM = false>
 __global__ __launch_bounds__(256) void affinity_tile_kernel(const float *__restrict__ ehat, int T, int N, int C, float tau,
                                                             float *__restrict__ A, float *__restrict__ part, int tiles,
-                                                            float *__restrict__ direct) {
+                                                            float *__restrict__ direct, float *__restrict__ ehat_out = nullptr,
+                                                            float *__restrict__ norm_out = nullptr) {
   constexpr int LD = TS + 16, TW = TS / 32, HW = TS / 2, TSLD = TS + 4;
   static_assert(!X6 || TS == 128, "the bf16 form is built for 128-tiles");
+  static_assert(!NORM || (!X6 && TS == 64), "the normalising form is the one-tile fp32 kernel");
+  __shared__ float dn[NORM ? 2 * TS : 1];
   extern __shared__ __attribute__((aligned(16))) float lds_f[];
   float *As = lds_f, *Bs = lds_f + BK * LD, *tile = lds_f;
   const int tm = blockIdx.x / tiles, tn = blockIdx.x % tiles, m0 = tm * TS, n0 = tn * TS;
@@ -419,6 +435,37 @@
   const float *E0 = ehat + (b * T + t) * (long)N * C, *E1 = E0 + (long)N * C;
   const int tid = threadIdx.x, lane = tid & 63, wave = tid >> 6;
   const int wm = (wave >> 1) * HW, wn = (wave & 1) * HW;
+  if constexpr (NORM) {
+    constexpr int RB = 16;
+    for (int base = wave * 32; base < wave * 32 + 32; base += RB) {
+      float x[RB][4];
+#pragma unroll
+      for (int u = 0; u < RB; ++u) {
+        const int f = (base + u) / TS, row = (base + u) % TS;
+        const float *src = (f ? E1 : E0) + (long)min(row, N - 1) * C;
+#pragma unroll
+        for (int i = 0; i < 4; ++i) x[u][i] = lane + 64 * i < C ? src[lane + 64 * i] : 0.f;
+      }
+#pragma unroll
+      for (int u = 0; u < RB; ++u) {
+        const int f = (base + u) / TS, row = (base + u) % TS;
+        float ss = 0.f;
+#pragma unroll
+        for (int i = 0; i < 4; ++i) ss += x[u][i] * x[u][i];
+        ss = wave_sum(ss);
+        const float d = row < N ? fmaxf(sqrtf(ss), 1e-12f) : 1.f;
+        if (lane == 0) dn[f * TS + row] = d;
+        if (row < N && (f == 0 || t == T - 2)) {
+          const long o = (b * T + t + f) * (long)N + row;
+#pragma unroll
+          for (int i = 0; i < 4; ++i)
+            if (lane + 64 * i < C) ehat_out[o * C + lane + 64 * i] = x[u][i] / d;
+          if (lane == 0) norm_out[o] = d;
+        }
+      }
+    }
+    __syncthreads();
+  }
   f32x4 acc[TW][TW];
 #pragma unroll
   for (int i = 0; i < TW; ++i)
@@ -457,6 +504,10 @@
   sa.load(E0, C, m0, 0, true, N, C, tid);
   sb.load(E1, C, n0, 0, true, N, C, tid);
   for (int kt = 0; kt < nk; ++kt) {
+    if constexpr (NORM) {
+      sa.div_rows(dn, tid);
+      sb.div_rows(dn + (NORM ? TS : 0), tid);
+    }
     sa.template store<LD>(As, true, tid);
     sb.template store<LD>(Bs, true, tid);
     __syncthreads();
@@ -582,11 +633,14 @@
   stats[((2 * which + 1) * nmat + mat) * N + n] = s;
 }
 
-template <int TN, int RM = 128, bool AL = true>
+template <int TN, int RM = 128, bool AL = true, bool NB = false>
 __global__ __launch_bounds__(256) void affinity_bwd_tile_kernel(const float *__restrict__ dA, const float *__restrict__ ehat,
-                                                                int T, int N, float tau, float *__restrict__ dehat) {
-  constexpr int C = 32 * TN, LDA = RM + 16, LDB = C + 16, TM = RM / 32;
-  __shared__ __attribute__((aligned(16))) float lds_f[BK * LDA + BK * LDB];
+                                                                int T, int N, float tau, float *__restrict__ dehat,
+                                                                const float *__restrict__ norm = nullptr, float *__restrict__ de = nullptr) {
+  constexpr int C = 32 * TN, LDA = RM + 16, LDB = C + 16, TM = RM / 32, LDI = C + 4;
+  static_assert(!NB || RM == 64, "the fused normalise-backward needs the whole matrix in one tile");
+  constexpr int OPERANDS = BK * LDA + BK * LDB, IMAGE = NB ? RM * LDI : 0;
+  __shared__ __attribute__((aligned(16))) float lds_f[OPERANDS > IMAGE ? OPERANDS : IMAGE];
   float *As = lds_f, *Bs = lds_f + BK * LDA;
   const int m0 = blockIdx.x * RM;
   const long bt = blockIdx.y, b = bt / T, t = bt % T;
@@ -619,6 +673,25 @@
       mfma_block<TM, TN, LDA, LDB>(As, Bs, wm, wn, lane, acc);
       __syncthreads();
     }
+  }
+  if constexpr (NB) {
+    float *img = lds_f;
+#pragma unroll
+    for (int i = 0; i < TM; ++i)
+#pragma unroll
+      for (int j = 0; j < TN; ++j)
+#pragma unroll
+        for (int r = 0; r < 4; ++r) img[(wm + 16 * i + 4 * (lane >> 4) + r) * LDI + wn + 16 * j + (lane & 15)] = acc[i][j][r] / tau;
+    __syncthreads();
+    for (int row = wave; row < N; row += 4) {
+      const float *eh = ehat + bt * NC + (long)row * C, *dh = img + row * LDI;
+      float dot = 0.f;
+      for (int c = lane; c < C; c += 64) dot += eh[c] * dh[c];
+      dot = wave_sum(dot);
+      const float d = norm[bt * N + row];
+      for (int c = lane; c < C; c += 64) de[bt * NC + (long)row * C + c] = (dh[c] - eh[c] * dot) / d;
+    }
+    return;
   }
   float *D = dehat + bt * NC;
 #pragma unroll
@@ -700,6 +773,16 @@
   if (g.nprob < 1 || g.nprob > MAX_GROUP || g.n <= 0 || g.n % 32 || g.batch < 1) return CRW_EINVAL;
   const int tile = pick_tile(g.n, (long)g.batch * g.nprob);
   dim3 grid((g.n / tile) * (g.n / tile), g.batch, g.nprob);
+  if (g.p[0].Asum) {
+    if (g.nprob != 1 || g.p[0].A2) return CRW_EINVAL;
+    if (tile == 128)
+      hipLaunchKernelGGL((gemm_pad_f32_kernel<128, 128, true>), grid, dim3(256), 0, s, g);
+    else if (tile == 64)
+      hipLaunchKernelGGL((gemm_pad_f32_kernel<64, 64, true>), grid, dim3(256), 0, s, g);
+    else
+      hipLaunchKernelGGL((gemm_pad_f32_kernel<32, 32, true>), grid, dim3(256), 0, s, g);
+    return check_launch();
+  }
   if (tile == 128)
     hipLaunchKernelGGL((gemm_pad_f32_kernel<128, 128>), grid, dim3(256), 0, s, g);
   else if (tile == 64)
@@ -728,8 +811,9 @@
 }
 
 int launch_affinity_tiles(const float *ehat, int B, int T, int N, int C, float tau, float *A, float *stats, float *part,
-                          hipStream_t s) {
+                          hipStream_t s, float *ehat_out, float *norm_out) {
   if (C % 4 || C < 4 || (stats && !part)) return CRW_EINVAL;
+  if (ehat_out && (N > 64 || C > 256 || !norm_out)) return CRW_EINVAL;
   const int tiles = (N + AT - 1) / AT, nmat = B * (T - 1);
   const size_t lds = sizeof(float) * (size_t)(AT * ATLD + 2 * 2 * AT * 2);
   static bool attr = false;
@@ -744,16 +828,20 @@
   const bool single = tiles == 1;
   if (N <= 64) {
     const size_t lds64 = sizeof(float) * (size_t)(64 * 68 + 2 * 2 * 64 * 2);
-    hipLaunchKernelGGL((affinity_tile_kernel<false, 64>), dim3(1, nmat), dim3(256), lds64, s, ehat, T, N, C, tau, A, nullptr, 1,
-                       stats);
+    if (ehat_out)
+      hipLaunchKernelGGL((affinity_tile_kernel<false, 64, true>), dim3(1, nmat), dim3(256), lds64, s, ehat, T, N, C, tau, A, nullptr, 1,
+                         stats, ehat_out, norm_out);
+    else
+      hipLaunchKernelGGL((affinity_tile_kernel<false, 64>), dim3(1, nmat), dim3(256), lds64, s, ehat, T, N, C, tau, A, nullptr, 1,
+                         stats, nullptr, nullptr);
     return check_launch();
   }
   if (affinity_on_bf16(N, C))
     hipLaunchKernelGGL(affinity_tile_kernel<true>, dim3(tiles * tiles, nmat), dim3(256), lds, s, ehat, T, N, C, tau, A,
-                       (stats && !single) ? part : nullptr, tiles, (stats && single) ? stats : nullptr);
+                       (stats && !single) ? part : nullptr, tiles, (stats && single) ? stats : nullptr, nullptr, nullptr);
   else
     hipLaunchKernelGGL(affinity_tile_kernel<false>, dim3(tiles * tiles, nmat), dim3(256), lds, s, ehat, T, N, C, tau, A,
-                       (stats && !single) ? part : nullptr, tiles, (stats && single) ? stats : nullptr);
+                       (stats && !single) ? part : nullptr, tiles, (stats && single) ? stats : nullptr, nullptr, nullptr);
   if (stats && !single) {
     const long n = 2L * nmat * N;
     hipLaunchKernelGGL(affinity_stats_merge_kernel, dim3((unsigned)((n + 255) / 256)), dim3(256), 0, s, part, nmat, tiles, N, stats);
@@ -762,14 +850,28 @@
 }
 
 int launch_affinity_bwd_tiles(const float *dA, const float *ehat, int B, int T, int N, int C, float tau, float *dehat,
-                              hipStream_t s) {
+                              hipStream_t s, const float *norm, float *de) {
   if (N < 1) return CRW_EINVAL;
   const dim3 grid((N + AT - 1) / AT, B * T);
+  if (de) {
+    if (N > 64 || !norm) return CRW_EINVAL;
+#define CRW_AFB_NB(TNV)                                                                                                                   \
+  if (!(N & 3)) hipLaunchKernelGGL((affinity_bwd_tile_kernel<TNV, 64, true, true>), dim3(1, B * T), dim3(256), 0, s, dA, ehat, T, N, tau, dehat, norm, de); \
+  else hipLaunchKernelGGL((affinity_bwd_tile_kernel<TNV, 64, false, true>), dim3(1, B * T), dim3(256), 0, s, dA, ehat, T, N, tau, dehat, norm, de);
+    switch (C) {
+      case 32: CRW_AFB_NB(1) break;
+      case 64: CRW_AFB_NB(2) break;
+      case 128: CRW_AFB_NB(4) break;
+      default: return CRW_EINVAL;
+    }
+#undef CRW_AFB_NB
+    return check_launch();
+  }
   if (N <= 64 || (N & 3)) {
 #define CRW_AFB(TNV)                                                                                                            \
-  if (N <= 64 && !(N & 3)) hipLaunchKernelGGL((affinity_bwd_tile_kernel<TNV, 64, true>), dim3(1, B * T), dim3(256), 0, s, dA, ehat, T, N, tau, dehat); \
-  else if (N <= 64) hipLaunchKernelGGL((affinity_bwd_tile_kernel<TNV, 64, false>), dim3(1, B * T), dim3(256), 0, s, dA, ehat, T, N, tau, dehat);       \
-  else hipLaunchKernelGGL((affinity_bwd_tile_kernel<TNV, 128, false>), grid, dim3(256), 0, s, dA, ehat, T, N, tau, dehat);
+  if (N <= 64 && !(N & 3)) hipLaunchKernelGGL((affinity_bwd_tile_kernel<TNV, 64, true>), dim3(1, B * T), dim3(256), 0, s, dA, ehat, T, N, tau, dehat, nullptr, nullptr); \
+  else if (N <= 64) hipLaunchKernelGGL((affinity_bwd_tile_kernel<TNV, 64, false>), dim3(1, B * T), dim3(256), 0, s, dA, ehat, T, N, tau, dehat, nullptr, nullptr);       \
+  else hipLaunchKernelGGL((affinity_bwd_tile_kernel<TNV, 128, false>), grid, dim3(256), 0, s, dA, ehat, T, N, tau, dehat, nullptr, nullptr);
     switch (C) {
       case 32: CRW_AFB(1) break;
       case 64: CRW_AFB(2) break;
@@ -784,9 +886,9 @@
     return check_launch();
   }
   switch (C) {
-    case 32: hipLaunchKernelGGL(affinity_bwd_tile_kernel<1>, grid, dim3(256), 0, s, dA, ehat, T, N, tau, dehat); break;
-    case 64: hipLaunchKernelGGL(affinity_bwd_tile_kernel<2>, grid, dim3(256), 0, s, dA, ehat, T, N, tau, dehat); break;
-    case 128: hipLaunchKernelGGL(affinity_bwd_tile_kernel<4>, grid, dim3(256), 0, s, dA, ehat, T, N, tau, dehat); break;
+    case 32: hipLaunchKernelGGL(affinity_bwd_tile_kernel<1>, grid, dim3(256), 0, s, dA, ehat, T, N, tau, dehat, nullptr, nullptr); break;
+    case 64: hipLaunchKernelGGL(affinity_bwd_tile_kernel<2>, grid, dim3(256), 0, s, dA, ehat, T, N, tau, dehat, nullptr, nullptr); break;
+    case 128: hipLaunchKernelGGL(affinity_bwd_tile_kernel<4>, grid, dim3(256), 0, s, dA, ehat, T, N, tau, dehat, nullptr, nullptr); break;
     default: return CRW_EINVAL;
   }
   return check_launch();
@@ -806,6 +908,24 @@
   }
   for (; b < nb; ++b) s += part[(long)b * n + e];
   out[e] = s;
+}
+
+__global__ __launch_bounds__(256) void batch_sum2_kernel(const float *__restrict__ part, int nb, int n1, int n2, float *__restrict__ out1,
+                                                         float *__restrict__ out2) {
+  const int e = blockIdx.x * 256 + threadIdx.x, n = n1 + n2;
+  if (e >= n) return;
+  float s = 0.f;
+  int b = 0;
+  for (; b + 8 <= nb; b += 8) {
+    float v[8];
+#pragma unroll
+    for (int u = 0; u < 8; ++u) v[u] = part[(long)(b + u) * n + e];
+#pragma unroll
+    for (int u = 0; u < 8; ++u) s += v[u];
+  }
+  for (; b < nb; ++b) s += part[(long)b * n + e];
+  if (e < n1) out1[e] = s;
+  else out2[e - n1] = s;
 }
 
 }
@@ -832,6 +952,33 @@
   return crw::check_launch();
 }
 
+extern "C" size_t crw_linear128_wgrad_bias_ws_bytes(int P) {
+  return P < 128 ? 0 : (size_t)(P / 128) * (128 * 128 + 128) * sizeof(float);
+}
+
+extern "C" int crw_linear128_wgrad_bias(const float *dy, const float *x, float *dw, float *db, int P, void *ws, size_t ws_bytes,
+                                        crw_stream_t stream) {
+  crw::clear_stale_error();
+  if (!dy || !x || !dw || !db || !ws || P < 128 || P % 128) return CRW_EINVAL;
+  if (ws_bytes < crw_linear128_wgrad_bias_ws_bytes(P)) return CRW_EWORKSPACE;
+  hipStream_t s = (hipStream_t)stream;
+  constexpr long SLAB = 128L * 128 + 128;
+  crw::GemmGroup g{};
+  g.nprob = 1;
+  g.n = 128;
+  g.batch = P / 128;
+  crw::GemmProb &p = g.p[0];
+  p.A = dy; p.B = x; p.C = static_cast<float *>(ws);
+  p.Asum = static_cast<float *>(ws) + 128 * 128;
+  p.sA = p.sB = 128L * 128;
+  p.sC = SLAB;
+  p.ta = 1; p.tb = 0; p.beta = 0;
+  CRW_TRY(crw::launch_gemm_group_f32(g, s));
+  hipLaunchKernelGGL(crw::batch_sum2_kernel, dim3((unsigned)((SLAB + 255) / 256)), dim3(256), 0, s, static_cast<const float *>(ws), P / 128,
+                     128 * 128, 128, dw, db);
+  return crw::check_launch();
+}
+
 extern "C" int crw_gemm_f32(const float *A, const float *B, float *C, int n, int batch, int transA, int transB,
                             int beta, crw_stream_t stream) {
   crw::clear_stale_error();
diff --git a/radar-sounder-crw_amd/csrc/walk.hip b/radar-sounder-crw_amd/csrc/walk.hip
--- a/radar-sounder-crw_amd/csrc/walk.hip
+++ b/radar-sounder-crw_amd/csrc/walk.hip
@@ -1,3 +1,4 @@
+#include <stdlib.h>
 #include "crw_common.h"
 
 namespace crw {
@@ -48,6 +49,7 @@
 struct WalkState {
   Mat F, Gt, Lt, R, At;
   float *lse, *terms, *stats;
+  unsigned *ticket;
   size_t bytes;
 };
 struct WalkScratch {
@@ -87,6 +89,7 @@
   s.lse = carve<float>(p, K * B * Np);
   s.terms = carve<float>(p, K * B * Np);
   s.stats = carve<float>(p, 4 * nA * Np);
+  s.ticket = carve<unsigned>(p, 1);
   s.bytes = p - static_cast<char *>(base);
   return s;
 }
@@ -107,6 +110,11 @@
 
 bool bad_shape(int B, int T, int N) { return B < 1 || T < 2 || N < 1 || N > 16384 || (long)B * T > 65535; }
 bool bad_chain(int chain) { return chain != CRW_CHAIN_F32 && chain != CRW_CHAIN_BF16 && chain != CRW_CHAIN_BF16X3; }
+
+bool walk_fused() {
+  const char *e = getenv("CRW_WALK_FUSED");
+  return !(e && e[0] == '0');
+}
 
 struct Opnd {
   const Mat *m;
@@ -204,6 +212,8 @@
   if (!emb || !ehat || !norm || !A || bad_shape(B, T, N) || C < 1 || !(tau > 0.f)) return CRW_EINVAL;
   if (stats && (!ws || ws_bytes < crw_affinity_ws_bytes(B, T, N))) return CRW_EWORKSPACE;
   hipStream_t s = (hipStream_t)stream;
+  if (C % 4 == 0 && C <= 256 && N <= 64 && T > 1 && walk_fused())
+    return launch_affinity_tiles(emb, B, T, N, C, tau, A, stats, static_cast<float *>(ws), s, ehat, norm);
   CRW_TRY(crw_normalize(emb, B * T * N, C, ehat, norm, stream));
   if (C % 4 == 0)
     return launch_affinity_tiles(ehat, B, T, N, C, tau, A, stats, static_cast<float *>(ws), s);
@@ -241,6 +251,14 @@
   const bool small = chain == CRW_CHAIN_F32 && Np <= 64;
 
   (void)nA;
+  if (small && walk_fused()) {
+    CRW_TRY(launch_walk_softmax_small(A, stats_ext, B, T - 1, N, Np, st.F.f, st.Gt.f, st.Lt.f, st.R.f, st.stats, st.ticket, s));
+    CRW_TRY(launch_chain_small_fwd(st.Gt.f, st.F.f, st.Lt.f, st.R.f, B, K, Np, s));
+    CRW_TRY(launch_walk_cycle_small(st.Lt.f, st.R.f, K * B, N, Np, st.At.f, st.lse, st.terms, 1.0f / ((float)B * (float)N * (float)N),
+                                    loss, st.ticket, s));
+    if (At_out) CRW_TRY(launch_unpad_At(st.At.f, K, B, N, Np, At_out, s));
+    return CRW_OK;
+  }
   CRW_TRY(launch_softmax_fwd(A, stats_ext, B, T - 1, N, Np, st.F.f, st.Gt.f, st.F.h, st.F.l, st.Gt.h, st.Gt.l, st.stats, s));
   if (chain == CRW_CHAIN_F32) {
     CRW_TRY(launch_identity(st.R.f, nullptr, B, Np, N, s, st.Lt.f, st.Gt.f));
@@ -302,6 +320,11 @@
   const bool small = chain == CRW_CHAIN_F32 && Np <= 64;
 
   const float coef = 1.0f / ((float)N * (float)B * (float)N);
+  if (small && walk_fused()) {
+    CRW_TRY(launch_walk_local_small(st.At.f, st.lse, gloss, coef, st.R.f, st.Lt.f, K * B, N, Np, sc.dLt.f, sc.dR.f, s));
+    CRW_TRY(launch_chain_small_bwd(st.Gt.f, st.F.f, sc.dLt.f, sc.dR.f, B, K, Np, s));
+    return launch_walk_softmax_bwd_small(A, st.stats, st.Lt.f, st.R.f, sc.dLt.f, sc.dR.f, B, T - 1, N, Np, dA, s);
+  }
   CRW_TRY(launch_dAt(st.At.f, st.lse, gloss, coef, K * B, N, Np, sc.dAt.f, sc.dAt.h, sc.dAt.l, s));
   if ((reinterpret_cast<uintptr_t>(sc.dF.f) | reinterpret_cast<uintptr_t>(sc.dGt.f)) & 15) {
     if (hipMemsetAsync(sc.dF.f, 0, sizeof(float) * BM, s) != hipSuccess) return CRW_EHIP;
@@ -372,6 +395,7 @@
   hipStream_t s = (hipStream_t)stream;
   const long NC = (long)N * C, NN = (long)N * N;
   if (C == 32 || C == 64 || C == 128) {
+    if (N <= 64 && walk_fused()) return launch_affinity_bwd_tiles(dA, ehat, B, T, N, C, tau, dehat_ws, s, norm, demb);
     CRW_TRY(launch_affinity_bwd_tiles(dA, ehat, B, T, N, C, tau, dehat_ws, s));
     const long rows_ = (long)B * T * N;
     hipLaunchKernelGGL(normalize_bwd_kernel, dim3((unsigned)((rows_ + 3) / 4)), dim3(256), 0, s, dehat_ws, ehat, norm, rows_, C, demb);
diff --git a/radar-sounder-crw_amd/csrc/walk_small.hip b/radar-sounder-crw_amd/csrc/walk_small.hip
--- /dev/null
+++ b/radar-sounder-crw_amd/csrc/walk_small.hip
@@ -0,0 +1,306 @@
+#include "crw_common.h"
+
+namespace crw {
+namespace {
+
+__device__ inline long caller_mat(long mat, int B, int Tm1) { return (mat % B) * Tm1 + mat / B; }
+
+template <int NP, bool TA, bool TB>
+__device__ inline f32x4 tile_mm(const float *as, int lda, const float *bs, int ldb, int r0, int c0, int lane, f32x4 acc) {
+  const int q = lane >> 4, c = lane & 15;
+#pragma unroll 4
+  for (int kk = 0; kk < NP; kk += 4) {
+    const int k = kk + q;
+    const float a = TA ? as[k * lda + r0 + c] : as[(r0 + c) * lda + k];
+    const float b = TB ? bs[(c0 + c) * ldb + k] : bs[k * ldb + c0 + c];
+    acc = __builtin_amdgcn_mfma_f32_16x16x4f32(a, b, acc, 0, 0, 0);
+  }
+  return acc;
+}
+
+template <int NP>
+__device__ inline void stage(const float *__restrict__ src, float *dst, int ld, int tid) {
+  const int e = 4 * tid, r = e / NP, c = e % NP;
+  *reinterpret_cast<float4 *>(dst + r * ld + c) = *reinterpret_cast<const float4 *>(src + e);
+}
+
+template <int NP>
+__global__ __launch_bounds__(NP * NP / 4) void walk_softmax_small_kernel(const float *__restrict__ A, const float *__restrict__ ext,
+                                                                         int B, int Tm1, int N, float *__restrict__ F,
+                                                                         float *__restrict__ Gt, float *__restrict__ Lt1,
+                                                                         float *__restrict__ R1, float *__restrict__ stats,
+                                                                         unsigned *__restrict__ ticket) {
+  constexpr int NTH = NP * NP / 4, NW = NTH / 64, LDA = NP + 1;
+  __shared__ float a[NP * LDA];
+  __shared__ float st[4][NP];
+  const long mat = blockIdx.x, amat = caller_mat(mat, B, Tm1), nmat = (long)B * Tm1;
+  const int tid = threadIdx.x, lane = tid & 63, wave = tid >> 6;
+  const float *ag = A + amat * N * N;
+  if (mat == 0 && tid == 0) *ticket = 0u;
+  for (int idx = tid; idx < N * N; idx += NTH) a[(idx / N) * LDA + idx % N] = ag[idx];
+  __syncthreads();
+  if (ext) {
+    for (int i = tid; i < 4 * N; i += NTH) st[i / N][i % N] = ext[((i / N) * nmat + amat) * N + i % N];
+  } else {
+    for (int row = wave; row < N; row += NW) {
+      const float *r = a + row * LDA;
+      const int c = 4 * lane;
+      const float x = c < N ? r[c] : -INFINITY, y = c + 1 < N ? r[c + 1] : -INFINITY;
+      const float z = c + 2 < N ? r[c + 2] : -INFINITY, w = c + 3 < N ? r[c + 3] : -INFINITY;
+      const float m = wave_max(fmaxf(fmaxf(-INFINITY, fmaxf(x, y)), fmaxf(z, w)));
+      float s = 0.f;
+      if (c < N) s += (expf(x - m) + expf(y - m)) + (expf(z - m) + expf(w - m));
+      s = wave_sum(s);
+      if (lane == 0) {
+        st[0][row] = m;
+        st[1][row] = s;
+      }
+    }
+    if (tid < N) {
+      float m = -INFINITY, s = 0.f;
+      for (int r = 0; r < N; ++r) {
+        const float v = a[r * LDA + tid];
+        if (v > m) {
+          s = s * expf(m - v) + 1.f;
+          m = v;
+        } else {
+          s += expf(v - m);
+        }
+      }
+      st[2][tid] = m;
+      st[3][tid] = s;
+    }
+  }
+  __syncthreads();
+  for (int i = tid; i < 4 * N; i += NTH) stats[((i / N) * nmat + mat) * NP + i % N] = st[i / N][i % N];
+  const int e = 4 * tid, row = e / NP, c0 = e % NP;
+  float f[4], g[4], id[4];
+#pragma unroll
+  for (int i = 0; i < 4; ++i) {
+    const int c = c0 + i;
+    f[i] = g[i] = 0.f;
+    if (row < N && c < N) {
+      const float v = a[row * LDA + c];
+      f[i] = expf(v - st[0][row]) / st[1][row];
+      g[i] = expf(v - st[2][c]) / st[3][c];
+    }
+    id[i] = (row == c && row < N) ? 1.f : 0.f;
+  }
+  const long o = mat * NP * NP + e;
+  *reinterpret_cast<float4 *>(F + o) = float4{f[0], f[1], f[2], f[3]};
+  *reinterpret_cast<float4 *>(Gt + o) = float4{g[0], g[1], g[2], g[3]};
+  if (mat < B) {
+    *reinterpret_cast<float4 *>(Lt1 + o) = float4{g[0], g[1], g[2], g[3]};
+    *reinterpret_cast<float4 *>(R1 + o) = float4{id[0], id[1], id[2], id[3]};
+  }
+}
+
+template <int NP>
+__global__ __launch_bounds__(NP * NP / 4) void walk_cycle_small_kernel(const float *__restrict__ Lt, const float *__restrict__ R, int N,
+                                                                       float *__restrict__ At, float *__restrict__ lse,
+                                                                       float *__restrict__ terms, float scale,
+                                                                       float *__restrict__ loss, unsigned *__restrict__ ticket) {
+  constexpr int NTH = NP * NP / 4, NW = NTH / 64, NT = NP / 16, LD = NP + 16, LDC = NP + 1;
+  __shared__ __attribute__((aligned(16))) float ls[NP * LD];
+  __shared__ __attribute__((aligned(16))) float rs[NP * LD];
+  __shared__ float red[NTH];
+  __shared__ unsigned drawn;
+  const long mat = blockIdx.x, M = (long)NP * NP;
+  const int tid = threadIdx.x, lane = tid & 63, wave = tid >> 6;
+  stage<NP>(Lt + mat * M, ls, LD, tid);
+  stage<NP>(R + mat * M, rs, LD, tid);
+  __syncthreads();
+  const int r0 = (wave / NT) * 16, c0 = (wave % NT) * 16;
+  const f32x4 acc = tile_mm<NP, true, false>(ls, LD, rs, LD, r0, c0, lane, f32x4{0.f, 0.f, 0.f, 0.f});
+  __syncthreads();
+  float *cs = ls;
+#pragma unroll
+  for (int r = 0; r < 4; ++r) {
+    const int row = r0 + (lane >> 4) * 4 + r, col = c0 + (lane & 15);
+    At[mat * M + (long)row * NP + col] = acc[r];
+    cs[row * LDC + col] = acc[r];
+  }
+  __syncthreads();
+  for (int row = wave; row < NP; row += NW) {
+    float l = 0.f, t = 0.f;
+    if (row < N) {
+      const float v = lane < N ? cs[row * LDC + lane] : -INFINITY;
+      const float m = wave_max(v);
+      const float s = wave_sum(lane < N ? expf(v - m) : 0.f);
+      l = logf(s) + m;
+      t = l - cs[row * LDC + row];
+    }
+    if (lane == 0) {
+      lse[mat * NP + row] = l;
+      __hip_atomic_store(&terms[mat * NP + row], t, __ATOMIC_RELAXED, __HIP_MEMORY_SCOPE_AGENT);
+    }
+  }
+  asm volatile("s_waitcnt vmcnt(0)" ::: "memory");
+  __syncthreads();
+  if (tid == 0) {
+    const unsigned t = __hip_atomic_fetch_add(ticket, 1u, __ATOMIC_RELEASE, __HIP_MEMORY_SCOPE_AGENT);
+    if (t == gridDim.x - 1) {
+      __builtin_amdgcn_fence(__ATOMIC_ACQUIRE, "agent");
+      asm volatile("s_waitcnt vmcnt(0)" ::: "memory");
+    }
+    drawn = t;
+  }
+  __syncthreads();
+  if (drawn != gridDim.x - 1) return;
+  const long n = (long)gridDim.x * NP;
+  float s = 0.f;
+  for (long i = tid; i < n; i += NTH) s += __hip_atomic_load(&terms[i], __ATOMIC_RELAXED, __HIP_MEMORY_SCOPE_AGENT);
+  red[tid] = s;
+  __syncthreads();
+  for (int o = NTH / 2; o > 0; o >>= 1) {
+    if (tid < o) red[tid] += red[tid + o];
+    __syncthreads();
+  }
+  if (tid == 0) {
+    loss[0] = red[0] * scale;
+    __hip_atomic_store(ticket, 0u, __ATOMIC_RELAXED, __HIP_MEMORY_SCOPE_AGENT);
+  }
+}
+
+template <int NP>
+__global__ __launch_bounds__(NP * NP / 4) void walk_local_small_kernel(const float *__restrict__ At, const float *__restrict__ lse,
+                                                                       const float *__restrict__ gloss, float coef,
+                                                                       const float *__restrict__ R, const float *__restrict__ Lt, int N,
+                                                                       float *__restrict__ dLt, float *__restrict__ dR) {
+  constexpr int NT = NP / 16, LD = NP + 4;
+  __shared__ __attribute__((aligned(16))) float rs[NP * LD];
+  __shared__ __attribute__((aligned(16))) float ls[NP * LD];
+  __shared__ __attribute__((aligned(16))) float ds[NP * LD];
+  const long mat = blockIdx.x, M = (long)NP * NP;
+  const int tid = threadIdx.x, lane = tid & 63, wave = tid >> 6;
+  stage<NP>(R + mat * M, rs, LD, tid);
+  stage<NP>(Lt + mat * M, ls, LD, tid);
+  {
+    const int e = 4 * tid, row = e / NP, c = e % NP;
+    const float g = gloss[0] * coef;
+    float4 v = float4{0.f, 0.f, 0.f, 0.f};
+    if (row < N && c < N) {
+      const float4 a = *reinterpret_cast<const float4 *>(At + mat * M + e);
+      const float l = lse[mat * NP + row];
+      v.x = g * (expf(a.x - l) - (c == row ? 1.f : 0.f));
+      v.y = c + 1 < N ? g * (expf(a.y - l) - (c + 1 == row ? 1.f : 0.f)) : 0.f;
+      v.z = c + 2 < N ? g * (expf(a.z - l) - (c + 2 == row ? 1.f : 0.f)) : 0.f;
+      v.w = c + 3 < N ? g * (expf(a.w - l) - (c + 3 == row ? 1.f : 0.f)) : 0.f;
+    }
+    *reinterpret_cast<float4 *>(ds + row * LD + c) = v;
+  }
+  __syncthreads();
+  const int r0 = (wave / NT) * 16, c0 = (wave % NT) * 16;
+  const f32x4 z = f32x4{0.f, 0.f, 0.f, 0.f};
+  const f32x4 a1 = tile_mm<NP, false, true>(rs, LD, ds, LD, r0, c0, lane, z);
+  const f32x4 a2 = tile_mm<NP, false, false>(ls, LD, ds, LD, r0, c0, lane, z);
+#pragma unroll
+  for (int r = 0; r < 4; ++r) {
+    const long o = mat * M + (long)(r0 + (lane >> 4) * 4 + r) * NP + c0 + (lane & 15);
+    dLt[o] = a1[r];
+    dR[o] = a2[r];
+  }
+}
+
+template <int NP>
+__global__ __launch_bounds__(NP * NP / 4) void walk_softmax_bwd_small_kernel(const float *__restrict__ A, const float *__restrict__ stats,
+                                                                             const float *__restrict__ Lt, const float *__restrict__ R,
+                                                                             const float *__restrict__ dLt, const float *__restrict__ dR,
+                                                                             int B, int Tm1, int N, float *__restrict__ dA) {
+  constexpr int NTH = NP * NP / 4, NW = NTH / 64, NT = NP / 16, LD = NP + 4, LDA = NP + 1;
+  __shared__ __attribute__((aligned(16))) float xs[NP * LD];
+  __shared__ __attribute__((aligned(16))) float ys[NP * LD];
+  __shared__ float a[NP * LDA];
+  __shared__ float st[4][NP];
+  __shared__ float rdot[NP], cdot[NP];
+  __shared__ float part[NW][64];
+  const long mat = blockIdx.x, amat = caller_mat(mat, B, Tm1), nmat = (long)B * Tm1;
+  const long M = (long)NP * NP, BM = (long)B * M;
+  const int j = (int)(mat / B), b = (int)(mat % B), K = Tm1 - 1;
+  const int tid = threadIdx.x, lane = tid & 63, wave = tid >> 6;
+  float *out = dA + amat * N * N;
+  if (j == K) {
+    for (int idx = tid; idx < N * N; idx += NTH) out[idx] = 0.f;
+    return;
+  }
+  const float *ag = A + amat * N * N;
+  for (int idx = tid; idx < N * N; idx += NTH) a[(idx / N) * LDA + idx % N] = ag[idx];
+  for (int i = tid; i < 4 * N; i += NTH) st[i / N][i % N] = stats[((i / N) * nmat + mat) * NP + i % N];
+  const int r0 = (wave / NT) * 16, c0 = (wave % NT) * 16;
+  f32x4 dg = f32x4{0.f, 0.f, 0.f, 0.f}, df = dg;
+  if (j == 0) {
+#pragma unroll
+    for (int r = 0; r < 4; ++r) dg[r] = dLt[(long)b * M + (long)(r0 + (lane >> 4) * 4 + r) * NP + c0 + (lane & 15)];
+  } else {
+    stage<NP>(dLt + j * BM + b * M, xs, LD, tid);
+    stage<NP>(Lt + (j - 1) * BM + b * M, ys, LD, tid);
+    __syncthreads();
+    dg = tile_mm<NP, false, true>(xs, LD, ys, LD, r0, c0, lane, dg);
+    __syncthreads();
+    stage<NP>(dR + j * BM + b * M, xs, LD, tid);
+    stage<NP>(R + (j - 1) * BM + b * M, ys, LD, tid);
+    __syncthreads();
+    df = tile_mm<NP, false, true>(xs, LD, ys, LD, r0, c0, lane, df);
+  }
+  __syncthreads();
+#pragma unroll
+  for (int r = 0; r < 4; ++r) {
+    const int o = (r0 + (lane >> 4) * 4 + r) * LD + c0 + (lane & 15);
+    xs[o] = dg[r];
+    ys[o] = df[r];
+  }
+  __syncthreads();
+  for (int row = wave; row < N; row += NW) {
+    const float s = wave_sum(lane < N ? expf(a[row * LDA + lane] - st[0][row]) * ys[row * LD + lane] : 0.f);
+    if (lane == 0) rdot[row] = s / st[1][row];
+  }
+  {
+    float s = 0.f;
+    if (lane < N)
+      for (int r = wave; r < N; r += NW) s += expf(a[r * LDA + lane] - st[2][lane]) * xs[r * LD + lane];
+    part[wave][lane] = s;
+  }
+  __syncthreads();
+  if (tid < N) {
+    float s = 0.f;
+#pragma unroll
+    for (int w = 0; w < NW; ++w) s += part[w][tid];
+    cdot[tid] = s / st[3][tid];
+  }
+  __syncthreads();
+  for (int idx = tid; idx < N * N; idx += NTH) {
+    const int row = idx / N, c = idx % N;
+    const float v = a[row * LDA + c];
+    out[idx] = expf(v - st[0][row]) / st[1][row] * (ys[row * LD + c] - rdot[row]) +
+               expf(v - st[2][c]) / st[3][c] * (xs[row * LD + c] - cdot[c]);
+  }
+}
+
+}
+
+#define CRW_WALK_SMALL_LAUNCH(kernel, blocks, ...)                                                                  \
+  do {                                                                                                              \
+    if (Np == 64) hipLaunchKernelGGL((kernel<64>), dim3(blocks), dim3(1024), 0, s, __VA_ARGS__);                    \
+    else if (Np == 32) hipLaunchKernelGGL((kernel<32>), dim3(blocks), dim3(256), 0, s, __VA_ARGS__);                \
+    else return CRW_EINVAL;                                                                                         \
+    return check_launch();                                                                                          \
+  } while (0)
+
+int launch_walk_softmax_small(const float *A, const float *stats_ext, int B, int Tm1, int N, int Np, float *F, float *Gt, float *Lt1,
+                              float *R1, float *stats, unsigned *ticket, hipStream_t s) {
+  CRW_WALK_SMALL_LAUNCH(walk_softmax_small_kernel, B * Tm1, A, stats_ext, B, Tm1, N, F, Gt, Lt1, R1, stats, ticket);
+}
+int launch_walk_cycle_small(const float *Lt, const float *R, int nmat, int N, int Np, float *At, float *lse, float *terms, float scale,
+                            float *loss, unsigned *ticket, hipStream_t s) {
+  CRW_WALK_SMALL_LAUNCH(walk_cycle_small_kernel, nmat, Lt, R, N, At, lse, terms, scale, loss, ticket);
+}
+int launch_walk_local_small(const float *At, const float *lse, const float *gloss, float coef, const float *R, const float *Lt, int nmat,
+                            int N, int Np, float *dLt, float *dR, hipStream_t s) {
+  CRW_WALK_SMALL_LAUNCH(walk_local_small_kernel, nmat, At, lse, gloss, coef, R, Lt, N, dLt, dR);
+}
+int launch_walk_softmax_bwd_small(const float *A, const float *stats, const float *Lt, const float *R, const float *dLt, const float *dR,
+                                  int B, int Tm1, int N, int Np, float *dA, hipStream_t s) {
+  CRW_WALK_SMALL_LAUNCH(walk_softmax_bwd_small_kernel, B * Tm1, A, stats, Lt, R, dLt, dR, B, Tm1, N, dA);
+}
+
+}
diff --git a/radar-sounder-crw_amd/encoder.py b/radar-sounder-crw_amd/encoder.py
--- a/radar-sounder-crw_amd/encoder.py
+++ b/radar-sounder-crw_amd/encoder.py
@@ -13,8 +13,7 @@
     def forward(ctx, x, w1, b1, w2, b2, w3, b3, w4, b4, w5, b5, split, bwd_split=None):
         import crw_hip
         x = x.contiguous()
-        w2p = crw_hip.enc_front_pack(w2, split)
-        packed = [crw_hip.enc_pack_weights(w, split) for w in (w3, w4, w5)]
+        w2p, *packed = crw_hip.enc_pack_all(w2, (w3, w4, w5), split)
         ctx.bwd_split = bwd_split or split
         x3h, x3l, fsaved = crw_hip.enc_front_fwd(split, x, w1, b1, w2p[:2], b2, save=True)
         y3h, y3l, _, _ = crw_hip.enc_conv3x3(0, split, x3h, x3l, packed[0][0], packed[0][1], 64, bias=b3)
@@ -61,8 +60,7 @@
         x = x.contiguous()
         P, _, h, w = x.shape
         H, W = h - 6, w - 6
-        w2p = crw_hip.enc_front_pack(w2, split)
-        packed = [crw_hip.enc_pack_weights(wt, split) for wt in (w3, w4, w5)]
+        w2p, *packed = crw_hip.enc_pack_all(w2, (w3, w4, w5), split)
         x3h, x3l = crw_hip.enc_front_fwd_map(split, x, w1, b1, w2p[:2], b2)
         y3h, y3l, _ = crw_hip.enc_conv3x3_map(split, x3h, x3l, packed[0][0], packed[0][1], 64, H, W, bias=b3)
         y4h, y4l, _ = crw_hip.enc_conv3x3_map(split, y3h, y3l, packed[1][0], packed[1][1], 128, H, W, bias=b4)
@@ -108,7 +106,8 @@
         import crw_hip
         x, w = ctx.saved_tensors
         dy = dy.contiguous()
-        return dy @ w, crw_hip.linear128_wgrad(dy, x), dy.sum(0)
+        dw, db = crw_hip.linear128_wgrad_bias(dy, x)
+        return dy @ w, dw, db
 
 
 _CNN_STACK = (("1", 8, 5, True), ("2", 32, 5, True), ("3", 64, 3, False), ("4", 128, 3, False), ("5", 128, 3, False))
```

Result: faster. 662,400 radargram columns/s (median of 6 runs) (+1.1%).
